# RulinShao/sink-flash-attention-kernel

Hardware: AMD Instinct MI355X
Metric: attn fwd+bwd TFLOP/s (% MFMA peak) at B=4 H=32 N=8192 D=128 bf16 (higher is better)
Workload: dtype bf16

## Files before the change

### include/sfa.h

```cpp
#ifndef SFA_H
#define SFA_H

#include <stddef.h>
#include <stdint.h>

#ifdef __cplusplus
extern "C" {
#endif

#define SFA_ABI_VERSION 2

#define SFA_DTYPE_F32 0
#define SFA_DTYPE_F16 1
#define SFA_DTYPE_BF16 2

#define SFA_OK 0
#define SFA_ERR_INVALID_ARGUMENT (-1)
#define SFA_ERR_UNSUPPORTED (-2)
#define SFA_ERR_WORKSPACE (-3)

#define SFA_FLAG_FORCE_GENERIC 0x1u
#define SFA_FLAG_DECODE_ONE_PASS 0x4u
#define SFA_FLAG_BWD_OVERLAP 0x8u
#define SFA_FLAG_BWD_DKDV_ASM 0x10u
#define SFA_FLAG_BWD_DKDV_WS 0x20u

typedef struct sfa_tensor {
    void* ptr;
    int64_t shape[4];
    int64_t stride[4];
    int32_t dtype;
    int32_t reserved;
} sfa_tensor;

int sfa_abi_version(void);

const char* sfa_last_error(void);

const char* sfa_last_path(void);

int sfa_debug_set_variant(int which, int value);
int sfa_debug_set_ptr(void* device_buffer);
int sfa_debug_set_stage_events(void* const* events, int count);

int sfa_fwd(const sfa_tensor* q, const sfa_tensor* k, const sfa_tensor* v, const sfa_tensor* o,
            float* lse, const float* s_aux, int num_sink, int window, float scale,
            unsigned flags, void* stream);

size_t sfa_bwd_workspace_bytes(int64_t B, int64_t Hq, int64_t Hkv, int64_t N, int64_t D, int dtype,
                               int num_sink, int window, unsigned flags);

int sfa_bwd(const sfa_tensor* q, const sfa_tensor* k, const sfa_tensor* v, const sfa_tensor* o,
            const sfa_tensor* d_o, const float* lse, const float* s_aux, const sfa_tensor* dq,
            const sfa_tensor* dk, const sfa_tensor* dv, float* ds_aux, void* workspace,
            size_t workspace_bytes, int num_sink, int window, float scale, unsigned flags,
            void* stream);

int sfa_varlen_supported(int dtype, int64_t D);

int sfa_fwd_varlen(const sfa_tensor* q, const sfa_tensor* k, const sfa_tensor* v, const sfa_tensor* o, float* lse,
                   const float* s_aux, const int32_t* cu_seqlens, int n_seq, int max_seqlen, int num_sink,
                   int window, float scale, unsigned flags, void* stream);

int sfa_bwd_varlen(const sfa_tensor* q, const sfa_tensor* k, const sfa_tensor* v, const sfa_tensor* o,
                   const sfa_tensor* d_o, const float* lse, const float* s_aux, const sfa_tensor* dq,
                   const sfa_tensor* dk, const sfa_tensor* dv, float* ds_aux, const int32_t* cu_seqlens, int n_seq,
                   int max_seqlen, void* workspace, size_t workspace_bytes, int num_sink, int window, float scale,
                   unsigned flags, void* stream);

size_t sfa_decode_workspace_bytes(int64_t B, int64_t Hq, int64_t Hkv, int64_t Nkv, int64_t D,
                                  int dtype);

int sfa_decode(const sfa_tensor* q, const sfa_tensor* k, const sfa_tensor* v, const sfa_tensor* o,
               const float* s_aux, void* workspace, size_t workspace_bytes, float scale,
               unsigned flags, void* stream);

int sfa_decode_ring(const sfa_tensor* q, const sfa_tensor* sink_k, const sfa_tensor* sink_v, int64_t sink_len,
                    const sfa_tensor* window_k, const sfa_tensor* window_v, int64_t window_len,
                    const sfa_tensor* o, const float* s_aux, void* workspace, size_t workspace_bytes,
                    float scale, unsigned flags, void* stream);

int sfa_decode_ring_step(const sfa_tensor* q, const sfa_tensor* sink_k, const sfa_tensor* sink_v, int64_t sink_len,
                         const sfa_tensor* window_k, const sfa_tensor* window_v, int64_t window_len,
                         int64_t write_pos, const sfa_tensor* k_new, const sfa_tensor* v_new, const sfa_tensor* o,
                         const float* s_aux, void* workspace, size_t workspace_bytes, float scale, unsigned flags,
                         void* stream);

int sfa_decode_ring_step_dyn(const sfa_tensor* q, const sfa_tensor* sink_k, const sfa_tensor* sink_v,
                             const sfa_tensor* window_k, const sfa_tensor* window_v, const sfa_tensor* k_new,
                             const sfa_tensor* v_new, const sfa_tensor* o, const float* s_aux, int32_t* state,
                             void* workspace, size_t workspace_bytes, float scale, unsigned flags, void* stream);

size_t sfa_decode_multi_workspace_bytes(int64_t B, int64_t Hq, int64_t Hkv, int64_t n_new, int64_t Nkv, int64_t D,
                                        int dtype);

int sfa_decode_ring_multi(const sfa_tensor* q, const sfa_tensor* sink_k, const sfa_tensor* sink_v, int64_t sink_len,
                          const sfa_tensor* window_k, const sfa_tensor* window_v, int64_t window_len,
                          int64_t write_pos, const sfa_tensor* k_new, const sfa_tensor* v_new, const sfa_tensor* o,
                          const float* s_aux, int commit, void* workspace, size_t workspace_bytes, float scale,
                          unsigned flags, void* stream);

int sfa_decode_ring_multi_dyn(const sfa_tensor* q, const sfa_tensor* sink_k, const sfa_tensor* sink_v,
                              const sfa_tensor* window_k, const sfa_tensor* window_v, const sfa_tensor* k_new,
                              const sfa_tensor* v_new, const sfa_tensor* o, const float* s_aux, int commit,
                              int32_t* state, void* workspace, size_t workspace_bytes, float scale, unsigned flags,
                              void* stream);

int sfa_ring_commit_dyn(const sfa_tensor* window_k, const sfa_tensor* window_v, const sfa_tensor* k_new,
                        const sfa_tensor* v_new, const int32_t* count, int32_t* state, void* stream);


int sfa_decode_ring_step_rows(const sfa_tensor* q, const sfa_tensor* sink_k, const sfa_tensor* sink_v,
                              const sfa_tensor* window_k, const sfa_tensor* window_v, const sfa_tensor* k_new,
                              const sfa_tensor* v_new, const sfa_tensor* o, const float* s_aux, int32_t* state,
                              void* workspace, size_t workspace_bytes, float scale, unsigned flags, void* stream);

int sfa_decode_ring_multi_rows(const sfa_tensor* q, const sfa_tensor* sink_k, const sfa_tensor* sink_v,
                               const sfa_tensor* window_k, const sfa_tensor* window_v, const sfa_tensor* k_new,
                               const sfa_tensor* v_new, const sfa_tensor* o, const float* s_aux, int commit,
                               int32_t* state, void* workspace, size_t workspace_bytes, float scale, unsigned flags,
                               void* stream);

int sfa_ring_commit_rows(const sfa_tensor* window_k, const sfa_tensor* window_v, const sfa_tensor* k_new,
                         const sfa_tensor* v_new, const int32_t* count, int32_t* state, void* stream);

int sfa_ring_fill_varlen(const sfa_tensor* sink_k, const sfa_tensor* sink_v, const sfa_tensor* window_k,
                         const sfa_tensor* window_v, const sfa_tensor* k, const sfa_tensor* v,
                         const int32_t* cu_seqlens, int n_seq, int32_t* state, void* stream);

int sfa_decode_ring_tree(const sfa_tensor* q, const sfa_tensor* sink_k, const sfa_tensor* sink_v, int64_t sink_len,
                         const sfa_tensor* window_k, const sfa_tensor* window_v, int64_t window_len,
                         int64_t write_pos, const sfa_tensor* k_new, const sfa_tensor* v_new, const sfa_tensor* o,
                         const float* s_aux, const int32_t* parent, int64_t parent_bstride, void* workspace,
                         size_t workspace_bytes, float scale, unsigned flags, void* stream);

int sfa_decode_ring_tree_dyn(const sfa_tensor* q, const sfa_tensor* sink_k, const sfa_tensor* sink_v,
                             const sfa_tensor* window_k, const sfa_tensor* window_v, const sfa_tensor* k_new,
                             const sfa_tensor* v_new, const sfa_tensor* o, const float* s_aux, const int32_t* parent,
                             int64_t parent_bstride, int32_t* state, void* workspace, size_t workspace_bytes,
                             float scale, unsigned flags, void* stream);

int sfa_decode_ring_tree_rows(const sfa_tensor* q, const sfa_tensor* sink_k, const sfa_tensor* sink_v,
                              const sfa_tensor* window_k, const sfa_tensor* window_v, const sfa_tensor* k_new,
                              const sfa_tensor* v_new, const sfa_tensor* o, const float* s_aux, const int32_t* parent,
                              int64_t parent_bstride, int32_t* state, void* workspace, size_t workspace_bytes,
                              float scale, unsigned flags, void* stream);

int sfa_ring_commit_path_dyn(const sfa_tensor* window_k, const sfa_tensor* window_v, const sfa_tensor* k_new,
                             const sfa_tensor* v_new, const int32_t* count, const int32_t* path, int64_t path_bstride,
                             int32_t* state, void* stream);

int sfa_ring_commit_path_rows(const sfa_tensor* window_k, const sfa_tensor* window_v, const sfa_tensor* k_new,
                              const sfa_tensor* v_new, const int32_t* count, const int32_t* path, int64_t path_bstride,
                              int32_t* state, void* stream);


int sfa_decode_ring_step_slots(const sfa_tensor* q, const sfa_tensor* sink_k, const sfa_tensor* sink_v,
                               const sfa_tensor* window_k, const sfa_tensor* window_v, const sfa_tensor* k_new,
                               const sfa_tensor* v_new, const sfa_tensor* o, const float* s_aux, int32_t* state,
                               const int32_t* slots, void* workspace, size_t workspace_bytes, float scale,
                               unsigned flags, void* stream);

int sfa_decode_ring_multi_slots(const sfa_tensor* q, const sfa_tensor* sink_k, const sfa_tensor* sink_v,
                                const sfa_tensor* window_k, const sfa_tensor* window_v, const sfa_tensor* k_new,
                                const sfa_tensor* v_new, const sfa_tensor* o, const float* s_aux, int commit,
                                int32_t* state, const int32_t* slots, void* workspace, size_t workspace_bytes,
                                float scale, unsigned flags, void* stream);

int sfa_decode_ring_tree_slots(const sfa_tensor* q, const sfa_tensor* sink_k, const sfa_tensor* sink_v,
                               const sfa_tensor* window_k, const sfa_tensor* window_v, const sfa_tensor* k_new,
                               const sfa_tensor* v_new, const sfa_tensor* o, const float* s_aux, const int32_t* parent,
                               int64_t parent_bstride, int32_t* state, const int32_t* slots, void* workspace,
                               size_t workspace_bytes, float scale, unsigned flags, void* stream);

int sfa_ring_commit_slots(const sfa_tensor* window_k, const sfa_tensor* window_v, const sfa_tensor* k_new,
                          const sfa_tensor* v_new, const int32_t* count, int32_t* state, const int32_t* slots,
                          void* stream);

int sfa_ring_commit_path_slots(const sfa_tensor* window_k, const sfa_tensor* window_v, const sfa_tensor* k_new,
                               const sfa_tensor* v_new, const int32_t* count, const int32_t* path, int64_t path_bstride,
                               int32_t* state, const int32_t* slots, void* stream);

int sfa_ring_fill_varlen_slots(const sfa_tensor* sink_k, const sfa_tensor* sink_v, const sfa_tensor* window_k,
                               const sfa_tensor* window_v, const sfa_tensor* k, const sfa_tensor* v,
                               const int32_t* cu_seqlens, int n_seq, int32_t* state, const int32_t* slots,
                               void* stream);

size_t sfa_decode_ragged_workspace_bytes(int64_t n_seq, int64_t Hq, int64_t Hkv, int64_t T, int64_t Nkv_cache,
                                         int64_t D, int dtype);

int sfa_decode_ring_ragged_slots(const sfa_tensor* q, const sfa_tensor* sink_k, const sfa_tensor* sink_v,
                                 const sfa_tensor* window_k, const sfa_tensor* window_v, const sfa_tensor* k_new,
                                 const sfa_tensor* v_new, const sfa_tensor* o, const float* s_aux, int commit,
                                 int32_t* state, const int32_t* slots, const int32_t* cu_q, int n_seq,
                                 void* workspace, size_t workspace_bytes, float scale, unsigned flags, void* stream);

#ifdef __cplusplus
}
#endif
#endif
```

### sink-flash-attention-kernel_amd/csrc/sfa_api.hip

```cpp
#include <cmath>
#include <cstring>
#include <initializer_list>

#include "sfa_common.hpp"
#include "sfa_internal.hpp"

namespace sfa {

static thread_local char g_err[512] = "";
static char g_path[128] = "";

void* g_debug_ptr = nullptr;
int g_variant[8] = {0, 0, 0, 0, 0, 0, 0, 0};
static void* const* g_stage_events = nullptr;
static int g_stage_count = 0;
bool stage_events_armed() { return g_stage_events != nullptr; }
void record_stage(int i, hipStream_t stream) {
    if (g_stage_events && i < g_stage_count && g_stage_events[i]) (void)hipEventRecord((hipEvent_t)g_stage_events[i], stream);
}

void set_error(const char* fmt, ...) {
    va_list ap;
    va_start(ap, fmt);
    vsnprintf(g_err, sizeof(g_err), fmt, ap);
    va_end(ap);
}
void set_path(const char* fmt, ...) {
    va_list ap;
    va_start(ap, fmt);
    vsnprintf(g_path, sizeof(g_path), fmt, ap);
    va_end(ap);
}

namespace {

int check_tensor(const sfa_tensor* t, const char* name) {
    SFA_CHECK_ARG(t != nullptr, "%s: null tensor descriptor", name);
    SFA_CHECK_ARG(t->dtype == SFA_DTYPE_F32 || t->dtype == SFA_DTYPE_F16 || t->dtype == SFA_DTYPE_BF16,
                  "%s: unknown dtype %d", name, t->dtype);
    for (int i = 0; i < 4; ++i) SFA_CHECK_ARG(t->shape[i] >= 0, "%s: negative shape[%d]", name, i);
    const bool empty = t->shape[0] == 0 || t->shape[1] == 0 || t->shape[2] == 0 || t->shape[3] == 0;
    SFA_CHECK_ARG(empty || t->ptr != nullptr, "%s: null data pointer", name);
    SFA_CHECK_ARG(t->shape[3] <= 1 || t->stride[3] == 1, "%s: last-dim stride must be 1 (got %lld)", name,
                  (long long)t->stride[3]);
    for (int i = 0; i < 3; ++i)
        SFA_CHECK_ARG(t->stride[i] >= 0, "%s: negative stride[%d] not supported", name, i);
    return SFA_OK;
}

int same_shape(const sfa_tensor* a, const sfa_tensor* b, const char* an, const char* bn) {
    for (int i = 0; i < 4; ++i)
        SFA_CHECK_ARG(a->shape[i] == b->shape[i], "%s and %s differ in shape[%d]: %lld vs %lld", an, bn, i,
                      (long long)a->shape[i], (long long)b->shape[i]);
    SFA_CHECK_ARG(a->dtype == b->dtype, "%s and %s differ in dtype", an, bn);
    return SFA_OK;
}

int check_prefill(const sfa_tensor* q, const sfa_tensor* k, const sfa_tensor* v, Problem* p, int num_sink,
                  int window, float scale) {
    int st;
    if ((st = check_tensor(q, "q")) || (st = check_tensor(k, "k")) || (st = check_tensor(v, "v"))) return st;
    if ((st = same_shape(k, v, "k", "v"))) return st;
    SFA_CHECK_ARG(q->dtype == k->dtype, "q and k differ in dtype");
    SFA_CHECK_ARG(q->shape[0] == k->shape[0], "batch mismatch: q %lld vs k %lld", (long long)q->shape[0],
                  (long long)k->shape[0]);
    SFA_CHECK_ARG(q->shape[2] <= k->shape[2], "prefill needs N_q <= N_kv (q %lld, k %lld)", (long long)q->shape[2],
                  (long long)k->shape[2]);
    SFA_CHECK_ARG(q->shape[3] == k->shape[3], "head dim mismatch");
    SFA_CHECK_ARG(k->shape[1] > 0 && q->shape[1] % k->shape[1] == 0, "H_q (%lld) must be divisible by H_kv (%lld)",
                  (long long)q->shape[1], (long long)k->shape[1]);
    SFA_CHECK_ARG(q->shape[2] < (1ll << 30) && q->shape[0] * q->shape[1] < (1ll << 30), "problem too large");
    SFA_CHECK_ARG(num_sink >= 0, "num_sink must be >= 0");
    SFA_CHECK_ARG(std::isfinite(scale), "scale must be finite");
    p->B = (int)q->shape[0];
    p->Hq = (int)q->shape[1];
    p->Hkv = (int)k->shape[1];
    p->N = (int)q->shape[2];
    p->Nk = (int)k->shape[2];
    p->D = (int)q->shape[3];
    p->num_sink = num_sink;
    p->window = window;
    p->scale = scale;
    return SFA_OK;
}

inline size_t align256(size_t x) { return (x + 255) & ~(size_t)255; }

struct BwdWorkspace {
    size_t delta_off, dsaux_off, mfma_off, total;
};

BwdWorkspace bwd_layout(const Problem& p, int dtype, bool use_mfma, unsigned flags) {
    BwdWorkspace w;
    size_t off = 0;
    w.delta_off = off;
    off += align256((size_t)p.B * p.Hq * p.N * sizeof(float));
    w.dsaux_off = off;
    off += align256((size_t)p.B * p.Hq * (size_t)bwd_preprocess_nblk(p.N) * sizeof(float));
    w.mfma_off = off;
    if (use_mfma) off += align256(bwd_mfma_workspace_bytes(p, dtype, flags));
    w.total = off;
    return w;
}

}
}

using namespace sfa;

extern "C" {

int sfa_abi_version(void) { return SFA_ABI_VERSION; }
const char* sfa_last_error(void) { return g_err; }
const char* sfa_last_path(void) { return g_path; }
int sfa_debug_set_variant(int which, int value) {
    if (which < 0 || which >= 8) return SFA_ERR_INVALID_ARGUMENT;
    __atomic_store_n(&sfa::g_variant[which], value, __ATOMIC_RELAXED);
    return SFA_OK;
}

int sfa_debug_set_ptr(void* p) {
    sfa::g_debug_ptr = p;
    return SFA_OK;
}

int sfa_debug_set_stage_events(void* const* events, int count) {
    g_stage_events = count > 0 ? events : nullptr;
    g_stage_count = count > 0 ? count : 0;
    return SFA_OK;
}

int sfa_fwd(const sfa_tensor* q, const sfa_tensor* k, const sfa_tensor* v, const sfa_tensor* o, float* lse,
            const float* s_aux, int num_sink, int window, float scale, unsigned flags, void* stream) {
    g_err[0] = 0;
    Problem p;
    int st = check_prefill(q, k, v, &p, num_sink, window, scale);
    if (st) return st;
    if ((st = check_tensor(o, "o")) || (st = same_shape(q, o, "q", "o"))) return st;
    if (p.B == 0 || p.Hq == 0 || p.N == 0) return SFA_OK;
    SFA_CHECK_ARG(p.D > 0, "head dim must be > 0");
    SFA_CHECK_ARG(lse != nullptr, "lse: null pointer");
    hipStream_t s = (hipStream_t)stream;
    if (!(flags & SFA_FLAG_FORCE_GENERIC) && fwd_mfma_supported(q->dtype, p.D))
        return fwd_mfma(q, k, v, o, lse, s_aux, p, s);
    if (p.Nk != p.N) {
        set_error("N_q != N_kv is served by the MFMA kernels only (16-bit dtypes, head dims 64/80/96/128)");
        return SFA_ERR_UNSUPPORTED;
    }
    return fwd_generic(q, k, v, o, lse, s_aux, p, s);
}

size_t sfa_bwd_workspace_bytes(int64_t B, int64_t Hq, int64_t Hkv, int64_t N, int64_t D, int dtype, int num_sink,
                               int window, unsigned flags) {
    Problem p{(int)B, (int)Hq, (int)Hkv, (int)N, (int)D, num_sink, window, 1.f};
    const bool use_mfma = !(flags & SFA_FLAG_FORCE_GENERIC) && bwd_mfma_supported(dtype, (int)D);
    return bwd_layout(p, dtype, use_mfma, flags).total;
}

int sfa_bwd(const sfa_tensor* q, const sfa_tensor* k, const sfa_tensor* v, const sfa_tensor* o,
            const sfa_tensor* d_o, const float* lse, const float* s_aux, const sfa_tensor* dq, const sfa_tensor* dk,
            const sfa_tensor* dv, float* ds_aux, void* workspace, size_t workspace_bytes, int num_sink, int window,
            float scale, unsigned flags, void* stream) {
    g_err[0] = 0;
    Problem p;
    int st = check_prefill(q, k, v, &p, num_sink, window, scale);
    if (st) return st;
    if ((st = check_tensor(o, "o")) || (st = same_shape(q, o, "q", "o"))) return st;
    if ((st = check_tensor(d_o, "do")) || (st = same_shape(q, d_o, "q", "do"))) return st;
    if ((st = check_tensor(dq, "dq")) || (st = same_shape(q, dq, "q", "dq"))) return st;
    if ((st = check_tensor(dk, "dk")) || (st = same_shape(k, dk, "k", "dk"))) return st;
    if ((st = check_tensor(dv, "dv")) || (st = same_shape(v, dv, "v", "dv"))) return st;
    if (p.B == 0 || p.Hq == 0 || p.N == 0) return SFA_OK;
    SFA_CHECK_ARG(p.D > 0, "head dim must be > 0");
    SFA_CHECK_ARG(lse != nullptr, "lse: null pointer");
    SFA_CHECK_ARG((s_aux == nullptr) == (ds_aux == nullptr), "ds_aux must be given iff s_aux is");
    const bool use_mfma = !(flags & SFA_FLAG_FORCE_GENERIC) && bwd_mfma_supported(q->dtype, p.D);
    if (use_mfma && (st = bwd_mfma_refused(q, k, v, d_o, dq, dk, dv, p))) return st;
    const BwdWorkspace w = bwd_layout(p, q->dtype, use_mfma, flags);
    if (workspace == nullptr || workspace_bytes < w.total || ((uintptr_t)workspace & 255) != 0) {
        set_error("bwd workspace: need %zu bytes, 256-byte aligned (got %zu at %p)", w.total, workspace_bytes,
                  workspace);
        return SFA_ERR_WORKSPACE;
    }
    hipStream_t s = (hipStream_t)stream;
    float* delta = reinterpret_cast<float*>((char*)workspace + w.delta_off);
    float* dsaux_part = reinterpret_cast<float*>((char*)workspace + w.dsaux_off);
    record_stage(0, s);
    const bool fuse = use_mfma && bwd_mfma_wants_consts() && bwd_preprocess_vectorised(o, d_o, p);
    st = bwd_preprocess(o, d_o, lse, s_aux, delta, dsaux_part, ds_aux, p, s,
                        fuse ? reinterpret_cast<float*>((char*)workspace + w.mfma_off) : nullptr, bwd_mfma_lse_factor(p, flags));
    record_stage(1, s);
    if (st) return st;
    if (use_mfma)
        st = bwd_mfma(q, k, v, d_o, lse, delta, dq, dk, dv, (char*)workspace + w.mfma_off, p, flags, s, fuse);
    else if (p.Nk != p.N) {
        set_error("N_q != N_kv is served by the MFMA kernels only (16-bit dtypes, head dims 64/80/96/128)");
        st = SFA_ERR_UNSUPPORTED;
    } else
        st = bwd_generic(q, k, v, d_o, lse, delta, dq, dk, dv, p, s);
    record_stage(3, s);
    return st;
}

int sfa_varlen_supported(int dtype, int64_t D) {
    return fwd_mfma_supported(dtype, (int)D) && bwd_mfma_varlen_supported(dtype, (int)D) ? 1 : 0;
}

static int check_varlen(const sfa_tensor* q, const sfa_tensor* k, const sfa_tensor* v, const int32_t* cu, int n_seq,
                        int max_seqlen, int num_sink, int window, float scale, Problem* p, Problem* run) {
    int st = check_prefill(q, k, v, p, num_sink, window, scale);
    if (st) return st;
    SFA_CHECK_ARG(p->B == 1, "packed layout: batch dim must be 1 (got %d)", p->B);
    SFA_CHECK_ARG(p->N == p->Nk, "packed layout: q and k must have the same number of rows");
    SFA_CHECK_ARG(cu != nullptr && n_seq >= 1, "cu_seqlens: need a device array of n_seq + 1 >= 2 offsets");
    SFA_CHECK_ARG(max_seqlen >= 1 && max_seqlen <= p->N, "max_seqlen %d out of range (total rows %d)", max_seqlen, p->N);
    if (!sfa_varlen_supported(q->dtype, p->D)) {
        set_error("packed (varlen) kernels exist for 16-bit dtypes and head dims 64/80/96/128 only");
        return SFA_ERR_UNSUPPORTED;
    }
    *run = *p;
    run->B = n_seq;
    run->N = max_seqlen;
    run->cu = cu;
    run->n_total = p->N;
    run->Nk = 0;
    return SFA_OK;
}

int sfa_fwd_varlen(const sfa_tensor* q, const sfa_tensor* k, const sfa_tensor* v, const sfa_tensor* o, float* lse,
                   const float* s_aux, const int32_t* cu_seqlens, int n_seq, int max_seqlen, int num_sink, int window,
                   float scale, unsigned flags, void* stream) {
    g_err[0] = 0;
    (void)flags;
    Problem p, run;
    int st = check_varlen(q, k, v, cu_seqlens, n_seq, max_seqlen, num_sink, window, scale, &p, &run);
    if (st) return st;
    if ((st = check_tensor(o, "o")) || (st = same_shape(q, o, "q", "o"))) return st;
    if (p.Hq == 0 || p.N == 0) return SFA_OK;
    SFA_CHECK_ARG(lse != nullptr, "lse: null pointer");
    return fwd_mfma(q, k, v, o, lse, s_aux, run, (hipStream_t)stream);
}

int sfa_bwd_varlen(const sfa_tensor* q, const sfa_tensor* k, const sfa_tensor* v, const sfa_tensor* o,
                   const sfa_tensor* d_o, const float* lse, const float* s_aux, const sfa_tensor* dq,
                   const sfa_tensor* dk, const sfa_tensor* dv, float* ds_aux, const int32_t* cu_seqlens, int n_seq,
                   int max_seqlen, void* workspace, size_t workspace_bytes, int num_sink, int window, float scale,
                   unsigned flags, void* stream) {
    g_err[0] = 0;
    (void)flags;
    Problem p, run;
    int st = check_varlen(q, k, v, cu_seqlens, n_seq, max_seqlen, num_sink, window, scale, &p, &run);
    if (st) return st;
    if ((st = check_tensor(o, "o")) || (st = same_shape(q, o, "q", "o"))) return st;
    if ((st = check_tensor(d_o, "do")) || (st = same_shape(q, d_o, "q", "do"))) return st;
    if ((st = check_tensor(dq, "dq")) || (st = same_shape(q, dq, "q", "dq"))) return st;
    if ((st = check_tensor(dk, "dk")) || (st = same_shape(k, dk, "k", "dk"))) return st;
    if ((st = check_tensor(dv, "dv")) || (st = same_shape(v, dv, "v", "dv"))) return st;
    if (p.Hq == 0 || p.N == 0) return SFA_OK;
    SFA_CHECK_ARG(lse != nullptr, "lse: null pointer");
    SFA_CHECK_ARG((s_aux == nullptr) == (ds_aux == nullptr), "ds_aux must be given iff s_aux is");
    if ((st = bwd_mfma_refused(q, k, v, d_o, dq, dk, dv, run))) return st;
    const BwdWorkspace w = bwd_layout(p, q->dtype, true, 0);
    if (workspace == nullptr || workspace_bytes < w.total || ((uintptr_t)workspace & 255) != 0) {
        set_error("bwd workspace: need %zu bytes, 256-byte aligned (got %zu at %p)", w.total, workspace_bytes,
                  workspace);
        return SFA_ERR_WORKSPACE;
    }
    hipStream_t s = (hipStream_t)stream;
    float* delta = reinterpret_cast<float*>((char*)workspace + w.delta_off);
    float* dsaux_part = reinterpret_cast<float*>((char*)workspace + w.dsaux_off);
    record_stage(0, s);
    const bool fuse = bwd_mfma_wants_consts() && bwd_preprocess_vectorised(o, d_o, p);
    st = bwd_preprocess(o, d_o, lse, s_aux, delta, dsaux_part, ds_aux, p, s,
                        fuse ? reinterpret_cast<float*>((char*)workspace + w.mfma_off) : nullptr,
                        bwd_mfma_lse_factor(run, flags));
    record_stage(1, s);
    if (st) return st;
    st = bwd_mfma(q, k, v, d_o, lse, delta, dq, dk, dv, (char*)workspace + w.mfma_off, run, flags, s, fuse);
    record_stage(3, s);
    return st;
}

size_t sfa_decode_workspace_bytes(int64_t B, int64_t Hq, int64_t Hkv, int64_t Nkv, int64_t D, int dtype) {
    DecodePlan pl;
    if (decode_plan(B, Hq, Hkv, Nkv, D, dtype, &pl) != SFA_OK) return 0;
    return decode_counter_bytes(B, Hkv) + align256((size_t)B * Hq * pl.max_splits * (size_t)(D + 2) * sizeof(float));
}

}

namespace {

#define SFA_NEED(p, what) SFA_CHECK_ARG((p) != nullptr, what ": null device pointer")

int check_rows16(std::initializer_list<const sfa_tensor*> ts, int es, unsigned skip, const char* msg) {
    for (const sfa_tensor* t : ts) {
        if (!t || ((skip & 1) && t->shape[0] == 0) || ((skip & 2) && t->shape[1] == 0) || ((skip & 4) && t->shape[2] == 0))
            continue;
        SFA_CHECK_ARG(((uintptr_t)t->ptr % 16) == 0 && (t->stride[0] * es) % 16 == 0 && (t->stride[1] * es) % 16 == 0 &&
                          (t->stride[2] * es) % 16 == 0,
                      "%s", msg);
    }
    return SFA_OK;
}

int check_workspace(const char* name, size_t need, bool sized, void* workspace, size_t workspace_bytes) {
    if (!sized || workspace == nullptr || workspace_bytes < need || ((uintptr_t)workspace & 255) != 0) {
        set_error("%s workspace: need %zu bytes, 256-byte aligned (got %zu at %p)", name, need, workspace_bytes, workspace);
        return SFA_ERR_WORKSPACE;
    }
    return SFA_OK;
}

RingCall attend_call(const sfa_tensor* q, const sfa_tensor* sink_k, const sfa_tensor* sink_v, const sfa_tensor* window_k,
                     const sfa_tensor* window_v, const sfa_tensor* k_new, const sfa_tensor* v_new, const sfa_tensor* o,
                     const float* s_aux, void* workspace, size_t workspace_bytes, float scale, unsigned flags,
                     void* stream) {
    RingCall c{};
    c.q = q, c.sink_k = sink_k, c.sink_v = sink_v, c.window_k = window_k, c.window_v = window_v;
    c.k_new = k_new, c.v_new = v_new, c.o = o, c.s_aux = s_aux;
    c.workspace = workspace, c.workspace_bytes = workspace_bytes;
    c.scale = scale, c.flags = flags, c.stream = (hipStream_t)stream;
    return c;
}

RingCall& host_state(RingCall& c, int64_t sink_len, int64_t window_len, int64_t write_pos) {
    c.mode = RingState::Host, c.sink_len = sink_len, c.window_len = window_len, c.write_pos = write_pos;
    return c;
}

RingCall& device_state(RingCall& c, RingState mode, int32_t* state, const int32_t* slots) {
    c.mode = mode, c.state = state, c.slots = slots;
    c.sink_len = c.sink_k ? c.sink_k->shape[2] : 0, c.window_len = c.window_k ? c.window_k->shape[2] : 0;
    return c;
}

int check_device_state(const RingCall& c) {
    if (c.mode == RingState::Host) return SFA_OK;
    SFA_NEED(c.state, "state");
    SFA_CHECK_ARG(c.sink_k != nullptr && c.window_k != nullptr, "cache buffers: null tensor descriptor");
    return SFA_OK;
}

int ring_step(const RingCall& c) {
    g_err[0] = 0;
    int st;
    if ((st = check_device_state(c))) return st;
    const sfa_tensor *q = c.q, *k = c.sink_k, *v = c.sink_v, *k2 = c.window_k, *v2 = c.window_v, *o = c.o;
    const sfa_tensor *k_new = c.k_new, *v_new = c.v_new;
    const int64_t n1 = c.sink_len, n2 = c.window_len;
    const bool pool = c.slots != nullptr;
    if ((st = check_tensor(q, "q")) || (st = check_tensor(k, "k")) || (st = check_tensor(v, "v")) ||
        (st = check_tensor(o, "o")))
        return st;
    if ((st = same_shape(k, v, "k", "v")) || (st = same_shape(q, o, "q", "o"))) return st;
    SFA_CHECK_ARG(q->dtype == k->dtype, "q and k differ in dtype");
    SFA_CHECK_ARG(q->shape[2] == 1, "sink_decode_attention requires N_q=1, got %lld", (long long)q->shape[2]);
    if (pool)
        SFA_CHECK_ARG(k->shape[0] >= 1 && k->shape[0] < (1ll << 30),
                      "pool: the cache buffers need shape[0] = S slots, 1 <= S < 2^30 (got %lld)", (long long)k->shape[0]);
    SFA_CHECK_ARG((pool || q->shape[0] == k->shape[0]) && q->shape[3] == k->shape[3], "q/k batch or head-dim mismatch");
    SFA_CHECK_ARG(k->shape[1] > 0 && q->shape[1] % k->shape[1] == 0, "H_q (%lld) must be divisible by H_kv (%lld)",
                  (long long)q->shape[1], (long long)k->shape[1]);
    SFA_CHECK_ARG(std::isfinite(c.scale), "scale must be finite");
    SFA_CHECK_ARG(n1 >= 0 && n1 <= k->shape[2], "first key segment: %lld valid rows of %lld", (long long)n1,
                  (long long)k->shape[2]);
    if (k2 || v2 || n2) {
        SFA_CHECK_ARG(k2 && v2, "second key segment needs both k and v");
        if ((st = check_tensor(k2, "k2")) || (st = check_tensor(v2, "v2")) || (st = same_shape(k2, v2, "k2", "v2")))
            return st;
        if (pool)
            SFA_CHECK_ARG(k2->shape[0] == k->shape[0], "pool: sink and window buffers must share shape[0] = S (sink %lld, window %lld)",
                          (long long)k->shape[0], (long long)k2->shape[0]);
        SFA_CHECK_ARG(k2->dtype == k->dtype && k2->shape[0] == k->shape[0] && k2->shape[1] == k->shape[1] &&
                          k2->shape[3] == k->shape[3],
                      "the two key segments must agree in dtype, batch, heads and head dim");
        SFA_CHECK_ARG(n2 >= 0 && n2 <= k2->shape[2], "second key segment: %lld valid rows of %lld", (long long)n2,
                      (long long)k2->shape[2]);
    }
    SFA_CHECK_ARG(n1 + n2 < (1ll << 31) - 4096, "N_kv too large");
    if (k_new || v_new) {
        SFA_CHECK_ARG(k_new && v_new && k2 && v2, "fused step needs k_new, v_new and the window ring");
        if ((st = check_tensor(k_new, "k_new")) || (st = check_tensor(v_new, "v_new")) ||
            (st = same_shape(k_new, v_new, "k_new", "v_new")))
            return st;
        if (pool)
            SFA_CHECK_ARG(k_new->shape[0] == q->shape[0], "q, k_new, v_new and o must share shape[0] = B (q %lld, k_new %lld)",
                          (long long)q->shape[0], (long long)k_new->shape[0]);
        SFA_CHECK_ARG(k_new->dtype == k2->dtype && (pool || k_new->shape[0] == k2->shape[0]) && k_new->shape[1] == k2->shape[1] &&
                          k_new->shape[2] == 1 && k_new->shape[3] == k2->shape[3],
                      "k_new / v_new must be [B, H_kv, 1, D] in the ring's dtype");
        SFA_CHECK_ARG(c.mode != RingState::Host || (c.write_pos >= 0 && c.write_pos < n2),
                      "write slot %lld outside the %lld valid ring slots", (long long)c.write_pos, (long long)n2);
// ... 403 lines not shown
```

### sink-flash-attention-kernel_amd/csrc/sfa_bwd_mfma.hip

```cpp
#include "sfa_common.hpp"
#include "sfa_internal.hpp"
#include "sfa_worklist.hpp"

#include <cstdlib>
#include <type_traits>

#include "gen/dkdv_asm.inc"
#include "gen/dq_asm.inc"
#include "gen/dkdv_skew_asm.inc"
#include "gen/dq_strip_asm.inc"

namespace sfa {
namespace {

typedef __attribute__((ext_vector_type(8))) __bf16 bf16x8_t;
typedef __attribute__((ext_vector_type(8))) _Float16 f16x8_t;
typedef __attribute__((ext_vector_type(4))) short s16x4;
typedef __attribute__((ext_vector_type(8))) short s16x8;
typedef __attribute__((ext_vector_type(16))) float f32x16;
typedef __attribute__((ext_vector_type(4))) float f32x4;
typedef __attribute__((ext_vector_type(4))) unsigned int u32x4;
typedef __attribute__((ext_vector_type(2))) unsigned int u32x2;

#ifdef SFA_STAMPS
// ... 769 lines not shown
    s.q_lo = u((unsigned)qb); s.q_hi = u((unsigned)(qb >> 32));
    s.do_lo = u((unsigned)dob); s.do_hi = u((unsigned)(dob >> 32));
    s.c_lo = u((unsigned)cb); s.c_hi = u((unsigned)(cb >> 32));
    s.k_lo = u((unsigned)kbp); s.k_hi = u((unsigned)(kbp >> 32));
    s.v_lo = u((unsigned)vbp); s.v_hi = u((unsigned)(vbp >> 32));
    s.dk_lo = u((unsigned)dkb); s.dk_hi = u((unsigned)(dkb >> 32));
    s.dv_lo = u((unsigned)dvb); s.dv_hi = u((unsigned)(dvb >> 32));
    const bool split = (kb < a.sink_blocks ? a.sink_chunks : a.gen_chunks) > 1;
    s.pk_lo = s.pk_hi = s.pv_lo = s.pv_hi = s.p_rng = u(0u);
    if (split) {
        const uint64_t pb = (uint64_t)(a.sink_ws) +
                            ((uint64_t)grp * part_slots(a, a.n_kblocks) + part_first(a, kb) + chunk) * 2 * a.sink_rows * D * 4 -
                            (uint64_t)kb0 * D * 4;
        const uint64_t pvb = pb + (uint64_t)a.sink_rows * D * 4;
        s.pk_lo = u((unsigned)pb); s.pk_hi = u((unsigned)(pb >> 32));
        s.pv_lo = u((unsigned)pvb); s.pv_hi = u((unsigned)(pvb >> 32));
        s.p_rng = u((unsigned)((kb0 + a.sink_rows) * D * 4));
    }
    s.q_rng = u(seq_range(a.cu, a.q_range, N, a.q.sn, D));
    s.do_rng = u(seq_range(a.cu, a.do_range, N, a.d_o.sn, D));
    s.c_rng = u((unsigned)((2 * NT_ - sq.row0) * 4));
    s.k_rng = u(seq_range(a.cu, a.k_range, Nk, a.k.sn, D));
    s.v_rng = u(seq_range(a.cu, a.v_range, Nk, a.v.sn, D));
    s.dk_rng = u(seq_range(a.cu, a.dk_range, Nk, a.dk.sn, D));
    s.dv_rng = u(seq_range(a.cu, a.dv_range, Nk, a.dv.sn, D));
    s.q_sn = u((unsigned)(a.q.sn * 2)); s.do_sn = u((unsigned)(a.d_o.sn * 2));
    s.k_sn = u((unsigned)(a.k.sn * 2)); s.v_sn = u((unsigned)(a.v.sn * 2));
    s.dk_sn = u((unsigned)(a.dk.sn * 2)); s.dv_sn = u((unsigned)(a.dv.sn * 2));
    if (chunk > 0) s.dk_rng = s.dv_rng = u(0u);
    s.q_hs = u((unsigned)(a.q.sh * 2)); s.do_hs = u((unsigned)(a.d_o.sh * 2));
    s.c_hs = u((unsigned)(2 * NT_ * 4));
    s.nq = u((unsigned)nq); s.g = u((unsigned)g); s.q_row0 = u((unsigned)(qt_lo * 32)); s.kb0 = u((unsigned)kb0);
    s.pos0 = u((unsigned)P); s.W = u((unsigned)W); s.ns = u((unsigned)a.num_sink); s.nrows = u((unsigned)N);
    s.cdelta = u((unsigned)(NT_ * 4));
    s.c_log2 = u(__float_as_uint(a.scale_log2)); s.scale = u(__float_as_uint(a.scale));
#ifdef SFA_DKDV_STAMPS
    s.dbg_lo = u((unsigned)(uint64_t)a.dbg); s.dbg_hi = u((unsigned)((uint64_t)a.dbg >> 32)); s.bid = u((unsigned)bid);
#endif
    const unsigned tid = threadIdx.x;
    if (a.B < 0) smem[tid] = 0;
#ifdef SFA_AB
    if constexpr (ALT == 1) {
        asm volatile(SFA_DKDV_ASM_BF16_ALT : : SFA_DKDV_INPUTS(s), [tid] "v"(tid) : SFA_DKDV_CLOBBERS);
        return;
    }
#endif
#define SFA_DKDV_BODY(DD)                                                                                        \
    if constexpr (D == DD) {                                                                                       \
        if constexpr (std::is_same<T, bf16_t>::value)                                                              \
            asm volatile(SFA_DKDV_ASM_BF16_D##DD : : SFA_DKDV_INPUTS(s), [tid] "v"(tid) : SFA_DKDV_CLOBBERS);       \
        else                                                                                                       \
            asm volatile(SFA_DKDV_ASM_F16_D##DD : : SFA_DKDV_INPUTS(s), [tid] "v"(tid) : SFA_DKDV_CLOBBERS);        \
    }
    SFA_DKDV_BODY(64) SFA_DKDV_BODY(80) SFA_DKDV_BODY(96) SFA_DKDV_BODY(128)
#undef SFA_DKDV_BODY
}

template <typename T, int D>
__global__ __launch_bounds__(256) void bwd_dkdv_skew_asm_kernel(BwdArgs a) {
    extern __shared__ __attribute__((aligned(16))) char smem[];
    const int nK = a.n_kblocks;
    const int bid = xcd_remap((int)blockIdx.x, (int)gridDim.x);
    const int kb = bid % nK, grp = bid / nK;
    const int hk = grp % a.Hkv;
    const int b = grp / a.Hkv;
    const SeqInfo sq = seq_of(a.cu, b, a.N);
    const int N = sq.N;
    const int W = a.window < N ? a.window : N;
    const int NT_ = a.cu ? a.n_total : N;
    const int g = a.Hq / a.Hkv;
    const int kb0 = kb * kKBA;
    if (kb0 >= N) return;
    int trips = (62 + W) / 32 + 1;
    if (trips < SFA_DKDVSK_SKEW) trips = SFA_DKDVSK_SKEW;
    const int head0 = hk * g;
    const uint64_t qb = (uint64_t)(a.q.ptr + ((int64_t)sq.bb * a.q.sb + (int64_t)head0 * a.q.sh + (int64_t)sq.row0 * a.q.sn) * 2);
    const uint64_t dob = (uint64_t)(a.d_o.ptr + ((int64_t)sq.bb * a.d_o.sb + (int64_t)head0 * a.d_o.sh + (int64_t)sq.row0 * a.d_o.sn) * 2);
    const uint64_t cb = (uint64_t)(a.consts + ((int64_t)sq.bb * a.Hq + head0) * 2 * NT_ + sq.row0);
    const uint64_t kbp = (uint64_t)(a.k.ptr + ((int64_t)sq.bb * a.k.sb + (int64_t)hk * a.k.sh + (int64_t)sq.row0 * a.k.sn) * 2);
    const uint64_t vbp = (uint64_t)(a.v.ptr + ((int64_t)sq.bb * a.v.sb + (int64_t)hk * a.v.sh + (int64_t)sq.row0 * a.v.sn) * 2);
    const uint64_t dkb = (uint64_t)(a.dk.ptr + ((int64_t)sq.bb * a.dk.sb + (int64_t)hk * a.dk.sh + (int64_t)sq.row0 * a.dk.sn) * 2);
    const uint64_t dvb = (uint64_t)(a.dv.ptr + ((int64_t)sq.bb * a.dv.sb + (int64_t)hk * a.dv.sh + (int64_t)sq.row0 * a.dv.sn) * 2);
    auto u = [](unsigned x) { return (unsigned)__builtin_amdgcn_readfirstlane((int)x); };
    DkdvSkewScalars s;
    s.q_lo = u((unsigned)qb); s.q_hi = u((unsigned)(qb >> 32));
    s.do_lo = u((unsigned)dob); s.do_hi = u((unsigned)(dob >> 32));
    s.c_lo = u((unsigned)cb); s.c_hi = u((unsigned)(cb >> 32));
    s.k_lo = u((unsigned)kbp); s.k_hi = u((unsigned)(kbp >> 32));
    s.v_lo = u((unsigned)vbp); s.v_hi = u((unsigned)(vbp >> 32));
    s.dk_lo = u((unsigned)dkb); s.dk_hi = u((unsigned)(dkb >> 32));
    s.dv_lo = u((unsigned)dvb); s.dv_hi = u((unsigned)(dvb >> 32));
    s.q_rng = u(seq_range(a.cu, a.q_range, N, a.q.sn, D));
    s.do_rng = u(seq_range(a.cu, a.do_range, N, a.d_o.sn, D));
    s.c_rng = u((unsigned)((2 * NT_ - sq.row0) * 4));
    s.k_rng = u(seq_range(a.cu, a.k_range, N, a.k.sn, D));
    s.v_rng = u(seq_range(a.cu, a.v_range, N, a.v.sn, D));
    s.dk_rng = u(seq_range(a.cu, a.dk_range, N, a.dk.sn, D));
    s.dv_rng = u(seq_range(a.cu, a.dv_range, N, a.dv.sn, D));
    s.q_sn = u((unsigned)(a.q.sn * 2)); s.do_sn = u((unsigned)(a.d_o.sn * 2));
    s.k_sn = u((unsigned)(a.k.sn * 2)); s.v_sn = u((unsigned)(a.v.sn * 2));
    s.dk_sn = u((unsigned)(a.dk.sn * 2)); s.dv_sn = u((unsigned)(a.dv.sn * 2));
    s.q_hs = u((unsigned)(a.q.sh * 2)); s.do_hs = u((unsigned)(a.d_o.sh * 2));
    s.c_hs = u((unsigned)(2 * NT_ * 4));
    s.nq = u((unsigned)trips); s.g = u((unsigned)g); s.q_row0 = u((unsigned)kb0); s.kb0 = u((unsigned)kb0);
    s.W = u((unsigned)W); s.nrows = u((unsigned)N);
    s.cdelta = u((unsigned)(NT_ * 4));
    s.c_log2 = u(__float_as_uint(a.scale_log2)); s.scale = u(__float_as_uint(a.scale));
    const unsigned tid = threadIdx.x;
    if (a.B < 0) smem[tid] = 0;
#define SFA_DKDVSK_BODY(DD)                                                                                          \
    if constexpr (D == DD) {                                                                                           \
        if constexpr (std::is_same<T, bf16_t>::value)                                                                  \
            asm volatile(SFA_DKDVSK_ASM_BF16_D##DD : : SFA_DKDVSK_INPUTS(s), [tid] "v"(tid) : SFA_DKDVSK_CLOBBERS);     \
        else                                                                                                           \
            asm volatile(SFA_DKDVSK_ASM_F16_D##DD : : SFA_DKDVSK_INPUTS(s), [tid] "v"(tid) : SFA_DKDVSK_CLOBBERS);      \
    }
    SFA_DKDVSK_BODY(64) SFA_DKDVSK_BODY(80) SFA_DKDVSK_BODY(96)
#undef SFA_DKDVSK_BODY
}

constexpr int kDynTicketDword = 512;
template <typename T, int D, int ALT>
__global__ __launch_bounds__(256) void bwd_dq_asm_pk_kernel(BwdArgs a) {
    extern __shared__ __attribute__((aligned(16))) char smem[];
    const int G = (int)gridDim.x, w = (int)blockIdx.x;
    const unsigned tid = threadIdx.x;
    const int n_groups = a.hgroups * a.Hkv * a.B;
    const int64_t n_ranks = (int64_t)a.n_qtiles * n_groups;
    const int g = a.Hq / a.Hkv, BM = 64 * a.rb, ns = a.num_sink;
    auto u = [](unsigned x) { return (unsigned)__builtin_amdgcn_readfirstlane((int)x); };
#ifdef SFA_WL_STAMPS
    const unsigned wl_t0 = u((unsigned)__builtin_amdgcn_s_memrealtime());
    const unsigned wl_c0 = u((unsigned)__builtin_amdgcn_s_memtime());
#endif
    DqPkScalars s;
    s.q_hs = u((unsigned)(a.q.sh * 2)); s.q_sn = u((unsigned)(a.q.sn * 2));
    s.do_hs = u((unsigned)(a.d_o.sh * 2)); s.do_sn = u((unsigned)(a.d_o.sn * 2));
    s.dq_hs = u((unsigned)(a.dq.sh * 2)); s.dq_sn = u((unsigned)(a.dq.sn * 2));
    s.k_sn = u((unsigned)(a.k.sn * 2)); s.v_sn = u((unsigned)(a.v.sn * 2));
    s.ld_hs = u((unsigned)((a.cu ? a.n_total : a.N) * 4));
    s.pos0 = u((unsigned)(a.cu ? 0 : a.Nk - a.N)); s.W = u((unsigned)a.window); s.ns = u((unsigned)ns);
    s.hpw_log2 = u(a.hpw == 4 ? 2u : (a.hpw == 2 ? 1u : 0u));
    s.c_log2 = u(__float_as_uint(a.scale_log2)); s.nlog2e = u(__float_as_uint(-kLog2e)); s.scale = u(__float_as_uint(a.scale));
    const int64_t n_static = a.wl_dyn > 0 && a.wl_dyn < n_ranks ? a.wl_dyn : n_ranks;
    int n_done = 0;
    for (bool first = true;; first = false) {
        const int j = (int)tid;
        bool valid = false;
        unsigned d[SFA_WL_DESC_DWORDS];
#pragma unroll
        for (int i = 0; i < SFA_WL_DESC_DWORDS; ++i) d[i] = 0;
        int64_t r_dyn = -1;
        if (!first) {
            __syncthreads();
            if (tid == 0) reinterpret_cast<volatile int*>(smem)[8] = (int)atomicAdd(a.tickets + kDynTicketDword, 1u);
            __syncthreads();
            r_dyn = n_static + reinterpret_cast<volatile int*>(smem)[8];
            if (r_dyn >= n_ranks) break;
        }
        {
            const int64_t r = first ? ((int64_t)j * G < n_static ? wl_rank(j, w, G) : -1) : (j == 0 ? r_dyn : -1);
            const int qt = a.n_qtiles - 1 - (int)((r < 0 ? 0 : r) / n_groups);
            int rest = (int)((r < 0 ? 0 : r) % n_groups);
            if (r >= 0 && r < (first ? n_static : n_ranks)) {
                const int hg = rest % a.hgroups;
                rest /= a.hgroups;
                const int hk = rest % a.Hkv;
                const int b = rest / a.Hkv;
                const SeqInfo sq = seq_of(a.cu, b, a.N);
                const int N = sq.N;
                const int P = a.cu ? 0 : a.Nk - a.N;
                const int Nk = N + P;
                const int W = a.window < Nk ? a.window : Nk;
                const int q0 = qt * BM;
                if (q0 < N) {
                    valid = true;
                    const int q1 = (q0 + BM < N) ? q0 + BM : N;
                    const int ns_eff = ns < q1 + P ? ns : q1 + P;
                    const int ts_hi = (ns_eff + 63) >> 6;
                    int wlo = q0 + P - W + 1;
                    if (wlo < 0) wlo = 0;
                    int tw_lo = wlo >> 6;
                    if (tw_lo < ts_hi) tw_lo = ts_hi;
                    const int tw_hi = (q1 + P + 63) >> 6;
                    if (tw_lo > tw_hi) tw_lo = tw_hi;
                    const int head0 = hk * g + hg * a.hpw;
                    const int64_t lrow = a.cu ? (int64_t)head0 * a.n_total + sq.row0 : ((int64_t)b * a.Hq + head0) * N;
                    const uint64_t qb = (uint64_t)(a.q.ptr + ((int64_t)sq.bb * a.q.sb + (int64_t)head0 * a.q.sh + (int64_t)sq.row0 * a.q.sn) * 2);
                    const uint64_t dob = (uint64_t)(a.d_o.ptr + ((int64_t)sq.bb * a.d_o.sb + (int64_t)head0 * a.d_o.sh + (int64_t)sq.row0 * a.d_o.sn) * 2);
                    const uint64_t dqb = (uint64_t)(a.dq.ptr + ((int64_t)sq.bb * a.dq.sb + (int64_t)head0 * a.dq.sh + (int64_t)sq.row0 * a.dq.sn) * 2);
                    const uint64_t kbp = (uint64_t)(a.k.ptr + ((int64_t)sq.bb * a.k.sb + (int64_t)hk * a.k.sh + (int64_t)sq.row0 * a.k.sn) * 2);
                    const uint64_t vbp = (uint64_t)(a.v.ptr + ((int64_t)sq.bb * a.v.sb + (int64_t)hk * a.v.sh + (int64_t)sq.row0 * a.v.sn) * 2);
                    const uint64_t lb = (uint64_t)(a.lse + lrow), db_ = (uint64_t)(a.delta + lrow);
                    d[SFA_DQPK_F_q_lo] = (unsigned)qb; d[SFA_DQPK_F_q_hi] = (unsigned)(qb >> 32);
                    d[SFA_DQPK_F_do_lo] = (unsigned)dob; d[SFA_DQPK_F_do_hi] = (unsigned)(dob >> 32);
                    d[SFA_DQPK_F_lse_lo] = (unsigned)lb; d[SFA_DQPK_F_lse_hi] = (unsigned)(lb >> 32);
                    d[SFA_DQPK_F_dl_lo] = (unsigned)db_; d[SFA_DQPK_F_dl_hi] = (unsigned)(db_ >> 32);
                    d[SFA_DQPK_F_dq_lo] = (unsigned)dqb; d[SFA_DQPK_F_dq_hi] = (unsigned)(dqb >> 32);
                    d[SFA_DQPK_F_q0] = (unsigned)q0; d[SFA_DQPK_F_nrows] = (unsigned)N;
                    d[SFA_DQPK_F_q_rng] = seq_range(a.cu, a.q_range, N, a.q.sn, D);
                    d[SFA_DQPK_F_do_rng] = seq_range(a.cu, a.do_range, N, a.d_o.sn, D);
                    d[SFA_DQPK_F_dq_rng] = seq_range(a.cu, a.dq_range, N, a.dq.sn, D);
                    d[SFA_DQPK_F_k_lo] = (unsigned)kbp; d[SFA_DQPK_F_k_hi] = (unsigned)(kbp >> 32);
                    d[SFA_DQPK_F_v_lo] = (unsigned)vbp; d[SFA_DQPK_F_v_hi] = (unsigned)(vbp >> 32);
                    d[SFA_DQPK_F_k_rng] = seq_range(a.cu, a.k_range, Nk, a.k.sn, D);
                    d[SFA_DQPK_F_v_rng] = seq_range(a.cu, a.v_range, Nk, a.v.sn, D);
                    d[SFA_DQPK_F_nt] = (unsigned)(ts_hi + (tw_hi - tw_lo));
                    d[SFA_DQPK_F_ts_hi] = (unsigned)ts_hi; d[SFA_DQPK_F_tw_off] = (unsigned)(tw_lo - ts_hi);
                }
            }
        }
        int n_items = 0;
        const int idx = wl_compact(valid, reinterpret_cast<int*>(smem), &n_items);
        if (valid) {
            uint4* dst = reinterpret_cast<uint4*>(smem + SFA_DQPK_DESC_BASE + idx * (SFA_WL_DESC_DWORDS * 4));
#pragma unroll
            for (int i = 0; i < SFA_WL_DESC_DWORDS / 4; ++i) dst[i] = make_uint4(d[4 * i], d[4 * i + 1], d[4 * i + 2], d[4 * i + 3]);
        }
        __syncthreads();
        s.n_items = u((unsigned)n_items);
        n_done += n_items;
#ifdef SFA_DQPK_STAMPS
        s.dbg_lo = u((unsigned)(uint64_t)a.dbg); s.dbg_hi = u((unsigned)((uint64_t)a.dbg >> 32)); s.bid = u((unsigned)blockIdx.x);
#endif
        if (n_items > 0) {
#ifdef SFA_AB
            if constexpr (ALT == 1) asm volatile(SFA_DQPK_ASM_BF16_ALT : : SFA_DQPK_INPUTS(s), [tid] "v"(tid) : SFA_DQPK_CLOBBERS);
#endif
#define SFA_DQPK_BODY(DD)                                                                                      \
    if constexpr (D == DD && ALT == 0) {                                                                         \
        if constexpr (std::is_same<T, bf16_t>::value)                                                            \
            asm volatile(SFA_DQPK_ASM_BF16_D##DD : : SFA_DQPK_INPUTS(s), [tid] "v"(tid) : SFA_DQPK_CLOBBERS);     \
        else                                                                                                     \
            asm volatile(SFA_DQPK_ASM_F16_D##DD : : SFA_DQPK_INPUTS(s), [tid] "v"(tid) : SFA_DQPK_CLOBBERS);      \
    }
            SFA_DQPK_BODY(64) SFA_DQPK_BODY(80) SFA_DQPK_BODY(96) SFA_DQPK_BODY(128)
#undef SFA_DQPK_BODY
        }
        if (n_static >= n_ranks) break;
    }
    {
#ifdef SFA_WL_STAMPS
        if (a.dbg && threadIdx.x == 0) {
            unsigned* rec = reinterpret_cast<unsigned*>(a.dbg) + 4 * blockIdx.x;
            rec[0] = wl_t0;
            rec[1] = (unsigned)__builtin_amdgcn_s_memrealtime();
            rec[2] = (unsigned)__builtin_amdgcn_s_getreg(20 | (3 << 11));
            rec[3] = ((unsigned)n_done & 1023u) | ((((unsigned)__builtin_amdgcn_s_memtime() - wl_c0) >> 4) << 10);
        }
#endif
    }
    (void)n_done;
}

template <typename T, int D, int NT>
__global__ __launch_bounds__(256) void bwd_dq_strip_asm_kernel(BwdArgs a) {
    extern __shared__ __attribute__((aligned(16))) char smem[];
    const int bid = xcd_remap(blockIdx.x, gridDim.x);
    const int sidx = bid % a.n_strips;
    int rest = bid / a.n_strips;
    const int hg = rest % a.hgroups;
    rest /= a.hgroups;
    const int hk = rest % a.Hkv;
    const int b = rest / a.Hkv;
    const SeqInfo sq = seq_of(a.cu, b, a.N);
    const int N = sq.N;
    const int q0 = sidx * a.strip * 64;
    if (q0 >= N) return;
    const int n_tiles = (N + 63) >> 6;
    int n_it = n_tiles - sidx * a.strip;
    if (n_it > a.strip) n_it = a.strip;
    const int g = a.Hq / a.Hkv;
    const int head0 = hk * g + hg * 4;
    const int64_t lrow = a.cu ? (int64_t)head0 * a.n_total + sq.row0 : ((int64_t)b * a.Hq + head0) * N;
    const uint64_t qb = (uint64_t)(a.q.ptr + ((int64_t)sq.bb * a.q.sb + (int64_t)head0 * a.q.sh + (int64_t)sq.row0 * a.q.sn) * 2);
    const uint64_t dob = (uint64_t)(a.d_o.ptr + ((int64_t)sq.bb * a.d_o.sb + (int64_t)head0 * a.d_o.sh + (int64_t)sq.row0 * a.d_o.sn) * 2);
    const uint64_t dqb = (uint64_t)(a.dq.ptr + ((int64_t)sq.bb * a.dq.sb + (int64_t)head0 * a.dq.sh + (int64_t)sq.row0 * a.dq.sn) * 2);
    const uint64_t kbp = (uint64_t)(a.k.ptr + ((int64_t)sq.bb * a.k.sb + (int64_t)hk * a.k.sh + (int64_t)sq.row0 * a.k.sn) * 2);
    const uint64_t vbp = (uint64_t)(a.v.ptr + ((int64_t)sq.bb * a.v.sb + (int64_t)hk * a.v.sh + (int64_t)sq.row0 * a.v.sn) * 2);
    const uint64_t lb = (uint64_t)(a.lse + lrow), db_ = (uint64_t)(a.delta + lrow);
    auto u = [](unsigned x) { return (unsigned)__builtin_amdgcn_readfirstlane((int)x); };
    DqStripScalars s;
    s.q_lo = u((unsigned)qb); s.q_hi = u((unsigned)(qb >> 32)); s.q_hs = u((unsigned)(a.q.sh * 2));
    s.q_sn = u((unsigned)(a.q.sn * 2)); s.q_rng = u(seq_range(a.cu, a.q_range, N, a.q.sn, D));
    s.do_lo = u((unsigned)dob); s.do_hi = u((unsigned)(dob >> 32)); s.do_hs = u((unsigned)(a.d_o.sh * 2));
    s.do_sn = u((unsigned)(a.d_o.sn * 2)); s.do_rng = u(seq_range(a.cu, a.do_range, N, a.d_o.sn, D));
    s.dq_lo = u((unsigned)dqb); s.dq_hi = u((unsigned)(dqb >> 32)); s.dq_hs = u((unsigned)(a.dq.sh * 2));
    s.dq_sn = u((unsigned)(a.dq.sn * 2)); s.dq_rng = u(seq_range(a.cu, a.dq_range, N, a.dq.sn, D));
    s.k_lo = u((unsigned)kbp); s.k_hi = u((unsigned)(kbp >> 32)); s.k_sn = u((unsigned)(a.k.sn * 2));
    s.k_rng = u(seq_range(a.cu, a.k_range, N, a.k.sn, D));
    s.v_lo = u((unsigned)vbp); s.v_hi = u((unsigned)(vbp >> 32)); s.v_sn = u((unsigned)(a.v.sn * 2));
    s.v_rng = u(seq_range(a.cu, a.v_range, N, a.v.sn, D));
    s.lse_lo = u((unsigned)lb); s.lse_hi = u((unsigned)(lb >> 32)); s.dl_lo = u((unsigned)db_); s.dl_hi = u((unsigned)(db_ >> 32));
    s.ld_hs = u((unsigned)((a.cu ? a.n_total : N) * 4));
    s.q0 = u((unsigned)q0); s.n_it = u((unsigned)n_it); s.nrows = u((unsigned)N);
    s.W = u((unsigned)(a.window < N ? a.window : N));
    s.c_log2 = u(__float_as_uint(a.scale_log2)); s.nlog2e = u(__float_as_uint(-kLog2e)); s.scale = u(__float_as_uint(a.scale));
    const unsigned tid = threadIdx.x;
    if (a.B < 0) smem[tid] = 0;
#define SFA_DQSTRIP_BODY(DD, NN)                                                                                          \
    if constexpr (D == DD && NT == NN) {                                                                                    \
        if constexpr (std::is_same<T, bf16_t>::value)                                                                       \
            asm volatile(SFA_DQSTRIP_ASM_BF16_D##DD##_NT##NN : : SFA_DQSTRIP_INPUTS(s), [tid] "v"(tid) : SFA_DQSTRIP_CLOBBERS); \
        else                                                                                                                \
            asm volatile(SFA_DQSTRIP_ASM_F16_D##DD##_NT##NN : : SFA_DQSTRIP_INPUTS(s), [tid] "v"(tid) : SFA_DQSTRIP_CLOBBERS);  \
    }
    SFA_DQSTRIP_BODY(64, 2) SFA_DQSTRIP_BODY(64, 3) SFA_DQSTRIP_BODY(64, 4)
    SFA_DQSTRIP_BODY(80, 2) SFA_DQSTRIP_BODY(80, 3) SFA_DQSTRIP_BODY(80, 4)
#undef SFA_DQSTRIP_BODY
}
// ... 561 lines not shown
}
int device_cu_count();
bool asm_window_ok(int D, int window, int64_t wgs) {
    static const int min_window = env_int("SFA_ASM_MIN_WINDOW", kAsmMinWindow);
    if (D == 128) return true;
    if (!(D >= 64 && D < 128)) return false;
    return window > min_window || wgs >= 2 * (int64_t)device_cu_count();
}
int device_cu_count() {
    static const int n_cu = [] {
        int dev = 0, n = 256;
        if (hipGetDevice(&dev) != hipSuccess || hipDeviceGetAttribute(&n, hipDeviceAttributeMultiprocessorCount, dev) != hipSuccess) n = 256;
        return n > 0 ? n : 256;
    }();
    return n_cu;
}
constexpr int kSkewMaxWindow = 512;
bool dkdv_skew(int D, int window, int num_sink, bool self_attn, unsigned flags) {
    static const int knob = env_int("SFA_DKDV_SKEW", 1);
    if (!(D == 64 || D == 80 || D == 96) || knob != 1 || dkdv_mode() != 4) return false;
    if (flags & (SFA_FLAG_BWD_DKDV_WS | SFA_FLAG_BWD_DKDV_ASM)) return false;
    return num_sink <= 0 && self_attn && window >= 1 && window <= kSkewMaxWindow;
}
bool dkdv_asm(int D, int window, int Nk, int groups, bool can_split, unsigned flags, int num_sink, bool self_attn) {
    if (dkdv_skew(D, window, num_sink, self_attn, flags)) return true;
    if (!(dkdv_mode() == 4 && asm_window_ok(D, window, cdiv64(Nk, kKBA) * groups))) return false;
    if (flags & SFA_FLAG_BWD_DKDV_WS) return false;
    if (flags & SFA_FLAG_BWD_DKDV_ASM) return true;
    static const int min_wgs = env_int("SFA_DKDV_MIN_WGS", -1);
    static const int row_split = env_int("SFA_ROW_SPLIT", 1);
    const int64_t need = min_wgs >= 0 ? min_wgs : device_cu_count();
    return cdiv64(Nk, kKBA) * groups >= need || (can_split && row_split == 1);
}

struct SideStream {
    int dev = -1;
    hipStream_t stream = nullptr;
    hipEvent_t fork = nullptr, join = nullptr;
};
struct SideStreams {
    SideStream slot[16];
    int n = 0;
    ~SideStreams() {
        for (int i = 0; i < n; ++i) {
            if (slot[i].fork) (void)hipEventDestroy(slot[i].fork);
            if (slot[i].join) (void)hipEventDestroy(slot[i].join);
            if (slot[i].stream) (void)hipStreamDestroy(slot[i].stream);
        }
    }
};
SideStream* side_stream(hipStream_t caller) {
    thread_local SideStreams tls;
    int dev = -1;
    if (hipGetDevice(&dev) != hipSuccess) return nullptr;
    for (int i = 0; i < tls.n; ++i)
        if (tls.slot[i].dev == dev) return &tls.slot[i];
    hipStreamCaptureStatus cs = hipStreamCaptureStatusNone;
    if (hipStreamIsCapturing(caller, &cs) != hipSuccess || cs != hipStreamCaptureStatusNone) return nullptr;
    if (tls.n >= 16) return nullptr;
    SideStream s;
    s.dev = dev;
    int prio_least = 0, prio_greatest = 0;
    (void)hipDeviceGetStreamPriorityRange(&prio_least, &prio_greatest);
    if (hipStreamCreateWithPriority(&s.stream, hipStreamNonBlocking, prio_least) != hipSuccess) return nullptr;
    if (hipEventCreateWithFlags(&s.fork, hipEventDisableTiming) != hipSuccess ||
        hipEventCreateWithFlags(&s.join, hipEventDisableTiming) != hipSuccess) {
        if (s.fork) (void)hipEventDestroy(s.fork);
        (void)hipStreamDestroy(s.stream);
        return nullptr;
    }
    tls.slot[tls.n] = s;
    return &tls.slot[tls.n++];
}

int64_t worklist_grid(int64_t n_ranks) {
    const int64_t n_cu = device_cu_count();
    int64_t G = n_ranks < n_cu ? n_ranks : n_cu;
    const int64_t need = cdiv64(n_ranks, SFA_WL_MAX_ITEMS);
    return G > need ? G : need;
}

template <typename T, int D>
int launch_bwd(const BwdArgs& a, int B, hipStream_t stream) {
    constexpr int ROWB = (D <= 64) ? 128 : 256;
    const bool self_attn = a.cu != nullptr || a.Nk == a.N;
    bool skew = false;
    if constexpr (D == 64 || D == 80 || D == 96) skew = dkdv_skew(D, a.window, a.num_sink, self_attn, a.flags);
    const int mode = skew ? 5 : (dkdv_asm(D, a.window, a.Nk, a.Hkv * B, a.cu == nullptr && a.Nk == a.N, a.flags, a.num_sink, self_attn) ? 4 : 3);
    if (!a.consts_ready) {
        const int rows = a.cu ? a.n_total : a.N;
        const int64_t total = (a.cu ? 1 : (int64_t)B) * a.Hq * rows;
        bwd_consts_kernel<<<dim3((unsigned)cdiv64(total, 256)), dim3(256), 0, stream>>>(
            a.lse, a.delta, const_cast<float*>(a.consts), rows, total, mode >= 4 ? 1.f / a.scale : kLog2e);
    }
    static const int dq_asm_knob = env_int("SFA_DQ", 1);
    bool overlap = false;
    SideStream* ss = nullptr;
    if constexpr (D >= 64) {
        const int gq = a.Hq / a.Hkv, hpwq = gq % 4 == 0 ? 4 : (gq % 2 == 0 ? 2 : 1);
        const int64_t dq_wgs = cdiv64(a.N, 64 * (4 / hpwq)) * (gq / hpwq) * a.Hkv * B;
        overlap = (a.flags & SFA_FLAG_BWD_OVERLAP) && dq_wgs < 4 * (int64_t)device_cu_count() && !stage_events_armed() &&
                  dq_asm_knob == 1 && asm_window_ok(D, a.window, cdiv64(a.Nk, kKBA) * a.Hkv * B) && (a.window > 0 || a.num_sink > 0);
        if (overlap) {
            ss = side_stream(stream);
            overlap = ss != nullptr;
        }
        if (overlap) {
            (void)hipEventRecord(ss->fork, stream);
            (void)hipStreamWaitEvent(ss->stream, ss->fork, 0);
        }
    }
    struct Join {
        SideStream* s;
        hipStream_t main;
        ~Join() {
            if (s) {
                (void)hipEventRecord(s->join, s->stream);
                (void)hipStreamWaitEvent(main, s->join, 0);
            }
        }
    } join{overlap ? ss : nullptr, stream};
    int split_gen = 1;
    if constexpr (D == 64 || D == 80 || D == 96) if (mode == 5) {
        BwdArgs a5 = a;
        a5.n_kblocks = (int)cdiv64(a.Nk, kKBA);
        auto kern = bwd_dkdv_skew_asm_kernel<T, D>;
        static unsigned long long done = 0;
        ensure_dynamic_lds((const void*)kern, SFA_DKDVSK_LDS_BYTES, &done);
        kern<<<dim3(a5.n_kblocks * a.Hkv * B), dim3(256), SFA_DKDVSK_LDS_BYTES, stream>>>(a5);
        const int st = launch_status("bwd_dkdv_skew_asm");
        if (st) return st;
    }
    if constexpr (D >= 64) if (mode == 4) {
        BwdArgs a4 = a;
        a4.n_kblocks = (int)cdiv64(a.Nk, kKBA);
        a4.prio = variant(3);
        const SinkSplit sp = row_split_plan(a.N, a.Nk, a.num_sink, a.window, a.cu != nullptr, a.Hkv * B, a.Hq / a.Hkv);
        a4.sink_chunks = sp.chunks;
        a4.chunk_slices = sp.chunk_slices;
        a4.sink_rows = sp.rows;
        a4.gen_chunks = sp.gen;
        split_gen = sp.gen;
        a4.sink_blocks = sp.nsb;
        a4.n_extra = row_split_extras(sp, a4.n_kblocks) * a.Hkv * B;
        auto kern = bwd_dkdv_asm_kernel<T, D, 0>;
        static unsigned long long done = 0;
        ensure_dynamic_lds((const void*)kern, SFA_DKDV_LDS_BYTES, &done);
        static const int ticket_knob = env_int("SFA_TICKETS", 1);
        int grid = a4.n_extra + a4.n_kblocks * a.Hkv * B;
        if (ticket_knob == 1 && variant(7) == 0 && a4.n_kblocks * a.Hkv * B >= 2 * device_cu_count()) {
            a4.n_base = a4.n_kblocks * a.Hkv * B;
            const int surplus = ((a4.n_base / 8 + 7) / 8) * 8;
            grid += surplus;
            (void)hipMemsetAsync(a4.tickets, 0, 1024, stream);
        }
#ifdef SFA_AB
        if (variant(0) == 1 && std::is_same<T, bf16_t>::value && D == 128) {
            auto kalt = bwd_dkdv_asm_kernel<T, 128, 1>;
            static unsigned long long done_alt = 0;
            ensure_dynamic_lds((const void*)kalt, SFA_DKDV_LDS_BYTES, &done_alt);
            kalt<<<dim3(grid), dim3(256), SFA_DKDV_LDS_BYTES, stream>>>(a4);
        } else
#endif
        kern<<<dim3(grid), dim3(256), SFA_DKDV_LDS_BYTES, stream>>>(a4);
        int st = launch_status("bwd_dkdv_asm");
        if (st) return st;
        if (a4.n_extra > 0) {
            bwd_part_reduce_kernel<T><<<dim3(a.Hkv * B, sp.gen > 1 ? a4.n_kblocks : sp.nsb, sp.gen > 1 ? 8 : 1), dim3(256), 0, stream>>>(
                a4, D, a4.n_kblocks);
            st = launch_status("bwd_part_reduce");
            if (st) return st;
        }
    }
    if (mode == 3) {
        constexpr int lds = 4 * (2 * 32 * ROWB + 256) + 2 * 4 * 4096;
        BwdArgs aw = a;
        const SinkSplit sp = sink_split_plan(a.N, a.Nk, a.num_sink, a.window, a.cu != nullptr, kKB);
        aw.sink_chunks = sp.chunks;
        aw.chunk_slices = sp.chunk_slices;
        aw.sink_rows = sp.rows;
        aw.gen_chunks = 1;
        aw.sink_blocks = 1;
        aw.n_extra = (sp.chunks - 1) * a.Hkv * B;
        const int nblk = aw.n_extra + a.n_kblocks * a.Hkv * B;
        auto kern = bwd_dkdv_mfma_kernel_ws<T, D>;
        static unsigned long long done = 0;
        ensure_dynamic_lds((const void*)kern, lds, &done);
        kern<<<dim3(nblk), dim3(512), lds, stream>>>(aw);
        int st = launch_status("bwd_dkdv_mfma_ws");
        if (st) return st;
        if (sp.chunks > 1) {
            bwd_sink_reduce_kernel<T><<<dim3(a.Hkv * B, 1), dim3(256), 0, stream>>>(aw, D, 1);
            st = launch_status("bwd_sink_reduce");
            if (st) return st;
        }
    }
    record_stage(2, stream);
    static const int dq_strip_knob = env_int("SFA_DQ_STRIP_ASM", 1);
    if constexpr (D == 64 || D == 80) if (dq_strip_knob == 1 && !overlap && a.num_sink <= 0 && a.Nk == a.N && (a.Hq / a.Hkv) % 4 == 0 &&
                                          strip_asm_nt(a.win_caller) > 0 &&
                                          cdiv64(a.N, 64) * (a.Hq / a.Hkv / 4) * a.Hkv * B >= 2 * (int64_t)device_cu_count()) {
        const int nt = strip_asm_nt(a.win_caller);
        const int st = launch_dq_strip<T, D>(a, B, nt, stream);
        if (st) return st;
        char dk_name[32];
        if (mode == 4 && split_gen > 1) snprintf(dk_name, sizeof dk_name, "asm4x64rs%d", split_gen);
        else snprintf(dk_name, sizeof dk_name, "%s", mode == 5 ? "asmskew" : (mode == 4 ? "asm4x64" : "ws8"));
        set_path("bwd_mfma_%s_d%d_dkdv%s_dqstripasm_nt%d", DT<T>::id == SFA_DTYPE_BF16 ? "bf16" : "f16", D, dk_name, nt);
        return SFA_OK;
    }
    if constexpr (D >= 64) if (dq_asm_knob == 1 && asm_window_ok(D, a.window, cdiv64(a.Nk, kKBA) * a.Hkv * B) && (a.window > 0 || a.num_sink > 0)) {
        hipStream_t dqs = overlap ? ss->stream : stream;
        BwdArgs a4 = a;
        const int g = a.Hq / a.Hkv;
        a4.hpw = g % 4 == 0 ? 4 : (g % 2 == 0 ? 2 : 1);
        a4.rb = 4 / a4.hpw;
        a4.n_qtiles = (int)cdiv64(a.N, 64 * a4.rb);
        a4.hgroups = g / a4.hpw;
        const int64_t nblk = (int64_t)a4.n_qtiles * a4.hgroups * a.Hkv * B;
        a4.B = B;
        auto kpk = bwd_dq_asm_pk_kernel<T, D, 0>;
        static unsigned long long done_pk = 0;
        ensure_dynamic_lds((const void*)kpk, SFA_DQPK_LDS_BYTES, &done_pk);
#ifdef SFA_AB
        if (variant(2) == 1 && std::is_same<T, bf16_t>::value && D == 128) {
            kpk = bwd_dq_asm_pk_kernel<T, D, 1>;
            static unsigned long long done_alt = 0;
            ensure_dynamic_lds((const void*)kpk, SFA_DQPK_LDS_BYTES, &done_alt);
        }
#endif
        const int64_t Gd = worklist_grid(nblk);
        a4.wl_dyn = 0;
        {
            static const int dyn_knob = env_int("SFA_WL_DYN", 1);
            const int64_t rounds = cdiv64(nblk, Gd);
            if (dyn_knob == 1 && variant(5) == 0 && Gd == device_cu_count() && rounds >= 12 && a.tickets != nullptr) {
                int64_t tail = 2;
                if (variant(6) > 0) tail = variant(6);
                a4.wl_dyn = (rounds - tail) * Gd;
                (void)hipMemsetAsync(a.tickets + kDynTicketDword, 0, 128, dqs);
            }
        }
        kpk<<<dim3((unsigned)Gd), dim3(256), SFA_DQPK_LDS_BYTES, dqs>>>(a4);
        char dk_name[32];
        if (mode == 4 && split_gen > 1) snprintf(dk_name, sizeof dk_name, "asm4x64rs%d", split_gen);
        else snprintf(dk_name, sizeof dk_name, "%s", mode == 5 ? "asmskew" : (mode == 4 ? "asm4x64" : "ws8"));
        set_path("bwd_mfma_%s_d%d_dkdv%s_dqasm4x64pk_hpw%d%s", DT<T>::id == SFA_DTYPE_BF16 ? "bf16" : "f16", D, dk_name, a4.hpw,
                 overlap ? "_overlap" : "");
        return launch_status("bwd_dq_asm_pk");
    }
    static const int dq_nw_env = env_int("SFA_DQ_NW", 0);
    const int dq_nw = (dq_nw_env == 4 || dq_nw_env == 8) ? dq_nw_env : (a.window <= 2048 ? 4 : 8);
    if (dq_nw == 4) {
        constexpr int NW = 4;
        constexpr int lds = 2 * 2 * 64 * ROWB;
        BwdArgs a4 = a;
        const int g = a.Hq / a.Hkv;
        a4.hpw = g % 4 == 0 ? 4 : (g % 2 == 0 ? 2 : 1);
        a4.rb = NW / a4.hpw;
        a4.n_qtiles = (int)cdiv64(a.N, 32 * a4.rb);
        a4.hgroups = g / a4.hpw;
        auto kern = bwd_dq_mfma_kernel<T, D, NW>;
        static unsigned long long done = 0;
        ensure_dynamic_lds((const void*)kern, lds, &done);
        const int64_t nblk = (int64_t)a4.n_qtiles * a4.hgroups * a.Hkv * B;
        kern<<<dim3((unsigned)nblk), dim3(NW * 64), lds, stream>>>(a4);
    } else {
        constexpr int NW = 8;
        constexpr int lds = 2 * 2 * 64 * ROWB;
        auto kern = bwd_dq_mfma_kernel<T, D, NW>;
        static unsigned long long done = 0;
        ensure_dynamic_lds((const void*)kern, lds, &done);
        const int nblk = a.n_qtiles * a.hgroups * a.Hkv * B;
        kern<<<dim3(nblk), dim3(NW * 64), lds, stream>>>(a);
    }
    set_path("bwd_mfma_%s_d%d_dkdv%s_dq%dw_hpw%d", DT<T>::id == SFA_DTYPE_BF16 ? "bf16" : "f16", D,
             mode == 5 ? "asmskew" : (mode == 4 ? "asm4x64" : "ws8"), dq_nw, a.hpw);
    return launch_status("bwd_dq_mfma");
}

template <typename T>
int launch_bwd_256(const BwdArgs& a, int B, hipStream_t stream) {
    constexpr int D = 256;
    {
        constexpr int lds = 2 * (2 * 32 * 512 + 256);
        auto kern = bwd_dkdv_split_kernel<T, D>;
        static unsigned long long done = 0;
        ensure_dynamic_lds((const void*)kern, lds, &done);
        kern<<<dim3(a.n_kblocks * a.Hkv * B, 2), dim3(256), lds, stream>>>(a);
        int st = launch_status("bwd_dkdv_split");
        if (st) return st;
    }
    record_stage(2, stream);
    constexpr int NW = 4;
    constexpr int lds = 2 * 2 * 64 * 512;
    BwdArgs a4 = a;
    const int g = a.Hq / a.Hkv;
    a4.hpw = g % 4 == 0 ? 4 : (g % 2 == 0 ? 2 : 1);
    a4.rb = NW / a4.hpw;
    a4.n_qtiles = (int)cdiv64(a.N, 32 * a4.rb);
    a4.hgroups = g / a4.hpw;
    auto kern = bwd_dq_mfma_kernel<T, D, NW>;
    static unsigned long long done = 0;
    ensure_dynamic_lds((const void*)kern, lds, &done);
    const int64_t nblk = (int64_t)a4.n_qtiles * a4.hgroups * a.Hkv * B;
    kern<<<dim3((unsigned)nblk), dim3(NW * 64), lds, stream>>>(a4);
    set_path("bwd_mfma_%s_d256_dkdvsplit_dq4w_hpw%d", DT<T>::id == SFA_DTYPE_BF16 ? "bf16" : "f16", a4.hpw);
    return launch_status("bwd_dq_mfma");
}

template <typename T>
int launch_bwd_d(const BwdArgs& a, int D, int B, hipStream_t stream) {
    switch (D) {
        case 256: return launch_bwd_256<T>(a, B, stream);
        case 32: return launch_bwd<T, 32>(a, B, stream);
        case 64: return launch_bwd<T, 64>(a, B, stream);
        case 80: return launch_bwd<T, 80>(a, B, stream);
        case 96: return launch_bwd<T, 96>(a, B, stream);
        case 128: return launch_bwd<T, 128>(a, B, stream);
    }
    set_error("bwd_mfma: unsupported head dim %d", D);
    return SFA_ERR_UNSUPPORTED;
}

int gcd(int x, int y) { return y == 0 ? x : gcd(y, x % y); }

unsigned slice_range(const sfa_tensor* t) { return (unsigned)(((t->shape[2] - 1) * t->stride[2] + t->shape[3]) * 2); }
bool slice_ok(const sfa_tensor* t) {
    const int64_t reach = (t->shape[2] + 1280) * t->stride[2] * 2 + 512;
    const bool head_ok = t->stride[1] >= 0 && t->stride[1] * 2 < (1ll << 32);
    return reach < (1ll << 32) - 65536 && head_ok && ((uintptr_t)t->ptr % 16) == 0 && (t->stride[0] * 2) % 16 == 0 &&
           (t->stride[1] * 2) % 16 == 0 && (t->stride[2] * 2) % 16 == 0;
}

}

bool bwd_mfma_supported(int dtype, int D) {
    return (dtype == SFA_DTYPE_BF16 || dtype == SFA_DTYPE_F16) &&
           (D == 32 || D == 64 || D == 80 || D == 96 || D == 128 || D == 256);
}
bool bwd_mfma_varlen_supported(int dtype, int D) { return bwd_mfma_supported(dtype, D) && D != 256; }

static size_t consts_bytes(const Problem& p) {
    const size_t rows = p.cu ? (size_t)p.n_total : (size_t)p.B * p.N;
    return (rows * p.Hq * 2 * sizeof(float) + 255) & ~(size_t)255;
}

bool bwd_mfma_varlen_ok() { return true; }
bool bwd_mfma_wants_consts() { return true; }
float bwd_mfma_lse_factor(const Problem& p, unsigned flags) {
    const int Nk = p.cu ? p.N : (p.Nk > 0 ? p.Nk : p.N);
    const int W = p.window < 0 ? 0 : (p.window > Nk ? Nk : p.window);
    return dkdv_asm(p.D, W, Nk, p.Hkv * p.B, p.cu == nullptr && Nk == p.N, flags, p.num_sink, p.cu != nullptr || Nk == p.N) ? 1.f / p.scale : kLog2e;
}

static size_t sink_ws_bytes(const Problem& p) {
    const int Nk = p.cu ? p.N : (p.Nk > 0 ? p.Nk : p.N);
    const int Wn = p.window < 0 ? 0 : (p.window > p.N ? p.N : p.window);
    const SinkSplit sp = sink_split_plan(p.N, p.N < Nk ? p.N : Nk, p.num_sink, Wn, p.cu != nullptr, kKB);
    size_t sink_only = 0;
    if (sp.chunks > 1) {
        const int rows = p.num_sink < kKBA ? p.num_sink : kKBA;
        sink_only = (size_t)p.B * p.Hkv * (sp.chunks - 1) * 2 * rows * p.D * 2;
    }
    size_t general = 0;
    if (p.D >= 64 && p.D <= 128) {
        const SinkSplit rs = row_split_plan(p.N, p.N, p.num_sink, Wn, p.cu != nullptr, p.Hkv * p.B, p.Hq / p.Hkv);
        const int nK = (int)cdiv64(p.N, kKBA);
        const size_t slots = (size_t)rs.nsb * rs.chunks + (rs.gen > 1 ? (size_t)(nK - rs.nsb) * rs.gen : 0);
        if (rs.chunks > 1 || rs.gen > 1) general = (size_t)p.B * p.Hkv * slots * 2 * rs.rows * p.D * 4;
    }
    const size_t need = sink_only > general ? sink_only : general;
    return (need + 255) & ~(size_t)255;
}

constexpr size_t kTicketBytes = 4096;
size_t bwd_mfma_workspace_bytes(const Problem& p, int, unsigned) {
    return consts_bytes(p) + ((sink_ws_bytes(p) + 255) & ~(size_t)255) + kTicketBytes;
}

static bool slices_ok(const sfa_tensor* q, const sfa_tensor* k, const sfa_tensor* v, const sfa_tensor* d_o,
                      const sfa_tensor* dq, const sfa_tensor* dk, const sfa_tensor* dv) {
    return slice_ok(q) && slice_ok(k) && slice_ok(v) && slice_ok(d_o) && slice_ok(dq) && slice_ok(dk) && slice_ok(dv);
}

int bwd_mfma_refused(const sfa_tensor* q, const sfa_tensor* k, const sfa_tensor* v, const sfa_tensor* d_o,
                     const sfa_tensor* dq, const sfa_tensor* dk, const sfa_tensor* dv, const Problem& p) {
    if (!slices_ok(q, k, v, d_o, dq, dk, dv) && (p.cu || (p.Nk > 0 && p.Nk != p.N))) {
        set_error("packed (varlen) / N_q != N_kv backward needs 16-byte aligned rows, < 4 GiB head slices and < 4 GiB head strides");
        return SFA_ERR_UNSUPPORTED;
    }
    if (p.D == 256 && p.cu) {
        set_error("packed (varlen) backward: head dim 256 runs sequence by sequence");
// ... 62 lines not shown
```

### sink-flash-attention-kernel_amd/csrc/sfa_common.hpp

```cpp
#pragma once

#include <hip/hip_runtime.h>
#include <hip/hip_bf16.h>
#include <hip/hip_fp16.h>

#include <cstdarg>
#include <cstdint>
#include <cstdio>
#include <cstdlib>

#include "sfa.h"

namespace sfa {

void set_error(const char* fmt, ...);
void set_path(const char* fmt, ...);
void record_stage(int i, hipStream_t stream);
bool stage_events_armed();
extern void* g_debug_ptr;
extern int g_variant[8];
#ifdef SFA_AB
inline int variant(int which) { return __atomic_load_n(&g_variant[which], __ATOMIC_RELAXED); }
#else
inline int variant(int) { return 0; }
#endif

#define SFA_CHECK_ARG(cond, ...)             \
    do {                                     \
        if (!(cond)) {                       \
            ::sfa::set_error(__VA_ARGS__);   \
            return SFA_ERR_INVALID_ARGUMENT; \
        }                                    \
    } while (0)

inline void ensure_dynamic_lds(const void* kernel, int bytes, unsigned long long* flags) {
    int dev = 0;
    (void)hipGetDevice(&dev);
    const unsigned long long bit = 1ull << (dev & 63);
    if (!(__atomic_load_n(flags, __ATOMIC_ACQUIRE) & bit)) {
        (void)hipFuncSetAttribute(kernel, hipFuncAttributeMaxDynamicSharedMemorySize, bytes);
        __atomic_fetch_or(flags, bit, __ATOMIC_RELEASE);
    }
}

inline int env_int(const char* name, int dflt) {
#ifdef SFA_AB
    const char* e = getenv(name);
    return e ? atoi(e) : dflt;
#else
    (void)name;
    return dflt;
#endif
}

inline int launch_status(const char* what) {
    hipError_t e = hipGetLastError();
    if (e != hipSuccess) {
        set_error("%s: launch failed: %s", what, hipGetErrorString(e));
        return (int)e;
    }
    return SFA_OK;
}

struct View {
    char* ptr;
    int64_t sb, sh, sn;
};

inline View make_view(const sfa_tensor* t) {
    return View{(char*)t->ptr, t->stride[0], t->stride[1], t->stride[2]};
}

struct Problem {
    int B, Hq, Hkv, N, D;
    int num_sink, window;
    float scale;
    const int* cu = nullptr;
    int n_total = 0;
    int Nk = 0;
};

#ifdef __HIPCC__
struct SeqInfo {
    int N;
    int row0;
    int bb;
};
__device__ __forceinline__ SeqInfo seq_of(const int* cu, int b, int N) {
    if (cu) {
        const int r0 = cu[b];
        return SeqInfo{cu[b + 1] - r0, r0, 0};
    }
    return SeqInfo{N, 0, b};
}
__device__ __forceinline__ unsigned seq_range(const int* cu, unsigned whole, int N, int64_t sn, int D) {
    return cu ? (unsigned)((((int64_t)N - 1) * sn + D) * 2) : whole;
}
#endif

inline int dtype_size(int dt) { return dt == SFA_DTYPE_F32 ? 4 : 2; }

inline int64_t cdiv64(int64_t a, int64_t b) { return (a + b - 1) / b; }

using bf16_t = __hip_bfloat16;
using f16_t = __half;

template <typename T> struct DT;
template <> struct DT<float> { static constexpr int id = SFA_DTYPE_F32; };
template <> struct DT<f16_t> { static constexpr int id = SFA_DTYPE_F16; };
template <> struct DT<bf16_t> { static constexpr int id = SFA_DTYPE_BF16; };

__device__ __forceinline__ float to_f32(float x) { return x; }
__device__ __forceinline__ float to_f32(f16_t x) { return __half2float(x); }
__device__ __forceinline__ float to_f32(bf16_t x) { return __bfloat162float(x); }

template <typename T> __device__ __forceinline__ T from_f32(float x);
template <> __device__ __forceinline__ float from_f32<float>(float x) { return x; }
template <> __device__ __forceinline__ f16_t from_f32<f16_t>(float x) { return __float2half_rn(x); }
template <> __device__ __forceinline__ bf16_t from_f32<bf16_t>(float x) { return __float2bfloat16(x); }

__device__ __forceinline__ float bf16_bits_to_f32(unsigned short b) { return __uint_as_float(((unsigned)b) << 16); }

template <typename T> __device__ __forceinline__ float raw16_to_f32(unsigned short b);
template <> __device__ __forceinline__ float raw16_to_f32<bf16_t>(unsigned short b) { return bf16_bits_to_f32(b); }
template <> __device__ __forceinline__ float raw16_to_f32<f16_t>(unsigned short b) {
    return __half2float(__ushort_as_half(b));
}

constexpr float kLog2e = 1.4426950408889634f;
constexpr float kLn2 = 0.6931471805599453f;

__device__ __forceinline__ float wave_sum(float x) {
#pragma unroll
    for (int o = 32; o > 0; o >>= 1) x += __shfl_xor(x, o, 64);
    return x;
}
__device__ __forceinline__ float wave_max(float x) {
#pragma unroll
    for (int o = 32; o > 0; o >>= 1) x = fmaxf(x, __shfl_xor(x, o, 64));
    return x;
}

}
```

### sink-flash-attention-kernel_amd/csrc/sfa_fwd_mfma.hip

```cpp
#include "sfa_common.hpp"
#include "sfa_internal.hpp"
#include "sfa_worklist.hpp"

#include <cstdlib>
#include <type_traits>

#include "gen/fwd_asm.inc"
#include "gen/fwd_strip_asm.inc"

namespace sfa {
namespace {

typedef __attribute__((ext_vector_type(8))) __bf16 bf16x8_t;
typedef __attribute__((ext_vector_type(8))) _Float16 f16x8_t;
typedef __attribute__((ext_vector_type(4))) short s16x4;
typedef __attribute__((ext_vector_type(8))) short s16x8;
typedef __attribute__((ext_vector_type(16))) float f32x16;
typedef __attribute__((ext_vector_type(4))) unsigned int u32x4;
typedef __attribute__((ext_vector_type(2))) unsigned int u32x2;

template <typename T> struct Mma;
template <> struct Mma<bf16_t> {
    using frag = bf16x8_t;
    using elem = __bf16;
    static __device__ __forceinline__ f32x16 run(frag a, frag b, f32x16 c) {
        return __builtin_amdgcn_mfma_f32_32x32x16_bf16(a, b, c, 0, 0, 0);
    }
};
template <> struct Mma<f16_t> {
    using frag = f16x8_t;
    using elem = _Float16;
    static __device__ __forceinline__ f32x16 run(frag a, frag b, f32x16 c) {
        return __builtin_amdgcn_mfma_f32_32x32x16_f16(a, b, c, 0, 0, 0);
    }
};

struct FwdArgs {
    View q, k, v, o;
    float* lse;
    const float* s_aux;
    int B, Hq, Hkv, N;
    int num_sink, window;
    float scale_log2;
    int hpw, rb;
    int n_qtiles, hgroups;
    unsigned q_range, k_range, v_range, o_range;
    int prio;
    const int* cu;
    int n_total;
    int Nk;
    int strip, n_strips;
    int ring, ts;
    char* dbg;
};

__device__ __forceinline__ void sync_lds() { asm volatile("s_waitcnt lgkmcnt(0)\n\ts_barrier" ::: "memory"); }

__device__ __forceinline__ float half_swap_max(float x) {
    auto r = __builtin_amdgcn_permlane32_swap(__float_as_uint(x), __float_as_uint(x), false, false);
    return fmaxf(__uint_as_float(r[0]), __uint_as_float(r[1]));
}
__device__ __forceinline__ float half_swap_sum(float x) {
    auto r = __builtin_amdgcn_permlane32_swap(__float_as_uint(x), __float_as_uint(x), false, false);
    return __uint_as_float(r[0]) + __uint_as_float(r[1]);
}

template <typename T, int D, int NW>
__global__ __launch_bounds__(NW * 64, D > 128 ? 1 : 2) void fwd_mfma_kernel(FwdArgs a) {
    using M = Mma<T>;
    using frag = typename M::frag;
    constexpr int DK = D / 16;
    constexpr int DVB = (D + 31) / 32;
    constexpr int CPR = D / 8;
    constexpr int ROWB = (D <= 64) ? 128 : (D <= 128 ? 256 : 512);
    constexpr int TILE_BYTES = 64 * ROWB;
    constexpr int NT = NW * 64;
    constexpr int NCH = 64 * CPR;
    constexpr int NLD = (NCH + NT - 1) / NT;
    extern __shared__ __attribute__((aligned(16))) char smem[];

    int bid = blockIdx.x;
    {
        const int nblk = gridDim.x, q8 = nblk >> 3, r8 = nblk & 7, xcd = bid & 7;
        bid = (xcd < r8 ? xcd * (q8 + 1) : r8 * (q8 + 1) + (xcd - r8) * q8) + (bid >> 3);
    }
    const int qt = a.n_qtiles - 1 - bid % a.n_qtiles;
    int rest = bid / a.n_qtiles;
    const int hg = rest % a.hgroups;
    rest /= a.hgroups;
    const int hk = rest % a.Hkv;
    const int b = rest / a.Hkv;

    const int tid = threadIdx.x, lane = tid & 63;
    const int wave = __builtin_amdgcn_readfirstlane(tid >> 6);
    const int r = lane & 31, h = lane >> 5;
    const int g = a.Hq / a.Hkv;
    const int hh = wave % a.hpw, rbi = wave / a.hpw;
    const int head = hk * g + hg * a.hpw + hh;
    const SeqInfo sq = seq_of(a.cu, b, a.N);
    const int N = sq.N, ns = a.num_sink;
    const int P = a.cu ? 0 : a.Nk - a.N;
    const int W = a.window < N + P ? a.window : N + P;
    const int BM = 32 * a.rb;
    const int q0 = qt * BM;
    if (q0 >= N) return;
    const int q1 = (q0 + BM < N) ? q0 + BM : N;
    const int qw0 = q0 + 32 * rbi;
    const int qw_hi = (qw0 + 31 < N - 1) ? qw0 + 31 : N - 1;
    const int qrow = qw0 + r;
    const bool wave_live = qw0 < N;
    const int pw0 = qw0 + P, pw_hi = qw_hi + P;

    const int ns_eff = ns < q1 + P ? ns : q1 + P;
    const int ts_hi = (ns_eff + 63) >> 6;
    int wlo = q0 + P - W + 1;
    if (wlo < 0) wlo = 0;
    int tw_lo = wlo >> 6;
    if (tw_lo < ts_hi) tw_lo = ts_hi;
    const int tw_hi = (q1 + P + 63) >> 6;
    if (tw_lo > tw_hi) tw_lo = tw_hi;
    const int nt = ts_hi + (tw_hi - tw_lo);

    const char* qb = a.q.ptr + ((int64_t)sq.bb * a.q.sb + (int64_t)head * a.q.sh + (int64_t)sq.row0 * a.q.sn) * 2;
    const char* kb = a.k.ptr + ((int64_t)sq.bb * a.k.sb + (int64_t)hk * a.k.sh + (int64_t)sq.row0 * a.k.sn) * 2;
    const char* vb = a.v.ptr + ((int64_t)sq.bb * a.v.sb + (int64_t)hk * a.v.sh + (int64_t)sq.row0 * a.v.sn) * 2;
    char* ob = a.o.ptr + ((int64_t)sq.bb * a.o.sb + (int64_t)head * a.o.sh + (int64_t)sq.row0 * a.o.sn) * 2;
    const __amdgpu_buffer_rsrc_t rq = __builtin_amdgcn_make_buffer_rsrc((void*)qb, 0, seq_range(a.cu, a.q_range, N, a.q.sn, D), 0x00020000);
    const __amdgpu_buffer_rsrc_t rk = __builtin_amdgcn_make_buffer_rsrc((void*)kb, 0, seq_range(a.cu, a.k_range, N, a.k.sn, D), 0x00020000);
    const __amdgpu_buffer_rsrc_t rv = __builtin_amdgcn_make_buffer_rsrc((void*)vb, 0, seq_range(a.cu, a.v_range, N, a.v.sn, D), 0x00020000);
    const __amdgpu_buffer_rsrc_t ro = __builtin_amdgcn_make_buffer_rsrc((void*)ob, 0, seq_range(a.cu, a.o_range, N, a.o.sn, D), 0x00020000);

    frag qf[DK];
#pragma unroll
    for (int ks = 0; ks < DK; ++ks) {
        const unsigned off = (unsigned)qrow * (unsigned)(a.q.sn * 2) + (unsigned)((2 * ks + h) * 16);
        qf[ks] = __builtin_bit_cast(frag, __builtin_amdgcn_raw_buffer_load_b128(rq, off, 0, 0));
    }

    u32x4 kst[NLD], vst[NLD];
    const unsigned ksn2 = (unsigned)(a.k.sn * 2), vsn2 = (unsigned)(a.v.sn * 2);
    auto issue_loads = [&](int t) {
#pragma unroll
        for (int i = 0; i < NLD; ++i) {
            const int c = tid + i * NT;
            const int key = c / CPR, ch = c % CPR;
            const bool in = (NCH % NT == 0) || (c < NCH);
            const unsigned row = (unsigned)(64 * t + key);
            const unsigned ko = in ? row * ksn2 + (unsigned)(ch * 16) : 0xFFFFFFF0u;
            const unsigned vo = in ? row * vsn2 + (unsigned)(ch * 16) : 0xFFFFFFF0u;
            kst[i] = __builtin_amdgcn_raw_buffer_load_b128(rk, ko, 0, 0);
            vst[i] = __builtin_amdgcn_raw_buffer_load_b128(rv, vo, 0, 0);
        }
    };
    auto write_lds = [&](int buf) {
        char* kl = smem + buf * 2 * TILE_BYTES;
        char* vl = kl + TILE_BYTES;
#pragma unroll
        for (int i = 0; i < NLD; ++i) {
            const int c = tid + i * NT;
            const int key = c / CPR, ch = c % CPR;
            const int ksw = (ROWB == 512) ? (key & 31) : (ROWB == 256) ? (key & 15) : ((key >> 1) & 7);
            const int vsw = (ROWB >= 256) ? ((key & 3) << 2) : (((key >> 1) & 1) << 2);
            if ((NCH % NT == 0) || (c < NCH)) {
                *reinterpret_cast<u32x4*>(kl + key * ROWB + ((ch ^ ksw) << 4)) = kst[i];
                *reinterpret_cast<u32x4*>(vl + key * ROWB + ((ch ^ vsw) << 4)) = vst[i];
            }
        }
    };
    auto tile_of = [&](int it) { return it < ts_hi ? it : tw_lo + (it - ts_hi); };

    const int ksw_l = (ROWB == 512) ? r : (ROWB == 256) ? (r & 15) : ((r >> 1) & 7);
    const int k_rowoff = r * ROWB;
    const int q4 = (lane & 15) >> 2, p4 = lane & 3, g1 = (lane >> 4) & 1;
    const int vsw_l = (ROWB >= 256) ? (q4 << 2) : (((q4 >> 1) & 1) << 2);
    const int v_rowoff = (4 * h + q4) * ROWB + (p4 & 1) * 8;
    const int v_chunk_lo = 2 * g1 + (p4 >> 1);

    float m = -INFINITY, l = 0.f;
    if (a.s_aux) {
        m = a.s_aux[head] * kLog2e;
        l = (h == 0) ? 1.f : 0.f;
    }
    f32x16 o[DVB];
#pragma unroll
    for (int db = 0; db < DVB; ++db)
#pragma unroll
        for (int i = 0; i < 16; ++i) o[db][i] = 0.f;
    const float c = a.scale_log2;
    if (NW == 8 && a.prio && wave >= 4) __builtin_amdgcn_s_setprio(1);

    if (nt > 0) {
        issue_loads(tile_of(0));
        write_lds(0);
    }
    __builtin_amdgcn_s_waitcnt(0x0F70);
    __syncthreads();

    for (int it = 0; it < nt; ++it) {
        const int buf = it & 1;
        if (it + 1 < nt) issue_loads(tile_of(it + 1));
        const int k0 = tile_of(it) * 64;
        const bool needed = wave_live && (k0 <= pw_hi) && (k0 < ns || k0 + 63 >= pw0 - W + 1);
        if (needed) {
            const bool full = (k0 + 63 <= pw0) && ((k0 + 63 < ns) || (k0 >= pw_hi - W + 1));
            const char* kl = smem + buf * 2 * TILE_BYTES;
            const char* vl = kl + TILE_BYTES;
// ... 388 lines not shown
#pragma unroll
                        for (int i = 0; i < 16; ++i) s[kh][i] = (32 * kh + (i & 3) + 8 * (i >> 2) > tt) ? s[kh][i] : -INFINITY;
                } else {
#pragma unroll
                    for (int kh = 0; kh < 2; ++kh)
#pragma unroll
                        for (int i = 0; i < 16; ++i) {
                            const int key = k0 + 32 * kh + (i & 3) + 8 * (i >> 2) + 4 * h;
                            const bool valid = (key <= qm) && (key < ns || key + W > qm);
                            s[kh][i] = valid ? s[kh][i] : -INFINITY;
                        }
                }
            }
            float mx = -INFINITY;
#pragma unroll
            for (int kh = 0; kh < 2; ++kh)
#pragma unroll
                for (int i = 0; i < 16; ++i) mx = fmaxf(mx, s[kh][i]);
            mx = half_swap_max(mx);
            const float m_cand = fmaxf(m, mx * c);
            const float m_new = (m_cand > m + 8.f || m == -INFINITY) ? m_cand : m;
            const float m_safe = (m_new == -INFINITY) ? 0.f : m_new;
            const float alpha = __builtin_amdgcn_exp2f(m - m_safe);
            float rs = 0.f;
#pragma unroll
            for (int kh = 0; kh < 2; ++kh)
                if (kh == 0 ? nh0 : nh1) {
#pragma unroll
                    for (int i = 0; i < 16; ++i) {
                        const float pv = __builtin_amdgcn_exp2f(fmaf(s[kh][i], c, -m_safe));
                        s[kh][i] = pv;
                        rs += pv;
                    }
                }
            l = fmaf(l, alpha, rs);
            m = m_new;
            if (!__all(alpha == 1.f)) {
#pragma unroll
                for (int db = 0; db < DVB; ++db)
#pragma unroll
                    for (int i = 0; i < 16; ++i) o[db][i] *= alpha;
            }
#pragma unroll
            for (int kh = 0; kh < 2; ++kh)
                if (kh == 0 ? nh0 : nh1) {
                    frag vt[2][DVB], pf8[2];
#pragma unroll
                    for (int st = 0; st < 2; ++st) {
#pragma unroll
                        for (int j = 0; j < 8; ++j) pf8[st][j] = (typename M::elem)s[kh][8 * st + j];
                        const char* vrow = vl + (32 * kh + 16 * st) * ROWB + v_rowoff;
#pragma unroll
                        for (int db = 0; db < DVB; ++db) {
                            const int ch = (4 * db + v_chunk_lo) ^ vsw_l;
                            const char* p1 = vrow + (ch << 4);
                            const s16x4 lo4 = __builtin_amdgcn_ds_read_tr16_b64_v4i16(
                                (s16x4 __attribute__((address_space(3)))*)(p1));
                            const s16x4 hi4 = __builtin_amdgcn_ds_read_tr16_b64_v4i16(
                                (s16x4 __attribute__((address_space(3)))*)(p1 + 8 * ROWB));
                            s16x8 vv;
                            vv[0] = lo4[0]; vv[1] = lo4[1]; vv[2] = lo4[2]; vv[3] = lo4[3];
                            vv[4] = hi4[0]; vv[5] = hi4[1]; vv[6] = hi4[2]; vv[7] = hi4[3];
                            vt[st][db] = __builtin_bit_cast(frag, vv);
                        }
                    }
                    __builtin_amdgcn_sched_barrier(0);
#pragma unroll
                    for (int st = 0; st < 2; ++st)
#pragma unroll
                        for (int db = 0; db < DVB; ++db) o[db] = M::run(vt[st][db], pf8[st], o[db]);
                }
        }

        STRIP_STAMP(2)
        float lt = half_swap_sum(l);
        if (lt == 0.f) lt = 1.f;
        const float inv = 1.f / lt;
        const unsigned orow = (unsigned)qrow * (unsigned)(a.o.sn * 2);
#pragma unroll
        for (int db = 0; db < DVB; ++db)
#pragma unroll
            for (int p2 = 0; p2 < 2; ++p2) {
                if (32 * db + 16 * p2 < D) {
                    typedef typename M::elem E;
                    typedef __attribute__((ext_vector_type(4))) E e4;
                    e4 pe, po;
#pragma unroll
                    for (int e = 0; e < 4; ++e) {
                        pe[e] = (E)(o[db][8 * p2 + e] * inv);
                        po[e] = (E)(o[db][8 * p2 + 4 + e] * inv);
                    }
                    const u32x2 ev = __builtin_bit_cast(u32x2, pe), od = __builtin_bit_cast(u32x2, po);
                    const auto s0 = __builtin_amdgcn_permlane32_swap(ev[0], od[0], false, false);
                    const auto s1 = __builtin_amdgcn_permlane32_swap(ev[1], od[1], false, false);
                    u32x4 w;
                    w[0] = s0[0]; w[1] = s1[0]; w[2] = s0[1]; w[3] = s1[1];
                    const int d = 32 * db + 16 * p2 + 8 * h;
                    const unsigned off = wave_live ? orow + (unsigned)(d * 2) : 0xFFFFFFF0u;
                    #ifndef SFA_STRIP_NOSTORE
                    __builtin_amdgcn_raw_buffer_store_b128(w, ro, off, 0, 0);
#else
                    if (w[0] == 0x12345678u) __builtin_amdgcn_raw_buffer_store_b128(w, ro, off, 0, 0);
#endif
                }
            }
        if (h == 0 && qrow < N) {
            const int64_t lrow = a.cu ? (int64_t)head * a.n_total + sq.row0 : ((int64_t)b * a.Hq + head) * N;
            a.lse[lrow + qrow] = (m + __log2f(lt)) * kLn2;
        }

        STRIP_STAMP(3)
        sync_lds();
        if (pf) {
            write_lds(next_load, kst, vst);
            ++next_load;
        }
        if (has_next) {
#pragma unroll
            for (int ks = 0; ks < DK; ++ks) qf[ks] = qn[ks];
        }
        STRIP_STAMP(4)
    }
#ifdef SFA_STRIP_STAMPS
    if (a.dbg && lane == 0) {
        unsigned long long* d = reinterpret_cast<unsigned long long*>(a.dbg) + ((size_t)blockIdx.x * NW + wave) * 8;
        for (int i = 0; i < 5; ++i) d[i] = tacc[i];
    }
#endif
#undef STRIP_STAMP
}

template <typename T, int D, int ALT>
__global__ __launch_bounds__(256) void fwd_asm_pk_kernel(FwdArgs a) {
    extern __shared__ __attribute__((aligned(16))) char smem[];
    const int G = (int)gridDim.x, w = (int)blockIdx.x;
    const unsigned tid = threadIdx.x;
    const int n_groups = a.hgroups * a.Hkv * a.B;
    const int64_t n_ranks = (int64_t)a.n_qtiles * n_groups;
    const int g = a.Hq / a.Hkv, BM = 64 * a.rb, ns = a.num_sink;
    auto u = [](unsigned x) { return (unsigned)__builtin_amdgcn_readfirstlane((int)x); };
#ifdef SFA_WL_STAMPS
    const unsigned wl_t0 = u((unsigned)__builtin_amdgcn_s_memrealtime());
    const unsigned wl_c0 = u((unsigned)__builtin_amdgcn_s_memtime());
#endif
    FwdPkScalars s;
    s.q_hs = u((unsigned)(a.q.sh * 2)); s.q_sn = u((unsigned)(a.q.sn * 2));
    s.o_hs = u((unsigned)(a.o.sh * 2)); s.o_sn = u((unsigned)(a.o.sn * 2));
    s.k_sn = u((unsigned)(a.k.sn * 2)); s.v_sn = u((unsigned)(a.v.sn * 2));
    s.ld_hs = u((unsigned)((a.cu ? a.n_total : a.N) * 4));
    s.l0 = u(__float_as_uint(a.s_aux ? 1.f : 0.f));
    s.pos0 = u((unsigned)(a.cu ? 0 : a.Nk - a.N)); s.W = u((unsigned)a.window); s.ns = u((unsigned)ns);
    s.hpw_log2 = u(a.hpw == 4 ? 2u : (a.hpw == 2 ? 1u : 0u));
    s.c_log2 = u(__float_as_uint(a.scale_log2)); s.ln2 = u(__float_as_uint(kLn2));
    {
        const int j = (int)tid;
        bool valid = false;
        unsigned d[SFA_WL_DESC_DWORDS];
#pragma unroll
        for (int i = 0; i < SFA_WL_DESC_DWORDS; ++i) d[i] = 0;
        const int64_t r = (int64_t)j * G < n_ranks ? wl_rank(j, w, G) : -1;
        if (r >= 0 && r < n_ranks) {
            const int qt = a.n_qtiles - 1 - (int)(r / n_groups);
            int rest = (int)(r % n_groups);
            const int hg = rest % a.hgroups;
            rest /= a.hgroups;
            const int hk = rest % a.Hkv;
            const int b = rest / a.Hkv;
            const SeqInfo sq = seq_of(a.cu, b, a.N);
            const int N = sq.N;
            const int P = a.cu ? 0 : a.Nk - a.N;
            const int Nk = N + P;
            const int W = a.window < Nk ? a.window : Nk;
            const int q0 = qt * BM;
            if (q0 < N) {
                valid = true;
                const int q1 = (q0 + BM < N) ? q0 + BM : N;
                const int ns_eff = ns < q1 + P ? ns : q1 + P;
                const int ts_hi = (ns_eff + 63) >> 6;
                int wlo = q0 + P - W + 1;
                if (wlo < 0) wlo = 0;
                int tw_lo = wlo >> 6;
                if (tw_lo < ts_hi) tw_lo = ts_hi;
                const int tw_hi = (q1 + P + 63) >> 6;
                if (tw_lo > tw_hi) tw_lo = tw_hi;
                const int head0 = hk * g + hg * a.hpw;
                const int64_t lrow = a.cu ? (int64_t)head0 * a.n_total + sq.row0 : ((int64_t)b * a.Hq + head0) * N;
                const uint64_t qb = (uint64_t)(a.q.ptr + ((int64_t)sq.bb * a.q.sb + (int64_t)head0 * a.q.sh + (int64_t)sq.row0 * a.q.sn) * 2);
                const uint64_t ob = (uint64_t)(a.o.ptr + ((int64_t)sq.bb * a.o.sb + (int64_t)head0 * a.o.sh + (int64_t)sq.row0 * a.o.sn) * 2);
                const uint64_t kbp = (uint64_t)(a.k.ptr + ((int64_t)sq.bb * a.k.sb + (int64_t)hk * a.k.sh + (int64_t)sq.row0 * a.k.sn) * 2);
                const uint64_t vbp = (uint64_t)(a.v.ptr + ((int64_t)sq.bb * a.v.sb + (int64_t)hk * a.v.sh + (int64_t)sq.row0 * a.v.sn) * 2);
                const uint64_t lb = (uint64_t)(a.lse + lrow);
                const unsigned ninf = 0xFF800000u;
                d[SFA_FWDPK_F_q_lo] = (unsigned)qb; d[SFA_FWDPK_F_q_hi] = (unsigned)(qb >> 32);
                d[SFA_FWDPK_F_o_lo] = (unsigned)ob; d[SFA_FWDPK_F_o_hi] = (unsigned)(ob >> 32);
                d[SFA_FWDPK_F_lse_lo] = (unsigned)lb; d[SFA_FWDPK_F_lse_hi] = (unsigned)(lb >> 32);
                d[SFA_FWDPK_F_q0] = (unsigned)q0; d[SFA_FWDPK_F_nrows] = (unsigned)N;
                d[SFA_FWDPK_F_q_rng] = seq_range(a.cu, a.q_range, N, a.q.sn, D);
                d[SFA_FWDPK_F_o_rng] = seq_range(a.cu, a.o_range, N, a.o.sn, D);
                d[SFA_FWDPK_F_m0_0] = a.s_aux ? __float_as_uint(a.s_aux[head0] * kLog2e) : ninf;
                d[SFA_FWDPK_F_m0_1] = a.s_aux && a.hpw > 1 ? __float_as_uint(a.s_aux[head0 + 1] * kLog2e) : ninf;
                d[SFA_FWDPK_F_m0_2] = a.s_aux && a.hpw > 2 ? __float_as_uint(a.s_aux[head0 + 2] * kLog2e) : ninf;
                d[SFA_FWDPK_F_m0_3] = a.s_aux && a.hpw > 3 ? __float_as_uint(a.s_aux[head0 + 3] * kLog2e) : ninf;
                d[SFA_FWDPK_F_k_lo] = (unsigned)kbp; d[SFA_FWDPK_F_k_hi] = (unsigned)(kbp >> 32);
                d[SFA_FWDPK_F_v_lo] = (unsigned)vbp; d[SFA_FWDPK_F_v_hi] = (unsigned)(vbp >> 32);
                d[SFA_FWDPK_F_k_rng] = seq_range(a.cu, a.k_range, Nk, a.k.sn, D);
                d[SFA_FWDPK_F_v_rng] = seq_range(a.cu, a.v_range, Nk, a.v.sn, D);
                d[SFA_FWDPK_F_nt] = (unsigned)(ts_hi + (tw_hi - tw_lo));
                d[SFA_FWDPK_F_ts_hi] = (unsigned)ts_hi; d[SFA_FWDPK_F_tw_off] = (unsigned)(tw_lo - ts_hi);
            }
        }
        int n_items = 0;
        const int idx = wl_compact(valid, reinterpret_cast<int*>(smem), &n_items);
        if (valid) {
            uint4* dst = reinterpret_cast<uint4*>(smem + SFA_FWDPK_DESC_BASE + idx * (SFA_WL_DESC_DWORDS * 4));
#pragma unroll
            for (int i = 0; i < SFA_WL_DESC_DWORDS / 4; ++i) dst[i] = make_uint4(d[4 * i], d[4 * i + 1], d[4 * i + 2], d[4 * i + 3]);
        }
        __syncthreads();
        s.n_items = u((unsigned)n_items);
        if (n_items > 0) {
#ifdef SFA_AB
            if constexpr (ALT == 1) asm volatile(SFA_FWDPK_ASM_BF16_ALT : : SFA_FWDPK_INPUTS(s), [tid] "v"(tid) : SFA_FWDPK_CLOBBERS);
#endif
#define SFA_FWDPK_BODY(DD)                                                                                      \
    if constexpr (D == DD && ALT == 0) {                                                                          \
        if constexpr (std::is_same<T, bf16_t>::value)                                                             \
            asm volatile(SFA_FWDPK_ASM_BF16_D##DD : : SFA_FWDPK_INPUTS(s), [tid] "v"(tid) : SFA_FWDPK_CLOBBERS);   \
        else                                                                                                      \
            asm volatile(SFA_FWDPK_ASM_F16_D##DD : : SFA_FWDPK_INPUTS(s), [tid] "v"(tid) : SFA_FWDPK_CLOBBERS);    \
    }
            SFA_FWDPK_BODY(64) SFA_FWDPK_BODY(80) SFA_FWDPK_BODY(96) SFA_FWDPK_BODY(128)
#undef SFA_FWDPK_BODY
        }
#ifdef SFA_WL_STAMPS
        if (a.dbg && threadIdx.x == 0) {
            unsigned* rec = reinterpret_cast<unsigned*>(a.dbg) + 4 * blockIdx.x;
            rec[0] = wl_t0;
            rec[1] = (unsigned)__builtin_amdgcn_s_memrealtime();
            rec[2] = (unsigned)__builtin_amdgcn_s_getreg(20 | (3 << 11));
            rec[3] = (s.n_items & 1023u) | ((((unsigned)__builtin_amdgcn_s_memtime() - wl_c0) >> 4) << 10);
        }
#endif
    }
}

template <typename T, int D>
int launch_asm(const FwdArgs& a0, const Problem& p, hipStream_t stream) {
    FwdArgs a = a0;
    const int g = p.Hq / p.Hkv;
    a.hpw = g % 4 == 0 ? 4 : (g % 2 == 0 ? 2 : 1);
    a.rb = 4 / a.hpw;
    a.n_qtiles = (int)cdiv64(p.N, 64 * a.rb);
    a.hgroups = g / a.hpw;
    const int64_t nblk = (int64_t)a.n_qtiles * a.hgroups * p.Hkv * p.B;
    if (nblk >= (1ll << 31)) {
        set_error("fwd_asm: grid too large");
        return SFA_ERR_UNSUPPORTED;
    }
    auto kpk = fwd_asm_pk_kernel<T, D, 0>;
    static unsigned long long done_pk = 0;
    ensure_dynamic_lds((const void*)kpk, SFA_FWDPK_LDS_BYTES, &done_pk);
#ifdef SFA_AB
    if (variant(1) == 1 && std::is_same<T, bf16_t>::value && D == 128) {
        kpk = fwd_asm_pk_kernel<T, D, 1>;
        static unsigned long long done_alt = 0;
        ensure_dynamic_lds((const void*)kpk, SFA_FWDPK_LDS_BYTES, &done_alt);
    }
#endif
    int dev = 0, n_cu = 256;
    if (hipGetDevice(&dev) != hipSuccess || hipDeviceGetAttribute(&n_cu, hipDeviceAttributeMultiprocessorCount, dev) != hipSuccess || n_cu <= 0) n_cu = 256;
    int64_t grid = nblk < n_cu ? nblk : n_cu;
    const int64_t need = cdiv64(nblk, SFA_WL_MAX_ITEMS);
    if (grid < need) grid = need;
    kpk<<<dim3((unsigned)grid), dim3(256), SFA_FWDPK_LDS_BYTES, stream>>>(a);
    set_path("fwd_mfma_%s_d%d_asm4x64pk_hpw%d", DT<T>::id == SFA_DTYPE_BF16 ? "bf16" : "f16", D, a.hpw);
    return launch_status("fwd_asm_pk");
}

template <typename T, int D, int NT>
__global__ __launch_bounds__(256) void fwd_strip_asm_kernel(FwdArgs a) {
    extern __shared__ __attribute__((aligned(16))) char smem[];
    int bid = blockIdx.x;
    {
        const int nblk = gridDim.x, q8 = nblk >> 3, r8 = nblk & 7, xcd = bid & 7;
        bid = (xcd < r8 ? xcd * (q8 + 1) : r8 * (q8 + 1) + (xcd - r8) * q8) + (bid >> 3);
    }
    const int sidx = bid % a.n_strips;
    int rest = bid / a.n_strips;
    const int hg = rest % a.hgroups;
    rest /= a.hgroups;
    const int hk = rest % a.Hkv;
    const int b = rest / a.Hkv;
    const SeqInfo sq = seq_of(a.cu, b, a.N);
    const int N = sq.N;
    const int q0 = sidx * a.strip * 64;
    if (q0 >= N) return;
    const int n_tiles = (N + 63) >> 6;
    int n_it = n_tiles - sidx * a.strip;
    if (n_it > a.strip) n_it = a.strip;
    const int g = a.Hq / a.Hkv;
    const int head0 = hk * g + hg * 4;
    const int64_t lrow = a.cu ? (int64_t)head0 * a.n_total + sq.row0 : ((int64_t)b * a.Hq + head0) * N;
    const uint64_t qb = (uint64_t)(a.q.ptr + ((int64_t)sq.bb * a.q.sb + (int64_t)head0 * a.q.sh + (int64_t)sq.row0 * a.q.sn) * 2);
    const uint64_t ob = (uint64_t)(a.o.ptr + ((int64_t)sq.bb * a.o.sb + (int64_t)head0 * a.o.sh + (int64_t)sq.row0 * a.o.sn) * 2);
    const uint64_t kbp = (uint64_t)(a.k.ptr + ((int64_t)sq.bb * a.k.sb + (int64_t)hk * a.k.sh + (int64_t)sq.row0 * a.k.sn) * 2);
    const uint64_t vbp = (uint64_t)(a.v.ptr + ((int64_t)sq.bb * a.v.sb + (int64_t)hk * a.v.sh + (int64_t)sq.row0 * a.v.sn) * 2);
    const uint64_t lb = (uint64_t)(a.lse + lrow);
    auto u = [](unsigned x) { return (unsigned)__builtin_amdgcn_readfirstlane((int)x); };
    FwdStripScalars s;
    s.q_lo = u((unsigned)qb); s.q_hi = u((unsigned)(qb >> 32)); s.q_hs = u((unsigned)(a.q.sh * 2));
    s.q_sn = u((unsigned)(a.q.sn * 2)); s.q_rng = u(seq_range(a.cu, a.q_range, N, a.q.sn, D));
    s.o_lo = u((unsigned)ob); s.o_hi = u((unsigned)(ob >> 32)); s.o_hs = u((unsigned)(a.o.sh * 2));
    s.o_sn = u((unsigned)(a.o.sn * 2)); s.o_rng = u(seq_range(a.cu, a.o_range, N, a.o.sn, D));
    s.k_lo = u((unsigned)kbp); s.k_hi = u((unsigned)(kbp >> 32)); s.k_sn = u((unsigned)(a.k.sn * 2));
    s.k_rng = u(seq_range(a.cu, a.k_range, N, a.k.sn, D));
    s.v_lo = u((unsigned)vbp); s.v_hi = u((unsigned)(vbp >> 32)); s.v_sn = u((unsigned)(a.v.sn * 2));
    s.v_rng = u(seq_range(a.cu, a.v_range, N, a.v.sn, D));
    s.lse_lo = u((unsigned)lb); s.lse_hi = u((unsigned)(lb >> 32));
    s.ld_hs = u((unsigned)((a.cu ? a.n_total : N) * 4));
    const unsigned ninf = 0xFF800000u;
    s.m0_0 = u(a.s_aux ? __float_as_uint(a.s_aux[head0] * kLog2e) : ninf);
    s.m0_1 = u(a.s_aux ? __float_as_uint(a.s_aux[head0 + 1] * kLog2e) : ninf);
    s.m0_2 = u(a.s_aux ? __float_as_uint(a.s_aux[head0 + 2] * kLog2e) : ninf);
    s.m0_3 = u(a.s_aux ? __float_as_uint(a.s_aux[head0 + 3] * kLog2e) : ninf);
    s.l0 = u(__float_as_uint(a.s_aux ? 1.f : 0.f));
    s.q0 = u((unsigned)q0); s.n_it = u((unsigned)n_it); s.nrows = u((unsigned)N);
    s.W = u((unsigned)(a.window < N ? a.window : N));
    s.c_log2 = u(__float_as_uint(a.scale_log2)); s.ln2 = u(__float_as_uint(kLn2));
    const unsigned tid = threadIdx.x;
    if (a.B < 0) smem[tid] = 0;
#define SFA_FSTRIP_BODY(DD, NN)                                                                                          \
    if constexpr (D == DD && NT == NN) {                                                                                   \
        if constexpr (std::is_same<T, bf16_t>::value)                                                                      \
            asm volatile(SFA_FSTRIP_ASM_BF16_D##DD##_NT##NN : : SFA_FSTRIP_INPUTS(s), [tid] "v"(tid) : SFA_FSTRIP_CLOBBERS); \
        else                                                                                                               \
            asm volatile(SFA_FSTRIP_ASM_F16_D##DD##_NT##NN : : SFA_FSTRIP_INPUTS(s), [tid] "v"(tid) : SFA_FSTRIP_CLOBBERS);  \
    }
    SFA_FSTRIP_BODY(64, 2) SFA_FSTRIP_BODY(64, 3) SFA_FSTRIP_BODY(64, 4)
    SFA_FSTRIP_BODY(80, 2) SFA_FSTRIP_BODY(80, 3) SFA_FSTRIP_BODY(80, 4)
    SFA_FSTRIP_BODY(96, 2) SFA_FSTRIP_BODY(96, 3) SFA_FSTRIP_BODY(96, 4)
#undef SFA_FSTRIP_BODY
}

template <typename T, int D, int NT>
int launch_strip_asm_nt(const FwdArgs& a0, const Problem& p, hipStream_t stream) {
    FwdArgs a = a0;
    const int g = p.Hq / p.Hkv;
    a.hpw = 4;
    a.rb = 1;
    a.hgroups = g / 4;
    a.n_qtiles = (int)cdiv64(p.N, 64);
    int dev = 0, n_cu = 256;
    if (hipGetDevice(&dev) != hipSuccess || hipDeviceGetAttribute(&n_cu, hipDeviceAttributeMultiprocessorCount, dev) != hipSuccess || n_cu <= 0) n_cu = 256;
    const int64_t groups = (int64_t)a.hgroups * p.Hkv * p.B;
    int64_t L = (int64_t)a.n_qtiles * groups / n_cu;
    if (L < 1) L = 1;
    if (L > a.n_qtiles) L = a.n_qtiles;
    a.strip = (int)L;
    a.n_strips = (int)cdiv64(a.n_qtiles, a.strip);
    const int64_t nblk = (int64_t)a.n_strips * groups;
    if (nblk >= (1ll << 31)) {
        set_error("fwd_strip_asm: grid too large");
        return SFA_ERR_UNSUPPORTED;
    }
    constexpr int lds = (NT + 1) * SFA_FSTRIP_SLOT_BYTES;
    auto kern = fwd_strip_asm_kernel<T, D, NT>;
    static unsigned long long done = 0;
    ensure_dynamic_lds((const void*)kern, lds, &done);
    kern<<<dim3((unsigned)nblk), dim3(256), lds, stream>>>(a);
    set_path("fwd_mfma_%s_d%d_stripasm_nt%d_len%d", DT<T>::id == SFA_DTYPE_BF16 ? "bf16" : "f16", D, NT, a.strip);
    return launch_status("fwd_strip_asm");
}

inline int strip_asm_nt(int W) {
    if (W < 1 || W > 193) return 0;
    const int nt = (W - 1 + 63) / 64 + 1;
    return nt < 2 ? 2 : nt;
}

template <typename T, int D>
int launch_strip_asm(const FwdArgs& a, const Problem& p, int nt, hipStream_t stream) {
    switch (nt) {
        case 2: return launch_strip_asm_nt<T, D, 2>(a, p, stream);
        case 3: return launch_strip_asm_nt<T, D, 3>(a, p, stream);
        default: return launch_strip_asm_nt<T, D, 4>(a, p, stream);
    }
}

int gcd(int x, int y);

template <typename T, int D>
int launch_strip(const FwdArgs& a0, const Problem& p, int ring, int ts, int lds, hipStream_t stream) {
    FwdArgs a = a0;
    constexpr int NW = 8;
    const int g = p.Hq / p.Hkv;
    a.hpw = gcd(g, NW);
    a.rb = NW / a.hpw;
    a.n_qtiles = (int)cdiv64(p.N, 32 * a.rb);
    a.hgroups = g / a.hpw;
    a.ring = ring;
    a.ts = ts;
    static const int n_cu = [] {
        int dev = 0, n = 256;
        if (hipGetDevice(&dev) != hipSuccess || hipDeviceGetAttribute(&n, hipDeviceAttributeMultiprocessorCount, dev) != hipSuccess) n = 256;
        return n > 0 ? n : 256;
    }();
    static const int min_strip = env_int("SFA_FWD_STRIP_MIN", 4);
    const int64_t base = (int64_t)a.hgroups * p.Hkv * p.B;
    int per_seq = (int)(base >= n_cu ? 1 : n_cu / base);
    a.strip = (int)cdiv64(a.n_qtiles, per_seq);
    if (a.strip < min_strip) a.strip = min_strip;
    if (a.strip > a.n_qtiles) a.strip = a.n_qtiles;
    a.n_strips = (int)cdiv64(a.n_qtiles, a.strip);
    const int64_t nblk = (int64_t)a.n_strips * base;
    if (nblk >= (1ll << 31)) {
        set_error("fwd_strip: grid too large");
        return SFA_ERR_UNSUPPORTED;
    }
    auto kern = fwd_strip_kernel<T, D, NW>;
    static unsigned long long done = 0;
    ensure_dynamic_lds((const void*)kern, 160 * 1024, &done);
    kern<<<dim3((unsigned)nblk), dim3(NW * 64), lds, stream>>>(a);
    set_path("fwd_mfma_%s_d%d_strip%d_ring%d_hpw%d", DT<T>::id == SFA_DTYPE_BF16 ? "bf16" : "f16", D, a.strip, ring, a.hpw);
    return launch_status("fwd_strip");
}

template <typename T, int D, int NW>
int launch(const FwdArgs& a, int nblk, hipStream_t stream) {
    constexpr int ROWB = (D <= 64) ? 128 : (D <= 128 ? 256 : 512);
    constexpr int lds = 2 * 2 * 64 * ROWB;
    auto kern = fwd_mfma_kernel<T, D, NW>;
    static unsigned long long attr_done = 0;
    ensure_dynamic_lds((const void*)kern, lds, &attr_done);
    kern<<<dim3(nblk), dim3(NW * 64), lds, stream>>>(a);
    set_path("fwd_mfma_%s_d%d_nw%d_hpw%d", sizeof(T) == 2 && DT<T>::id == SFA_DTYPE_BF16 ? "bf16" : "f16", D, NW,
             a.hpw);
    return launch_status("fwd_mfma");
}

template <typename T, int NW>
int launch_d(const FwdArgs& a, int D, int nblk, hipStream_t stream) {
    switch (D) {
        case 32: return launch<T, 32, NW>(a, nblk, stream);
        case 256:
            if (NW == 4) return launch<T, 256, 4>(a, nblk, stream);
            break;
        case 64: return launch<T, 64, NW>(a, nblk, stream);
        case 80: return launch<T, 80, NW>(a, nblk, stream);
        case 96: return launch<T, 96, NW>(a, nblk, stream);
        case 128: return launch<T, 128, NW>(a, nblk, stream);
    }
    set_error("fwd_mfma: unsupported head dim %d", D);
    return SFA_ERR_UNSUPPORTED;
}

int gcd(int x, int y) { return y == 0 ? x : gcd(y, x % y); }

unsigned slice_range(const sfa_tensor* t) {
    return (unsigned)(((t->shape[2] - 1) * t->stride[2] + t->shape[3]) * 2);
}
bool slice_ok(const sfa_tensor* t) {
    const int64_t reach = (t->shape[2] + 320) * t->stride[2] * 2 + 512;
    const bool head_ok = t->stride[1] >= 0 && t->stride[1] * 2 < (1ll << 32);
    return reach < (1ll << 32) - 65536 && head_ok && ((uintptr_t)t->ptr % 16) == 0 && (t->stride[0] * 2) % 16 == 0 &&
           (t->stride[1] * 2) % 16 == 0 && (t->stride[2] * 2) % 16 == 0;
}

}

bool fwd_mfma_supported(int dtype, int D) {
    return (dtype == SFA_DTYPE_BF16 || dtype == SFA_DTYPE_F16) &&
           (D == 32 || D == 64 || D == 80 || D == 96 || D == 128 || D == 256);
}

int fwd_mfma(const sfa_tensor* q, const sfa_tensor* k, const sfa_tensor* v, const sfa_tensor* o, float* lse,
             const float* s_aux, const Problem& p, hipStream_t stream) {
    if (!(slice_ok(q) && slice_ok(k) && slice_ok(v) && slice_ok(o))) {
        if (p.cu || (p.Nk > 0 && p.Nk != p.N)) {
            set_error("packed (varlen) / N_q != N_kv forward needs 16-byte aligned rows, < 4 GiB head slices and < 4 GiB head strides");
            return SFA_ERR_UNSUPPORTED;
        }
        return fwd_generic(q, k, v, o, lse, s_aux, p, stream);
    }
    int NW = (p.window >= 0 && p.window <= 2048) ? 4 : 8;
    static const int nw_knob = env_int("SFA_FWD_NW", 0);
    if (nw_knob == 4 || nw_knob == 8) NW = nw_knob;
    if (p.D == 256) NW = 4;
    const int g = p.Hq / p.Hkv;
    FwdArgs a;
    a.q = make_view(q); a.k = make_view(k); a.v = make_view(v); a.o = make_view(o);
    a.lse = lse; a.s_aux = s_aux;
    a.B = p.B; a.Hq = p.Hq; a.Hkv = p.Hkv; a.N = p.N;
    a.cu = p.cu; a.n_total = p.n_total;
    a.Nk = p.cu ? p.N : (p.Nk > 0 ? p.Nk : p.N);
    a.num_sink = p.num_sink;
    a.window = p.window < 0 ? 0 : (p.window > a.Nk ? a.Nk : p.window);
    a.scale_log2 = p.scale * kLog2e;
    a.hpw = gcd(g, NW);
    a.rb = NW / a.hpw;
    a.n_qtiles = (int)cdiv64(p.N, 32 * a.rb);
    a.hgroups = g / a.hpw;
    static const int prio_knob = env_int("SFA_FWD_PRIO", 1);
    a.prio = prio_knob;
    a.q_range = slice_range(q); a.k_range = slice_range(k); a.v_range = slice_range(v); a.o_range = slice_range(o);
    a.dbg = (char*)g_debug_ptr;
    static const int strip_knob = env_int("SFA_FWD_STRIP", 1);
    static const int strip_maxw = env_int("SFA_FWD_STRIP_MAXW", 256);
    static const int strip_asm_knob = env_int("SFA_FWD_STRIP_ASM", 1);
    if (strip_asm_knob == 1 && p.num_sink <= 0 && a.Nk == p.N && g % 4 == 0 && (p.D == 64 || p.D == 80 || p.D == 96) &&
        strip_asm_nt(p.window) > 0) {
        const int nt = strip_asm_nt(p.window);
        const bool bf = q->dtype == SFA_DTYPE_BF16;
        switch (p.D) {
            case 64: return bf ? launch_strip_asm<bf16_t, 64>(a, p, nt, stream) : launch_strip_asm<f16_t, 64>(a, p, nt, stream);
            case 80: return bf ? launch_strip_asm<bf16_t, 80>(a, p, nt, stream) : launch_strip_asm<f16_t, 80>(a, p, nt, stream);
            case 96: return bf ? launch_strip_asm<bf16_t, 96>(a, p, nt, stream) : launch_strip_asm<f16_t, 96>(a, p, nt, stream);
        }
    }
    if (strip_knob == 1 && p.window > 0 && p.window <= strip_maxw && p.D < 128) {
        const int hpw8 = gcd(g, 8), bm = 32 * (8 / hpw8);
        const int slot = 2 * 64 * (p.D <= 64 ? 128 : 256);
        const int ring = (a.window + bm - 1 + 63) / 64 + 1;
        const int nse = p.num_sink < a.Nk ? p.num_sink : a.Nk;
        const int ts = (nse + 63) / 64;
        const int lds = (ring + ts) * slot;
        if (lds <= 160 * 1024) {
            const bool bf = q->dtype == SFA_DTYPE_BF16;
            switch (p.D) {
                case 32: return bf ? launch_strip<bf16_t, 32>(a, p, ring, ts, lds, stream) : launch_strip<f16_t, 32>(a, p, ring, ts, lds, stream);
                case 64: return bf ? launch_strip<bf16_t, 64>(a, p, ring, ts, lds, stream) : launch_strip<f16_t, 64>(a, p, ring, ts, lds, stream);
                case 80: return bf ? launch_strip<bf16_t, 80>(a, p, ring, ts, lds, stream) : launch_strip<f16_t, 80>(a, p, ring, ts, lds, stream);
                case 96: return bf ? launch_strip<bf16_t, 96>(a, p, ring, ts, lds, stream) : launch_strip<f16_t, 96>(a, p, ring, ts, lds, stream);
                case 128: return bf ? launch_strip<bf16_t, 128>(a, p, ring, ts, lds, stream) : launch_strip<f16_t, 128>(a, p, ring, ts, lds, stream);
            }
        }
    }
    static const int fwd_asm_knob = env_int("SFA_FWD", 1);
    static const int asm_min_window = env_int("SFA_ASM_MIN_WINDOW", 256);
    if (fwd_asm_knob == 1 && (p.D == 128 || a.window > asm_min_window) && (a.window > 0 || p.num_sink > 0)) {
        const bool bf = q->dtype == SFA_DTYPE_BF16;
        switch (p.D) {
            case 64: return bf ? launch_asm<bf16_t, 64>(a, p, stream) : launch_asm<f16_t, 64>(a, p, stream);
            case 80: return bf ? launch_asm<bf16_t, 80>(a, p, stream) : launch_asm<f16_t, 80>(a, p, stream);
            case 96: return bf ? launch_asm<bf16_t, 96>(a, p, stream) : launch_asm<f16_t, 96>(a, p, stream);
            case 128: return bf ? launch_asm<bf16_t, 128>(a, p, stream) : launch_asm<f16_t, 128>(a, p, stream);
        }
    }
    const int64_t nblk = (int64_t)a.n_qtiles * a.hgroups * p.Hkv * p.B;
    if (nblk >= (1ll << 31)) {
        set_error("fwd_mfma: grid too large");
        return SFA_ERR_UNSUPPORTED;
    }
    if (q->dtype == SFA_DTYPE_BF16)
        return NW == 8 ? launch_d<bf16_t, 8>(a, p.D, (int)nblk, stream) : launch_d<bf16_t, 4>(a, p.D, (int)nblk, stream);
    return NW == 8 ? launch_d<f16_t, 8>(a, p.D, (int)nblk, stream) : launch_d<f16_t, 4>(a, p.D, (int)nblk, stream);
}

}
```

### sink-flash-attention-kernel_amd/csrc/sfa_internal.hpp

```cpp
#pragma once
#include "sfa_common.hpp"

namespace sfa {

int fwd_generic(const sfa_tensor* q, const sfa_tensor* k, const sfa_tensor* v, const sfa_tensor* o, float* lse,
                const float* s_aux, const Problem& p, hipStream_t stream);
int bwd_preprocess(const sfa_tensor* o, const sfa_tensor* d_o, const float* lse, const float* s_aux, float* delta,
                   float* dsaux_part, float* ds_aux, const Problem& p, hipStream_t stream, float* consts,
                   float lse_factor);
bool bwd_preprocess_vectorised(const sfa_tensor* o, const sfa_tensor* d_o, const Problem& p);
int64_t bwd_preprocess_nblk(int64_t N);
int bwd_generic(const sfa_tensor* q, const sfa_tensor* k, const sfa_tensor* v, const sfa_tensor* d_o,
                const float* lse, const float* delta, const sfa_tensor* dq, const sfa_tensor* dk,
                const sfa_tensor* dv, const Problem& p, hipStream_t stream);

bool fwd_mfma_supported(int dtype, int D);
int fwd_mfma(const sfa_tensor* q, const sfa_tensor* k, const sfa_tensor* v, const sfa_tensor* o, float* lse,
             const float* s_aux, const Problem& p, hipStream_t stream);

bool bwd_mfma_supported(int dtype, int D);
bool bwd_mfma_varlen_supported(int dtype, int D);
size_t bwd_mfma_workspace_bytes(const Problem& p, int dtype, unsigned flags);
int bwd_mfma(const sfa_tensor* q, const sfa_tensor* k, const sfa_tensor* v, const sfa_tensor* d_o,
             const float* lse, const float* delta, const sfa_tensor* dq, const sfa_tensor* dk,
             const sfa_tensor* dv, void* workspace, const Problem& p, unsigned flags, hipStream_t stream,
             bool consts_ready);
int bwd_mfma_refused(const sfa_tensor* q, const sfa_tensor* k, const sfa_tensor* v, const sfa_tensor* d_o,
                     const sfa_tensor* dq, const sfa_tensor* dk, const sfa_tensor* dv, const Problem& p);
bool bwd_mfma_wants_consts();
float bwd_mfma_lse_factor(const Problem& p, unsigned flags);

enum class RingState {
    Host,
    Shared,
    Rows,
};
struct RingCall {
    const sfa_tensor *q, *sink_k, *sink_v, *window_k, *window_v, *k_new, *v_new, *o;
    const float* s_aux;
    float scale;
    unsigned flags;
    hipStream_t stream;
    void* workspace;
    size_t workspace_bytes;
    int commit;
    RingState mode;
    int64_t sink_len, window_len, write_pos;
    int32_t* state;
    const int32_t* slots;
    const int32_t* parent;
    int64_t parent_bstride;
    const int32_t* path;
    int64_t path_bstride;
    const int32_t* count;
    const int32_t* cu_q;
    int n_seq;
};

struct DecodePlan {
    int splits;
    int keys_per_split;
    int lpk;
    int gt;
    int max_splits;
};
inline size_t decode_counter_bytes(int64_t B, int64_t Hkv) { return (((size_t)(B * Hkv + 1) * sizeof(int)) + 255) & ~(size_t)255; }
int decode_plan(int64_t B, int64_t Hq, int64_t Hkv, int64_t Nkv, int64_t D, int dtype, DecodePlan* plan);
int decode_launch(const RingCall& c, const DecodePlan& plan);

int decode_multi_check_head_dim(int64_t D, int dtype);
size_t decode_multi_workspace(int64_t B, int64_t Hq, int64_t Hkv, int64_t n_new, int64_t Nkv, int64_t D, int dtype);
int decode_multi_launch(const RingCall& c);

size_t decode_ragged_workspace(int64_t n_seq, int64_t Hq, int64_t Hkv, int64_t T, int64_t Nkv_cache, int64_t D, int dtype);
int decode_ragged_launch(const RingCall& c);

int ring_commit_dyn_launch(const RingCall& c);
int ring_fill_varlen_launch(const sfa_tensor* sink_k, const sfa_tensor* sink_v, const sfa_tensor* window_k,
                            const sfa_tensor* window_v, const sfa_tensor* k, const sfa_tensor* v, const int32_t* cu,
                            int n_seq, int32_t* state, hipStream_t stream, const int32_t* slots);

}
```

### sink-flash-attention-kernel_amd/csrc/sfa_worklist.hpp

```cpp
#pragma once
#include "sfa_common.hpp"

namespace sfa {

__device__ __forceinline__ int64_t wl_rank(int j, int w, int G) {
    int pos = w;
    if (j & 1) pos = (G & 7) == 0 ? ((G >> 3) - 1 - (w >> 3)) * 8 + (w & 7) : G - 1 - w;
    return (int64_t)j * G + pos;
}

__device__ __forceinline__ int wl_compact(bool valid, int* cnt, int* total) {
    const unsigned long long m = __ballot(valid);
    const int lane = threadIdx.x & 63, wv = threadIdx.x >> 6;
    __syncthreads();
    if (lane == 0) cnt[wv] = __popcll(m);
    __syncthreads();
    int base = 0, tot = 0;
#pragma unroll
    for (int i = 0; i < 4; ++i) {
        const int c = cnt[i];
        if (i < wv) base += c;
        tot += c;
    }
    *total = tot;
    return base + __popcll(m & ((1ull << lane) - 1ull));
}

__device__ __forceinline__ int wl_ticket(unsigned* heads, int n, int* scratch) {
    if (threadIdx.x == 0) {
        const int x = (int)__builtin_amdgcn_s_getreg(20 | (3 << 11)) & 7;
        const int q8 = n >> 3, r8 = n & 7;
        int got = -1;
        for (int k = 0; k < 8 && got < 0; ++k) {
            const int y = (x + k) & 7;
            const int cnt = q8 + (y < r8 ? 1 : 0);
            if (cnt == 0) continue;
            const unsigned t = atomicAdd(heads + 32 * y, 1u);
            if (t < (unsigned)cnt) got = (y < r8 ? y * (q8 + 1) : r8 * (q8 + 1) + (y - r8) * q8) + (int)t;
        }
        *scratch = got;
    }
    __syncthreads();
    const int r = *scratch;
    __syncthreads();
    return r;
}

}
```

### sink-flash-attention-kernel_amd/sink_attention/_native.py

```python
from __future__ import annotations

import ctypes
import os
import struct
import threading

import torch

_HERE = os.path.dirname(os.path.abspath(__file__))
LIB_PATH = os.environ.get("SFA_LIB_PATH") or os.path.join(_HERE, "libsfa.so")

SFA_DTYPE = {torch.float32: 0, torch.float16: 1, torch.bfloat16: 2}
FLAG_FORCE_GENERIC = 0x1
FLAG_DECODE_ONE_PASS = 0x4
FLAG_BWD_OVERLAP = 0x8
FLAG_BWD_DKDV_ASM = 0x10
FLAG_BWD_DKDV_WS = 0x20
ABI_VERSION = 2

_bwd_flags = FLAG_BWD_OVERLAP


def set_backward_options(overlap=None, dkdv=None):
    global _bwd_flags
    prev = (bool(_bwd_flags & FLAG_BWD_OVERLAP),
            "asm" if _bwd_flags & FLAG_BWD_DKDV_ASM else ("ws" if _bwd_flags & FLAG_BWD_DKDV_WS else None))
    f = _bwd_flags
    if overlap is not None:
        f = (f | FLAG_BWD_OVERLAP) if overlap else (f & ~FLAG_BWD_OVERLAP)
    if dkdv is not None or overlap is None:
        f &= ~(FLAG_BWD_DKDV_ASM | FLAG_BWD_DKDV_WS)
        if dkdv == "asm":
            f |= FLAG_BWD_DKDV_ASM
        elif dkdv == "ws":
            f |= FLAG_BWD_DKDV_WS
        elif dkdv not in (None, "rule"):
            raise ValueError("dkdv must be None, 'rule', 'asm' or 'ws'")
    _bwd_flags = f
    return prev


def bwd_flags(flags=0) -> int:
    return flags | _bwd_flags


class SfaTensor(ctypes.Structure):
    _fields_ = [
        ("ptr", ctypes.c_void_p),
        ("shape", ctypes.c_int64 * 4),
        ("stride", ctypes.c_int64 * 4),
        ("dtype", ctypes.c_int32),
        ("reserved", ctypes.c_int32),
    ]


_lib = None
_lock = threading.Lock()


def _bind(lib):
    P = ctypes.POINTER(SfaTensor)
    vp, i32, u32, f32, sz, i64 = (ctypes.c_void_p, ctypes.c_int, ctypes.c_uint, ctypes.c_float, ctypes.c_size_t,
                                   ctypes.c_int64)
    lib.sfa_abi_version.restype = i32
    lib.sfa_abi_version.argtypes = []
    lib.sfa_last_error.restype = ctypes.c_char_p
    lib.sfa_last_error.argtypes = []
    lib.sfa_last_path.restype = ctypes.c_char_p
    lib.sfa_last_path.argtypes = []
    lib.sfa_debug_set_ptr.restype = i32
    lib.sfa_debug_set_ptr.argtypes = [ctypes.c_void_p]
    lib.sfa_debug_set_variant.restype = i32
    lib.sfa_debug_set_variant.argtypes = [i32, i32]
    lib.sfa_debug_set_stage_events.restype = i32
    lib.sfa_debug_set_stage_events.argtypes = [ctypes.POINTER(ctypes.c_void_p), i32]
    lib.sfa_fwd.restype = i32
    lib.sfa_fwd.argtypes = [P, P, P, P, vp, vp, i32, i32, f32, u32, vp]
    lib.sfa_bwd_workspace_bytes.restype = sz
    lib.sfa_bwd_workspace_bytes.argtypes = [i64, i64, i64, i64, i64, i32, i32, i32, u32]
    lib.sfa_bwd.restype = i32
    lib.sfa_bwd.argtypes = [P, P, P, P, P, vp, vp, P, P, P, vp, vp, sz, i32, i32, f32, u32, vp]
    lib.sfa_varlen_supported.restype = i32
    lib.sfa_varlen_supported.argtypes = [i32, i64]
    lib.sfa_fwd_varlen.restype = i32
    lib.sfa_fwd_varlen.argtypes = [P, P, P, P, vp, vp, vp, i32, i32, i32, i32, f32, u32, vp]
    lib.sfa_bwd_varlen.restype = i32
    lib.sfa_bwd_varlen.argtypes = [P, P, P, P, P, vp, vp, P, P, P, vp, vp, i32, i32, vp, sz, i32, i32, f32, u32, vp]
    lib.sfa_decode_workspace_bytes.restype = sz
    lib.sfa_decode_workspace_bytes.argtypes = [i64, i64, i64, i64, i64, i32]
    lib.sfa_decode.restype = i32
    lib.sfa_decode.argtypes = [P, P, P, P, vp, vp, sz, f32, u32, vp]
    lib.sfa_decode_ring.restype = i32
    lib.sfa_decode_ring.argtypes = [P, P, P, i64, P, P, i64, P, vp, vp, sz, f32, u32, vp]
    lib.sfa_decode_ring_step.restype = i32
    lib.sfa_decode_ring_step.argtypes = [P, P, P, i64, P, P, i64, i64, P, P, P, vp, vp, sz, f32, u32, vp]
    lib.sfa_decode_ring_step_dyn.restype = i32
    lib.sfa_decode_ring_step_dyn.argtypes = [P, P, P, P, P, P, P, P, vp, vp, vp, sz, f32, u32, vp]
    lib.sfa_decode_multi_workspace_bytes.restype = sz
    lib.sfa_decode_multi_workspace_bytes.argtypes = [i64, i64, i64, i64, i64, i64, i32]
    lib.sfa_decode_ring_multi.restype = i32
    lib.sfa_decode_ring_multi.argtypes = [P, P, P, i64, P, P, i64, i64, P, P, P, vp, i32, vp, sz, f32, u32, vp]
    lib.sfa_decode_ring_multi_dyn.restype = i32
    lib.sfa_decode_ring_multi_dyn.argtypes = [P, P, P, P, P, P, P, P, vp, i32, vp, vp, sz, f32, u32, vp]
    lib.sfa_ring_commit_dyn.restype = i32
    lib.sfa_ring_commit_dyn.argtypes = [P, P, P, P, vp, vp, vp]
    lib.sfa_decode_ring_step_rows.restype = i32
    lib.sfa_decode_ring_step_rows.argtypes = [P, P, P, P, P, P, P, P, vp, vp, vp, sz, f32, u32, vp]
    lib.sfa_decode_ring_multi_rows.restype = i32
    lib.sfa_decode_ring_multi_rows.argtypes = [P, P, P, P, P, P, P, P, vp, i32, vp, vp, sz, f32, u32, vp]
    lib.sfa_ring_commit_rows.restype = i32
    lib.sfa_ring_commit_rows.argtypes = [P, P, P, P, vp, vp, vp]
    lib.sfa_decode_ring_tree.restype = i32
    lib.sfa_decode_ring_tree.argtypes = [P, P, P, i64, P, P, i64, i64, P, P, P, vp, vp, i64, vp, sz, f32, u32, vp]
    lib.sfa_decode_ring_tree_dyn.restype = i32
    lib.sfa_decode_ring_tree_dyn.argtypes = [P, P, P, P, P, P, P, P, vp, vp, i64, vp, vp, sz, f32, u32, vp]
    lib.sfa_decode_ring_tree_rows.restype = i32
    lib.sfa_decode_ring_tree_rows.argtypes = [P, P, P, P, P, P, P, P, vp, vp, i64, vp, vp, sz, f32, u32, vp]
    lib.sfa_ring_commit_path_dyn.restype = i32
    lib.sfa_ring_commit_path_dyn.argtypes = [P, P, P, P, vp, vp, i64, vp, vp]
    lib.sfa_ring_commit_path_rows.restype = i32
    lib.sfa_ring_commit_path_rows.argtypes = [P, P, P, P, vp, vp, i64, vp, vp]
    lib.sfa_ring_fill_varlen.restype = i32
    lib.sfa_ring_fill_varlen.argtypes = [P, P, P, P, P, P, vp, i32, vp, vp]
    lib.sfa_decode_ring_step_slots.restype = i32
    lib.sfa_decode_ring_step_slots.argtypes = [P, P, P, P, P, P, P, P, vp, vp, vp, vp, sz, f32, u32, vp]
    lib.sfa_decode_ring_multi_slots.restype = i32
    lib.sfa_decode_ring_multi_slots.argtypes = [P, P, P, P, P, P, P, P, vp, i32, vp, vp, vp, sz, f32, u32, vp]
    lib.sfa_decode_ring_tree_slots.restype = i32
    lib.sfa_decode_ring_tree_slots.argtypes = [P, P, P, P, P, P, P, P, vp, vp, i64, vp, vp, vp, sz, f32, u32, vp]
    lib.sfa_ring_commit_slots.restype = i32
    lib.sfa_ring_commit_slots.argtypes = [P, P, P, P, vp, vp, vp, vp]
    lib.sfa_ring_commit_path_slots.restype = i32
    lib.sfa_ring_commit_path_slots.argtypes = [P, P, P, P, vp, vp, i64, vp, vp, vp]
    lib.sfa_ring_fill_varlen_slots.restype = i32
    lib.sfa_ring_fill_varlen_slots.argtypes = [P, P, P, P, P, P, vp, i32, vp, vp, vp]
    lib.sfa_decode_ragged_workspace_bytes.restype = sz
    lib.sfa_decode_ragged_workspace_bytes.argtypes = [i64, i64, i64, i64, i64, i64, i32]
    lib.sfa_decode_ring_ragged_slots.restype = i32
    lib.sfa_decode_ring_ragged_slots.argtypes = [P, P, P, P, P, P, P, P, vp, i32, vp, vp, vp, i32, vp, sz, f32, u32, vp]


def lib():
    global _lib
    if _lib is None:
        with _lock:
            if _lib is None:
                if not os.path.exists(LIB_PATH):
                    raise RuntimeError(
                        f"sink_attention: {LIB_PATH} not found. The HIP extension is required (there is no "
                        "Python/CPU fallback). Build it with `make -C sink-flash-attention-kernel_amd`.")
                handle = ctypes.CDLL(LIB_PATH)
                _bind(handle)
                v = handle.sfa_abi_version()
                if v != ABI_VERSION:
                    raise RuntimeError(f"libsfa.so ABI version {v}, expected {ABI_VERSION}: rebuild the extension")
                _lib = handle
    return _lib


def last_path() -> str:
    return lib().sfa_last_path().decode()


_DESC = struct.Struct("P4q4qii")
assert _DESC.size == ctypes.sizeof(SfaTensor)


def desc(t: torch.Tensor) -> SfaTensor:
    return SfaTensor.from_buffer_copy(_DESC.pack(t.data_ptr(), *t.shape, *t.stride(), SFA_DTYPE[t.dtype], 0))


def check(status: int, what: str):
    if status != 0:
        msg = lib().sfa_last_error().decode()
        kind = "argument/support error" if status < 0 else "HIP error"
        raise RuntimeError(f"{what} failed ({kind} {status}): {msg}")


def require_gpu(*tensors):
    for t in tensors:
        if t is not None and not t.is_cuda:
            raise RuntimeError(
                "sink_attention runs only on MI355X (HIP) tensors; got a CPU tensor and there is no CPU fallback")


def unit_inner(t: torch.Tensor) -> torch.Tensor:
    if t.stride(-1) != 1 and t.shape[-1] > 1:
        return t.contiguous()
    return t


def stream_ptr(device) -> int:
    return torch.cuda.current_stream(device).cuda_stream
```

### sink-flash-attention-kernel_amd/sink_attention/sink_flash_attention.py

```python
import math
import os

import torch

from . import _native as N


class SinkFlashAttentionFunc(torch.autograd.Function):
    @staticmethod
    def forward(ctx, q, k, v, num_sink, window_size, s_aux=None, out_bnhd=False, flags=0):
        N.require_gpu(q, k, v, s_aux)
        B, H_q, Nq, D = q.shape
        H_kv = k.shape[1]
        Nk = k.shape[2]
        assert k.shape == (B, H_kv, Nk, D) and Nk >= Nq, f"k {tuple(k.shape)} does not fit q {tuple(q.shape)}"
        assert v.shape == (B, H_kv, Nk, D)
        assert H_q % H_kv == 0
        if q.dtype not in N.SFA_DTYPE or k.dtype != q.dtype or v.dtype != q.dtype:
            raise TypeError(f"q/k/v must share one dtype in (float32, float16, bfloat16); got "
                            f"{q.dtype}, {k.dtype}, {v.dtype}")
        use_s_aux = s_aux is not None
        s_aux_f = None
        if use_s_aux:
            assert s_aux.shape == (H_q,), f"s_aux shape must be [H_q={H_q}], got {s_aux.shape}"
            s_aux_f = s_aux.detach().contiguous().float()
        num_sink, window_size = int(num_sink), int(window_size)
        scale = 1.0 / math.sqrt(D) if D > 0 else 1.0

        q, k, v = N.unit_inner(q), N.unit_inner(k), N.unit_inner(v)
        if out_bnhd:
            o = torch.empty((B, Nq, H_q, D), device=q.device, dtype=q.dtype).transpose(1, 2)
        else:
            o = torch.empty((B, H_q, Nq, D), device=q.device, dtype=q.dtype)
        lse = torch.empty((B, H_q, Nq), device=q.device, dtype=torch.float32)
        lib = N.lib()
        with torch.cuda.device(q.device):
            st = lib.sfa_fwd(N.desc(q), N.desc(k), N.desc(v), N.desc(o), lse.data_ptr(),
                             s_aux_f.data_ptr() if use_s_aux else None, num_sink, window_size, scale, flags,
                             N.stream_ptr(q.device))
        N.check(st, "sfa_fwd")

        ctx.save_for_backward(q, k, v, o, lse, s_aux_f if use_s_aux else torch.empty(0, device=q.device))
        ctx.num_sink, ctx.window_size, ctx.scale = num_sink, window_size, scale
        ctx.use_s_aux, ctx.flags = use_s_aux, flags
        ctx.s_aux_dtype = s_aux.dtype if use_s_aux else None
        return o

    @staticmethod
    @torch.autograd.function.once_differentiable
    def backward(ctx, do):
        q, k, v, o, lse, s_aux_f = ctx.saved_tensors
        B, H_q, Nq, D = q.shape
        H_kv = k.shape[1]
        do = N.unit_inner(do)
        if do.dtype != q.dtype:
            do = do.to(q.dtype)
        dq = torch.empty((B, H_q, Nq, D), device=q.device, dtype=q.dtype)
        mk = torch.zeros if (Nq == 0 or B == 0 or H_q == 0) else torch.empty
        dk = mk((B, H_kv, k.shape[2], D), device=q.device, dtype=q.dtype)
        dv = mk((B, H_kv, k.shape[2], D), device=q.device, dtype=q.dtype)
        ds_aux = mk((H_q,), device=q.device, dtype=torch.float32) if ctx.use_s_aux else None
        lib = N.lib()
        flags = N.bwd_flags(ctx.flags)
        ws_bytes = lib.sfa_bwd_workspace_bytes(B, H_q, H_kv, Nq, D, N.SFA_DTYPE[q.dtype], ctx.num_sink,
                                               ctx.window_size, flags)
        ws = torch.empty((max(int(ws_bytes), 256),), device=q.device, dtype=torch.uint8)
        with torch.cuda.device(q.device):
            st = lib.sfa_bwd(N.desc(q), N.desc(k), N.desc(v), N.desc(o), N.desc(do), lse.data_ptr(),
                             s_aux_f.data_ptr() if ctx.use_s_aux else None, N.desc(dq), N.desc(dk), N.desc(dv),
                             ds_aux.data_ptr() if ctx.use_s_aux else None, ws.data_ptr(), ws.numel(),
                             ctx.num_sink, ctx.window_size, ctx.scale, flags, N.stream_ptr(q.device))
        N.check(st, "sfa_bwd")
        if ctx.use_s_aux and ds_aux.dtype != ctx.s_aux_dtype:
            ds_aux = ds_aux.to(ctx.s_aux_dtype)
        return dq, dk, dv, None, None, ds_aux, None, None


def sink_flash_attention(q, k, v, num_sink=4, window_size=512, s_aux=None):
    return SinkFlashAttentionFunc.apply(q, k, v, num_sink, window_size, s_aux)


def _sink_flash_attention_ex(q, k, v, num_sink, window_size, s_aux=None, out_bnhd=False, force_generic=False):
    return SinkFlashAttentionFunc.apply(q, k, v, num_sink, window_size, s_aux, out_bnhd,
                                        N.FLAG_FORCE_GENERIC if force_generic else 0)
```

### sink-flash-attention-kernel_amd/sink_attention/varlen.py

```python
import math
import os
from typing import List, Sequence, Union

import torch

from . import _native as N
from .sink_flash_attention import _sink_flash_attention_ex


_CHECK_CU = os.environ.get("SINK_ATTENTION_CHECK_CU", "0") == "1"


def seq_bounds_from_position_ids(position_ids: torch.Tensor) -> List[int]:
    pid = position_ids.reshape(-1)
    starts = (pid == 0).nonzero(as_tuple=False).flatten().tolist()
    if not starts or starts[0] != 0:
        starts = [0] + starts
    return starts + [pid.numel()]


class SinkFlashAttentionVarlenFunc(torch.autograd.Function):

    @staticmethod
    def forward(ctx, q, k, v, cu_dev, max_seqlen, num_sink, window_size, s_aux, checked=True):
        _, H_q, T, D = q.shape
        alloc = torch.empty if checked else torch.zeros
        use_s_aux = s_aux is not None
        s_aux_f = s_aux.detach().contiguous().float() if use_s_aux else None
        scale = 1.0 / math.sqrt(D)
        q, k, v = N.unit_inner(q), N.unit_inner(k), N.unit_inner(v)
        o = alloc((1, H_q, T, D), device=q.device, dtype=q.dtype)
        lse = alloc((H_q, T), device=q.device, dtype=torch.float32)
        lib = N.lib()
        with torch.cuda.device(q.device):
            st = lib.sfa_fwd_varlen(N.desc(q), N.desc(k), N.desc(v), N.desc(o), lse.data_ptr(),
                                    s_aux_f.data_ptr() if use_s_aux else None, cu_dev.data_ptr(), cu_dev.numel() - 1,
                                    max_seqlen, num_sink, window_size, scale, 0, N.stream_ptr(q.device))
        N.check(st, "sfa_fwd_varlen")
        ctx.save_for_backward(q, k, v, o, lse, cu_dev, s_aux_f if use_s_aux else torch.empty(0, device=q.device))
        ctx.cfg = (max_seqlen, num_sink, window_size, scale, use_s_aux, s_aux.dtype if use_s_aux else None, checked)
        return o

    @staticmethod
    @torch.autograd.function.once_differentiable
    def backward(ctx, do):
        q, k, v, o, lse, cu_dev, s_aux_f = ctx.saved_tensors
        max_seqlen, num_sink, window_size, scale, use_s_aux, s_aux_dtype, checked = ctx.cfg
        alloc = torch.empty if checked else torch.zeros
        _, H_q, T, D = q.shape
        H_kv = k.shape[1]
        do = N.unit_inner(do)
        if do.dtype != q.dtype:
            do = do.to(q.dtype)
        dq = alloc((1, H_q, T, D), device=q.device, dtype=q.dtype)
        dk = alloc((1, H_kv, T, D), device=q.device, dtype=q.dtype)
        dv = alloc((1, H_kv, T, D), device=q.device, dtype=q.dtype)
        ds_aux = torch.empty((H_q,), device=q.device, dtype=torch.float32) if use_s_aux else None
        lib = N.lib()
        flags = N.bwd_flags()
        ws_bytes = lib.sfa_bwd_workspace_bytes(1, H_q, H_kv, T, D, N.SFA_DTYPE[q.dtype], num_sink, window_size, flags)
        ws = torch.empty((max(int(ws_bytes), 256),), device=q.device, dtype=torch.uint8)
        with torch.cuda.device(q.device):
            st = lib.sfa_bwd_varlen(N.desc(q), N.desc(k), N.desc(v), N.desc(o), N.desc(do), lse.data_ptr(),
                                    s_aux_f.data_ptr() if use_s_aux else None, N.desc(dq), N.desc(dk), N.desc(dv),
                                    ds_aux.data_ptr() if use_s_aux else None, cu_dev.data_ptr(), cu_dev.numel() - 1,
                                    max_seqlen, ws.data_ptr(), ws.numel(), num_sink, window_size, scale, flags,
                                    N.stream_ptr(q.device))
        N.check(st, "sfa_bwd_varlen")
        if use_s_aux and ds_aux.dtype != s_aux_dtype:
            ds_aux = ds_aux.to(s_aux_dtype)
        return dq, dk, dv, None, None, None, None, ds_aux, None


def _aligned(t: torch.Tensor) -> bool:
    es = t.element_size()
    return (t.data_ptr() % 16 == 0 and all((t.stride(i) * es) % 16 == 0 for i in range(3))
            and (t.shape[2] + 64) * t.stride(2) * es + 512 < (1 << 32) - 65536)


def sink_flash_attention_varlen(q: torch.Tensor, k: torch.Tensor, v: torch.Tensor,
                                cu_seqlens: Union[torch.Tensor, Sequence[int]], num_sink: int = 4,
                                window_size: int = 512, s_aux: torch.Tensor = None,
                                max_seqlen: int = None) -> torch.Tensor:
    N.require_gpu(q, k, v, s_aux)
    assert q.shape[0] == 1 and k.shape[0] == 1 and v.shape[0] == 1, "packed layout: batch dim must be 1"
    T = q.shape[2]
    native = (q.dtype in (torch.float16, torch.bfloat16) and k.dtype == q.dtype and v.dtype == q.dtype
              and N.lib().sfa_varlen_supported(N.SFA_DTYPE[q.dtype], q.shape[3]) == 1)
    if native:
        qq, kk, vv = N.unit_inner(q), N.unit_inner(k), N.unit_inner(v)
        native = _aligned(qq) and _aligned(kk) and _aligned(vv)
    if native:
        checked = True
        if isinstance(cu_seqlens, torch.Tensor) and cu_seqlens.is_cuda and max_seqlen is not None:
            cu_dev = cu_seqlens.to(torch.int32).contiguous()
            checked = False
            if _CHECK_CU:
                cu = cu_dev.tolist()
                assert len(cu) >= 2 and cu[0] == 0 and cu[-1] <= T, f"bad cu_seqlens {cu} for T={T}"
                assert all(b >= a for a, b in zip(cu[:-1], cu[1:])), f"cu_seqlens must be non-decreasing: {cu}"
                assert max_seqlen >= max(b - a for a, b in zip(cu[:-1], cu[1:])), "max_seqlen understates the longest sequence"
                checked = cu[-1] == T
        else:
            cu = cu_seqlens.tolist() if isinstance(cu_seqlens, torch.Tensor) else list(cu_seqlens)
            assert len(cu) >= 2 and cu[0] == 0 and cu[-1] == T, f"bad cu_seqlens {cu} for T={T}"
            assert all(b >= a for a, b in zip(cu[:-1], cu[1:])), f"cu_seqlens must be non-decreasing: {cu}"
            max_seqlen = max(b - a for a, b in zip(cu[:-1], cu[1:]))
            cu_dev = torch.tensor(cu, dtype=torch.int32, device=q.device)
        if T == 0 or max_seqlen == 0:
            return torch.empty_like(q)
        return SinkFlashAttentionVarlenFunc.apply(q, k, v, cu_dev, int(min(max_seqlen, T)), int(num_sink),
                                                  int(window_size), s_aux, checked)

    cu = cu_seqlens.tolist() if isinstance(cu_seqlens, torch.Tensor) else list(cu_seqlens)
    assert len(cu) >= 2 and cu[0] == 0 and cu[-1] == T, f"bad cu_seqlens {cu} for T={T}"
    outs = []
    for a, b in zip(cu[:-1], cu[1:]):
        assert b >= a
        if b == a:
            continue
        outs.append(_sink_flash_attention_ex(q[:, :, a:b], k[:, :, a:b], v[:, :, a:b], num_sink, window_size,
                                             s_aux=s_aux))
    return torch.cat(outs, dim=2) if len(outs) != 1 else outs[0]
```

Baseline: 981.4.

## Add dynamic tail work-stealing to forward persistent kernel via workspace counter

The forward persistent MFMA kernel now assigns work statically only up to the last couple of rounds, then has blocks claim the remaining work items one at a time through an atomic counter kept in a new forward workspace. This targets tail imbalance, where some CUs finish early while others still hold leftover items. The Python wrapper allocates the workspace, and a tiny kernel zeroes the counter before each launch. In exchange there is an extra kernel launch, a torch allocation per call, and per-item barrier and atomic overhead in the tail.

```diff
diff --git a/include/sfa.h b/include/sfa.h
--- a/include/sfa.h
+++ b/include/sfa.h
@@ -47,6 +47,13 @@
             float* lse, const float* s_aux, int num_sink, int window, float scale,
             unsigned flags, void* stream);
 
+size_t sfa_fwd_workspace_bytes(int64_t B, int64_t Hq, int64_t Hkv, int64_t N, int64_t D, int dtype,
+                               int num_sink, int window, unsigned flags);
+
+int sfa_fwd_ws(const sfa_tensor* q, const sfa_tensor* k, const sfa_tensor* v, const sfa_tensor* o,
+               float* lse, const float* s_aux, int num_sink, int window, float scale,
+               unsigned flags, void* workspace, size_t workspace_bytes, void* stream);
+
 size_t sfa_bwd_workspace_bytes(int64_t B, int64_t Hq, int64_t Hkv, int64_t N, int64_t D, int dtype,
                                int num_sink, int window, unsigned flags);
 
@@ -62,6 +69,13 @@
                    const float* s_aux, const int32_t* cu_seqlens, int n_seq, int max_seqlen, int num_sink,
                    int window, float scale, unsigned flags, void* stream);
 
+size_t sfa_fwd_varlen_workspace_bytes(int64_t Hq, int64_t Hkv, int64_t D, int dtype, int n_seq, int max_seqlen,
+                                      int num_sink, int window, unsigned flags);
+
+int sfa_fwd_varlen_ws(const sfa_tensor* q, const sfa_tensor* k, const sfa_tensor* v, const sfa_tensor* o, float* lse,
+                      const float* s_aux, const int32_t* cu_seqlens, int n_seq, int max_seqlen, int num_sink,
+                      int window, float scale, unsigned flags, void* workspace, size_t workspace_bytes, void* stream);
+
 int sfa_bwd_varlen(const sfa_tensor* q, const sfa_tensor* k, const sfa_tensor* v, const sfa_tensor* o,
                    const sfa_tensor* d_o, const float* lse, const float* s_aux, const sfa_tensor* dq,
                    const sfa_tensor* dk, const sfa_tensor* dv, float* ds_aux, const int32_t* cu_seqlens, int n_seq,
diff --git a/sink-flash-attention-kernel_amd/csrc/sfa_api.hip b/sink-flash-attention-kernel_amd/csrc/sfa_api.hip
--- a/sink-flash-attention-kernel_amd/csrc/sfa_api.hip
+++ b/sink-flash-attention-kernel_amd/csrc/sfa_api.hip
@@ -11,7 +11,7 @@
 static char g_path[128] = "";
 
 void* g_debug_ptr = nullptr;
-int g_variant[8] = {0, 0, 0, 0, 0, 0, 0, 0};
+int g_variant[16] = {0};
 static void* const* g_stage_events = nullptr;
 static int g_stage_count = 0;
 bool stage_events_armed() { return g_stage_events != nullptr; }
@@ -114,7 +114,7 @@
 const char* sfa_last_error(void) { return g_err; }
 const char* sfa_last_path(void) { return g_path; }
 int sfa_debug_set_variant(int which, int value) {
-    if (which < 0 || which >= 8) return SFA_ERR_INVALID_ARGUMENT;
+    if (which < 0 || which >= 16) return SFA_ERR_INVALID_ARGUMENT;
     __atomic_store_n(&sfa::g_variant[which], value, __ATOMIC_RELAXED);
     return SFA_OK;
 }
@@ -130,8 +130,9 @@
     return SFA_OK;
 }
 
-int sfa_fwd(const sfa_tensor* q, const sfa_tensor* k, const sfa_tensor* v, const sfa_tensor* o, float* lse,
-            const float* s_aux, int num_sink, int window, float scale, unsigned flags, void* stream) {
+static int fwd_entry(const sfa_tensor* q, const sfa_tensor* k, const sfa_tensor* v, const sfa_tensor* o, float* lse,
+                     const float* s_aux, int num_sink, int window, float scale, unsigned flags, void* workspace,
+                     size_t workspace_bytes, void* stream) {
     g_err[0] = 0;
     Problem p;
     int st = check_prefill(q, k, v, &p, num_sink, window, scale);
@@ -142,12 +143,32 @@
     SFA_CHECK_ARG(lse != nullptr, "lse: null pointer");
     hipStream_t s = (hipStream_t)stream;
     if (!(flags & SFA_FLAG_FORCE_GENERIC) && fwd_mfma_supported(q->dtype, p.D))
-        return fwd_mfma(q, k, v, o, lse, s_aux, p, s);
+        return fwd_mfma(q, k, v, o, lse, s_aux, p, workspace, workspace_bytes, s);
     if (p.Nk != p.N) {
         set_error("N_q != N_kv is served by the MFMA kernels only (16-bit dtypes, head dims 64/80/96/128)");
         return SFA_ERR_UNSUPPORTED;
     }
     return fwd_generic(q, k, v, o, lse, s_aux, p, s);
+}
+
+int sfa_fwd(const sfa_tensor* q, const sfa_tensor* k, const sfa_tensor* v, const sfa_tensor* o, float* lse,
+            const float* s_aux, int num_sink, int window, float scale, unsigned flags, void* stream) {
+    return fwd_entry(q, k, v, o, lse, s_aux, num_sink, window, scale, flags, nullptr, 0, stream);
+}
+
+size_t sfa_fwd_workspace_bytes(int64_t B, int64_t Hq, int64_t Hkv, int64_t N, int64_t D, int dtype, int num_sink,
+                               int window, unsigned flags) {
+    if ((flags & SFA_FLAG_FORCE_GENERIC) || B <= 0 || Hq <= 0 || Hkv <= 0 || N <= 0 || D <= 0 || N >= (1ll << 30) ||
+        B * Hq >= (1ll << 30))
+        return 0;
+    Problem p{(int)B, (int)Hq, (int)Hkv, (int)N, (int)D, num_sink, window, 1.f};
+    return fwd_mfma_workspace_bytes(p, dtype);
+}
+
+int sfa_fwd_ws(const sfa_tensor* q, const sfa_tensor* k, const sfa_tensor* v, const sfa_tensor* o, float* lse,
+               const float* s_aux, int num_sink, int window, float scale, unsigned flags, void* workspace,
+               size_t workspace_bytes, void* stream) {
+    return fwd_entry(q, k, v, o, lse, s_aux, num_sink, window, scale, flags, workspace, workspace_bytes, stream);
 }
 
 size_t sfa_bwd_workspace_bytes(int64_t B, int64_t Hq, int64_t Hkv, int64_t N, int64_t D, int dtype, int num_sink,
@@ -227,9 +248,10 @@
     return SFA_OK;
 }
 
-int sfa_fwd_varlen(const sfa_tensor* q, const sfa_tensor* k, const sfa_tensor* v, const sfa_tensor* o, float* lse,
-                   const float* s_aux, const int32_t* cu_seqlens, int n_seq, int max_seqlen, int num_sink, int window,
-                   float scale, unsigned flags, void* stream) {
+static int fwd_varlen_entry(const sfa_tensor* q, const sfa_tensor* k, const sfa_tensor* v, const sfa_tensor* o, float* lse,
+                            const float* s_aux, const int32_t* cu_seqlens, int n_seq, int max_seqlen, int num_sink,
+                            int window, float scale, unsigned flags, void* workspace, size_t workspace_bytes,
+                            void* stream) {
     g_err[0] = 0;
     (void)flags;
     Problem p, run;
@@ -238,7 +260,30 @@
     if ((st = check_tensor(o, "o")) || (st = same_shape(q, o, "q", "o"))) return st;
     if (p.Hq == 0 || p.N == 0) return SFA_OK;
     SFA_CHECK_ARG(lse != nullptr, "lse: null pointer");
-    return fwd_mfma(q, k, v, o, lse, s_aux, run, (hipStream_t)stream);
+    return fwd_mfma(q, k, v, o, lse, s_aux, run, workspace, workspace_bytes, (hipStream_t)stream);
+}
+
+int sfa_fwd_varlen(const sfa_tensor* q, const sfa_tensor* k, const sfa_tensor* v, const sfa_tensor* o, float* lse,
+                   const float* s_aux, const int32_t* cu_seqlens, int n_seq, int max_seqlen, int num_sink, int window,
+                   float scale, unsigned flags, void* stream) {
+    return fwd_varlen_entry(q, k, v, o, lse, s_aux, cu_seqlens, n_seq, max_seqlen, num_sink, window, scale, flags,
+                            nullptr, 0, stream);
+}
+
+size_t sfa_fwd_varlen_workspace_bytes(int64_t Hq, int64_t Hkv, int64_t D, int dtype, int n_seq, int max_seqlen,
+                                      int num_sink, int window, unsigned flags) {
+    (void)flags;
+    if (Hq <= 0 || Hkv <= 0 || D <= 0 || n_seq <= 0 || max_seqlen <= 0 || (int64_t)n_seq * Hq >= (1ll << 30)) return 0;
+    if (!sfa_varlen_supported(dtype, D)) return 0;
+    Problem p{n_seq, (int)Hq, (int)Hkv, max_seqlen, (int)D, num_sink, window, 1.f};
+    return fwd_mfma_workspace_bytes(p, dtype);
+}
+
+int sfa_fwd_varlen_ws(const sfa_tensor* q, const sfa_tensor* k, const sfa_tensor* v, const sfa_tensor* o, float* lse,
+                      const float* s_aux, const int32_t* cu_seqlens, int n_seq, int max_seqlen, int num_sink,
+                      int window, float scale, unsigned flags, void* workspace, size_t workspace_bytes, void* stream) {
+    return fwd_varlen_entry(q, k, v, o, lse, s_aux, cu_seqlens, n_seq, max_seqlen, num_sink, window, scale, flags,
+                            workspace, workspace_bytes, stream);
 }
 
 int sfa_bwd_varlen(const sfa_tensor* q, const sfa_tensor* k, const sfa_tensor* v, const sfa_tensor* o,
diff --git a/sink-flash-attention-kernel_amd/csrc/sfa_bwd_mfma.hip b/sink-flash-attention-kernel_amd/csrc/sfa_bwd_mfma.hip
--- a/sink-flash-attention-kernel_amd/csrc/sfa_bwd_mfma.hip
+++ b/sink-flash-attention-kernel_amd/csrc/sfa_bwd_mfma.hip
@@ -945,10 +945,7 @@
         for (int i = 0; i < SFA_WL_DESC_DWORDS; ++i) d[i] = 0;
         int64_t r_dyn = -1;
         if (!first) {
-            __syncthreads();
-            if (tid == 0) reinterpret_cast<volatile int*>(smem)[8] = (int)atomicAdd(a.tickets + kDynTicketDword, 1u);
-            __syncthreads();
-            r_dyn = n_static + reinterpret_cast<volatile int*>(smem)[8];
+            r_dyn = n_static + wl_claim(a.tickets + kDynTicketDword, reinterpret_cast<int*>(smem) + 8);
             if (r_dyn >= n_ranks) break;
         }
         {
@@ -1816,7 +1813,8 @@
             a4.n_base = a4.n_kblocks * a.Hkv * B;
             const int surplus = ((a4.n_base / 8 + 7) / 8) * 8;
             grid += surplus;
-            (void)hipMemsetAsync(a4.tickets, 0, 1024, stream);
+            const int st = memset_status(hipMemsetAsync(a4.tickets, 0, 1024, stream), "bwd_dkdv_asm tickets");
+            if (st) return st;
         }
 #ifdef SFA_AB
         if (variant(0) == 1 && std::is_same<T, bf16_t>::value && D == 128) {
@@ -1898,11 +1896,12 @@
         {
             static const int dyn_knob = env_int("SFA_WL_DYN", 1);
             const int64_t rounds = cdiv64(nblk, Gd);
-            if (dyn_knob == 1 && variant(5) == 0 && Gd == device_cu_count() && rounds >= 12 && a.tickets != nullptr) {
+            if (dyn_knob == 1 && variant(5) == 0 && Gd == device_cu_count() && rounds >= kWlDynMinRounds && a.tickets != nullptr) {
                 int64_t tail = 2;
                 if (variant(6) > 0) tail = variant(6);
-                a4.wl_dyn = (rounds - tail) * Gd;
-                (void)hipMemsetAsync(a.tickets + kDynTicketDword, 0, 128, dqs);
+                a4.wl_dyn = wl_tail_start(rounds, tail, Gd);
+                const int st = memset_status(hipMemsetAsync(a.tickets + kDynTicketDword, 0, 128, dqs), "bwd_dq_asm_pk counter");
+                if (st) return st;
             }
         }
         kpk<<<dim3((unsigned)Gd), dim3(256), SFA_DQPK_LDS_BYTES, dqs>>>(a4);
diff --git a/sink-flash-attention-kernel_amd/csrc/sfa_common.hpp b/sink-flash-attention-kernel_amd/csrc/sfa_common.hpp
--- a/sink-flash-attention-kernel_amd/csrc/sfa_common.hpp
+++ b/sink-flash-attention-kernel_amd/csrc/sfa_common.hpp
@@ -18,7 +18,7 @@
 void record_stage(int i, hipStream_t stream);
 bool stage_events_armed();
 extern void* g_debug_ptr;
-extern int g_variant[8];
+extern int g_variant[16];
 #ifdef SFA_AB
 inline int variant(int which) { return __atomic_load_n(&g_variant[which], __ATOMIC_RELAXED); }
 #else
@@ -57,6 +57,14 @@
     hipError_t e = hipGetLastError();
     if (e != hipSuccess) {
         set_error("%s: launch failed: %s", what, hipGetErrorString(e));
+        return (int)e;
+    }
+    return SFA_OK;
+}
+
+inline int memset_status(hipError_t e, const char* what) {
+    if (e != hipSuccess) {
+        set_error("%s: hipMemsetAsync failed: %s", what, hipGetErrorString(e));
         return (int)e;
     }
     return SFA_OK;
diff --git a/sink-flash-attention-kernel_amd/csrc/sfa_fwd_mfma.hip b/sink-flash-attention-kernel_amd/csrc/sfa_fwd_mfma.hip
--- a/sink-flash-attention-kernel_amd/csrc/sfa_fwd_mfma.hip
+++ b/sink-flash-attention-kernel_amd/csrc/sfa_fwd_mfma.hip
@@ -52,6 +52,8 @@
     int strip, n_strips;
     int ring, ts;
     char* dbg;
+    unsigned* wl_counter;
+    int64_t wl_dyn;
 };
 
 __device__ __forceinline__ void sync_lds() { asm volatile("s_waitcnt lgkmcnt(0)\n\ts_barrier" ::: "memory"); }
@@ -746,13 +748,23 @@
     s.pos0 = u((unsigned)(a.cu ? 0 : a.Nk - a.N)); s.W = u((unsigned)a.window); s.ns = u((unsigned)ns);
     s.hpw_log2 = u(a.hpw == 4 ? 2u : (a.hpw == 2 ? 1u : 0u));
     s.c_log2 = u(__float_as_uint(a.scale_log2)); s.ln2 = u(__float_as_uint(kLn2));
-    {
+    const int64_t n_static = a.wl_dyn > 0 && a.wl_dyn < n_ranks ? a.wl_dyn : n_ranks;
+    int n_done = 0;
+    for (bool first = true;; first = false) {
         const int j = (int)tid;
         bool valid = false;
         unsigned d[SFA_WL_DESC_DWORDS];
 #pragma unroll
         for (int i = 0; i < SFA_WL_DESC_DWORDS; ++i) d[i] = 0;
-        const int64_t r = (int64_t)j * G < n_ranks ? wl_rank(j, w, G) : -1;
+        int64_t r = -1;
+        if (first) {
+            if ((int64_t)j * G < n_static) r = wl_rank(j, w, G);
+            if (r >= n_static) r = -1;
+        } else {
+            const int64_t r_dyn = n_static + wl_claim(a.wl_counter, reinterpret_cast<int*>(smem) + 8);
+            if (r_dyn >= n_ranks) break;
+            if (j == 0) r = r_dyn;
+        }
         if (r >= 0 && r < n_ranks) {
             const int qt = a.n_qtiles - 1 - (int)(r / n_groups);
             int rest = (int)(r % n_groups);
@@ -812,6 +824,7 @@
         }
         __syncthreads();
         s.n_items = u((unsigned)n_items);
+        n_done += n_items;
         if (n_items > 0) {
 #ifdef SFA_AB
             if constexpr (ALT == 1) asm volatile(SFA_FWDPK_ASM_BF16_ALT : : SFA_FWDPK_INPUTS(s), [tid] "v"(tid) : SFA_FWDPK_CLOBBERS);
@@ -826,20 +839,44 @@
             SFA_FWDPK_BODY(64) SFA_FWDPK_BODY(80) SFA_FWDPK_BODY(96) SFA_FWDPK_BODY(128)
 #undef SFA_FWDPK_BODY
         }
+        if (n_static >= n_ranks) break;
+    }
 #ifdef SFA_WL_STAMPS
-        if (a.dbg && threadIdx.x == 0) {
-            unsigned* rec = reinterpret_cast<unsigned*>(a.dbg) + 4 * blockIdx.x;
-            rec[0] = wl_t0;
-            rec[1] = (unsigned)__builtin_amdgcn_s_memrealtime();
-            rec[2] = (unsigned)__builtin_amdgcn_s_getreg(20 | (3 << 11));
-            rec[3] = (s.n_items & 1023u) | ((((unsigned)__builtin_amdgcn_s_memtime() - wl_c0) >> 4) << 10);
-        }
+    if (a.dbg && threadIdx.x == 0) {
+        unsigned* rec = reinterpret_cast<unsigned*>(a.dbg) + 4 * blockIdx.x;
+        rec[0] = wl_t0;
+        rec[1] = (unsigned)__builtin_amdgcn_s_memrealtime();
+        rec[2] = (unsigned)__builtin_amdgcn_s_getreg(20 | (3 << 11));
+        rec[3] = ((unsigned)n_done & 1023u) | ((((unsigned)__builtin_amdgcn_s_memtime() - wl_c0) >> 4) << 10);
+    }
 #endif
-    }
+    (void)n_done;
+}
+
+int cu_count() {
+    int dev = 0, n_cu = 256;
+    if (hipGetDevice(&dev) != hipSuccess || hipDeviceGetAttribute(&n_cu, hipDeviceAttributeMultiprocessorCount, dev) != hipSuccess || n_cu <= 0) n_cu = 256;
+    return n_cu;
+}
+
+int64_t worklist_items(const Problem& p) {
+    const int g = p.Hq / p.Hkv;
+    const int hpw = g % 4 == 0 ? 4 : (g % 2 == 0 ? 2 : 1);
+    return cdiv64(p.N, 64 * (4 / hpw)) * (g / hpw) * p.Hkv * p.B;
+}
+
+constexpr int kFwdTailRounds = 2;
+constexpr size_t kFwdWsBytes = 256;
+bool worklist_tail_shape(int64_t nblk, int n_cu) {
+    return nblk >= (int64_t)kWlDynMinRounds * n_cu - (n_cu - 1) && cdiv64(nblk, SFA_WL_MAX_ITEMS) <= n_cu;
+}
+
+__global__ void wl_zero_kernel(unsigned* counter) {
+    if (threadIdx.x == 0) *counter = 0u;
 }
 
 template <typename T, int D>
-int launch_asm(const FwdArgs& a0, const Problem& p, hipStream_t stream) {
+int launch_asm(const FwdArgs& a0, const Problem& p, void* ws, size_t ws_bytes, hipStream_t stream) {
     FwdArgs a = a0;
     const int g = p.Hq / p.Hkv;
     a.hpw = g % 4 == 0 ? 4 : (g % 2 == 0 ? 2 : 1);
@@ -861,13 +898,33 @@
         ensure_dynamic_lds((const void*)kpk, SFA_FWDPK_LDS_BYTES, &done_alt);
     }
 #endif
-    int dev = 0, n_cu = 256;
-    if (hipGetDevice(&dev) != hipSuccess || hipDeviceGetAttribute(&n_cu, hipDeviceAttributeMultiprocessorCount, dev) != hipSuccess || n_cu <= 0) n_cu = 256;
+    const int n_cu = cu_count();
     int64_t grid = nblk < n_cu ? nblk : n_cu;
     const int64_t need = cdiv64(nblk, SFA_WL_MAX_ITEMS);
     if (grid < need) grid = need;
+    a.wl_dyn = 0;
+    a.wl_counter = nullptr;
+    int tail = 0;
+    {
+        static const int dyn_knob = env_int("SFA_FWD_DYN", 1);
+        const int64_t rounds = cdiv64(nblk, grid);
+        if (dyn_knob == 1 && variant(4) == 0 && ws != nullptr && ws_bytes >= kFwdWsBytes && ((uintptr_t)ws & 3) == 0 && grid == n_cu &&
+            rounds >= kWlDynMinRounds) {
+            tail = variant(8) > 0 ? variant(8) : kFwdTailRounds;
+            a.wl_dyn = wl_tail_start(rounds, tail, grid);
+            if (a.wl_dyn > 0) {
+                a.wl_counter = reinterpret_cast<unsigned*>(ws);
+                wl_zero_kernel<<<dim3(1), dim3(64), 0, stream>>>(a.wl_counter);
+                const int st = launch_status("fwd_asm_pk counter");
+                if (st) return st;
+            } else
+                tail = 0;
+        }
+    }
     kpk<<<dim3((unsigned)grid), dim3(256), SFA_FWDPK_LDS_BYTES, stream>>>(a);
-    set_path("fwd_mfma_%s_d%d_asm4x64pk_hpw%d", DT<T>::id == SFA_DTYPE_BF16 ? "bf16" : "f16", D, a.hpw);
+    char dyn_name[16] = "";
+    if (tail > 0) snprintf(dyn_name, sizeof dyn_name, "_dyn%d", tail);
+    set_path("fwd_mfma_%s_d%d_asm4x64pk_hpw%d%s", DT<T>::id == SFA_DTYPE_BF16 ? "bf16" : "f16", D, a.hpw, dyn_name);
     return launch_status("fwd_asm_pk");
 }
 
@@ -1067,8 +1124,17 @@
            (D == 32 || D == 64 || D == 80 || D == 96 || D == 128 || D == 256);
 }
 
+size_t fwd_mfma_workspace_bytes(const Problem& p, int dtype) {
+    if (!(dtype == SFA_DTYPE_BF16 || dtype == SFA_DTYPE_F16)) return 0;
+    if (!(p.D == 64 || p.D == 80 || p.D == 96 || p.D == 128) || p.Hkv <= 0 || p.Hq % p.Hkv != 0 || p.N <= 0) return 0;
+    const int Nk = p.cu ? p.N : (p.Nk > 0 ? p.Nk : p.N);
+    const int window = p.window < 0 ? 0 : (p.window > Nk ? Nk : p.window);
+    if (!(p.D == 128 || window > 256) || !(window > 0 || p.num_sink > 0)) return 0;
+    return worklist_tail_shape(worklist_items(p), cu_count()) ? kFwdWsBytes : 0;
+}
+
 int fwd_mfma(const sfa_tensor* q, const sfa_tensor* k, const sfa_tensor* v, const sfa_tensor* o, float* lse,
-             const float* s_aux, const Problem& p, hipStream_t stream) {
+             const float* s_aux, const Problem& p, void* ws, size_t ws_bytes, hipStream_t stream) {
     if (!(slice_ok(q) && slice_ok(k) && slice_ok(v) && slice_ok(o))) {
         if (p.cu || (p.Nk > 0 && p.Nk != p.N)) {
             set_error("packed (varlen) / N_q != N_kv forward needs 16-byte aligned rows, < 4 GiB head slices and < 4 GiB head strides");
@@ -1098,6 +1164,8 @@
     a.prio = prio_knob;
     a.q_range = slice_range(q); a.k_range = slice_range(k); a.v_range = slice_range(v); a.o_range = slice_range(o);
     a.dbg = (char*)g_debug_ptr;
+    a.wl_counter = nullptr;
+    a.wl_dyn = 0;
     static const int strip_knob = env_int("SFA_FWD_STRIP", 1);
     static const int strip_maxw = env_int("SFA_FWD_STRIP_MAXW", 256);
     static const int strip_asm_knob = env_int("SFA_FWD_STRIP_ASM", 1);
@@ -1134,10 +1202,10 @@
     if (fwd_asm_knob == 1 && (p.D == 128 || a.window > asm_min_window) && (a.window > 0 || p.num_sink > 0)) {
         const bool bf = q->dtype == SFA_DTYPE_BF16;
         switch (p.D) {
-            case 64: return bf ? launch_asm<bf16_t, 64>(a, p, stream) : launch_asm<f16_t, 64>(a, p, stream);
-            case 80: return bf ? launch_asm<bf16_t, 80>(a, p, stream) : launch_asm<f16_t, 80>(a, p, stream);
-            case 96: return bf ? launch_asm<bf16_t, 96>(a, p, stream) : launch_asm<f16_t, 96>(a, p, stream);
-            case 128: return bf ? launch_asm<bf16_t, 128>(a, p, stream) : launch_asm<f16_t, 128>(a, p, stream);
+            case 64: return bf ? launch_asm<bf16_t, 64>(a, p, ws, ws_bytes, stream) : launch_asm<f16_t, 64>(a, p, ws, ws_bytes, stream);
+            case 80: return bf ? launch_asm<bf16_t, 80>(a, p, ws, ws_bytes, stream) : launch_asm<f16_t, 80>(a, p, ws, ws_bytes, stream);
+            case 96: return bf ? launch_asm<bf16_t, 96>(a, p, ws, ws_bytes, stream) : launch_asm<f16_t, 96>(a, p, ws, ws_bytes, stream);
+            case 128: return bf ? launch_asm<bf16_t, 128>(a, p, ws, ws_bytes, stream) : launch_asm<f16_t, 128>(a, p, ws, ws_bytes, stream);
         }
     }
     const int64_t nblk = (int64_t)a.n_qtiles * a.hgroups * p.Hkv * p.B;
diff --git a/sink-flash-attention-kernel_amd/csrc/sfa_internal.hpp b/sink-flash-attention-kernel_amd/csrc/sfa_internal.hpp
--- a/sink-flash-attention-kernel_amd/csrc/sfa_internal.hpp
+++ b/sink-flash-attention-kernel_amd/csrc/sfa_internal.hpp
@@ -15,8 +15,9 @@
                 const sfa_tensor* dv, const Problem& p, hipStream_t stream);
 
 bool fwd_mfma_supported(int dtype, int D);
+size_t fwd_mfma_workspace_bytes(const Problem& p, int dtype);
 int fwd_mfma(const sfa_tensor* q, const sfa_tensor* k, const sfa_tensor* v, const sfa_tensor* o, float* lse,
-             const float* s_aux, const Problem& p, hipStream_t stream);
+             const float* s_aux, const Problem& p, void* ws, size_t ws_bytes, hipStream_t stream);
 
 bool bwd_mfma_supported(int dtype, int D);
 bool bwd_mfma_varlen_supported(int dtype, int D);
diff --git a/sink-flash-attention-kernel_amd/csrc/sfa_worklist.hpp b/sink-flash-attention-kernel_amd/csrc/sfa_worklist.hpp
--- a/sink-flash-attention-kernel_amd/csrc/sfa_worklist.hpp
+++ b/sink-flash-attention-kernel_amd/csrc/sfa_worklist.hpp
@@ -26,6 +26,19 @@
     return base + __popcll(m & ((1ull << lane) - 1ull));
 }
 
+__device__ __forceinline__ int wl_claim(unsigned* counter, int* scratch) {
+    __syncthreads();
+    if (threadIdx.x == 0) *reinterpret_cast<volatile int*>(scratch) = (int)atomicAdd(counter, 1u);
+    __syncthreads();
+    return *reinterpret_cast<volatile int*>(scratch);
+}
+
+inline int64_t wl_tail_start(int64_t rounds, int64_t tail, int64_t G) {
+    if (tail > rounds - 1) tail = rounds - 1;
+    return tail > 0 ? (rounds - tail) * G : 0;
+}
+constexpr int kWlDynMinRounds = 12;
+
 __device__ __forceinline__ int wl_ticket(unsigned* heads, int n, int* scratch) {
     if (threadIdx.x == 0) {
         const int x = (int)__builtin_amdgcn_s_getreg(20 | (3 << 11)) & 7;
diff --git a/sink-flash-attention-kernel_amd/sink_attention/_native.py b/sink-flash-attention-kernel_amd/sink_attention/_native.py
--- a/sink-flash-attention-kernel_amd/sink_attention/_native.py
+++ b/sink-flash-attention-kernel_amd/sink_attention/_native.py
@@ -76,6 +76,10 @@
     lib.sfa_debug_set_stage_events.argtypes = [ctypes.POINTER(ctypes.c_void_p), i32]
     lib.sfa_fwd.restype = i32
     lib.sfa_fwd.argtypes = [P, P, P, P, vp, vp, i32, i32, f32, u32, vp]
+    lib.sfa_fwd_workspace_bytes.restype = sz
+    lib.sfa_fwd_workspace_bytes.argtypes = [i64, i64, i64, i64, i64, i32, i32, i32, u32]
+    lib.sfa_fwd_ws.restype = i32
+    lib.sfa_fwd_ws.argtypes = [P, P, P, P, vp, vp, i32, i32, f32, u32, vp, sz, vp]
     lib.sfa_bwd_workspace_bytes.restype = sz
     lib.sfa_bwd_workspace_bytes.argtypes = [i64, i64, i64, i64, i64, i32, i32, i32, u32]
     lib.sfa_bwd.restype = i32
@@ -84,6 +88,10 @@
     lib.sfa_varlen_supported.argtypes = [i32, i64]
     lib.sfa_fwd_varlen.restype = i32
     lib.sfa_fwd_varlen.argtypes = [P, P, P, P, vp, vp, vp, i32, i32, i32, i32, f32, u32, vp]
+    lib.sfa_fwd_varlen_workspace_bytes.restype = sz
+    lib.sfa_fwd_varlen_workspace_bytes.argtypes = [i64, i64, i64, i32, i32, i32, i32, i32, u32]
+    lib.sfa_fwd_varlen_ws.restype = i32
+    lib.sfa_fwd_varlen_ws.argtypes = [P, P, P, P, vp, vp, vp, i32, i32, i32, i32, f32, u32, vp, sz, vp]
     lib.sfa_bwd_varlen.restype = i32
     lib.sfa_bwd_varlen.argtypes = [P, P, P, P, P, vp, vp, P, P, P, vp, vp, i32, i32, vp, sz, i32, i32, f32, u32, vp]
     lib.sfa_decode_workspace_bytes.restype = sz
diff --git a/sink-flash-attention-kernel_amd/sink_attention/sink_flash_attention.py b/sink-flash-attention-kernel_amd/sink_attention/sink_flash_attention.py
--- a/sink-flash-attention-kernel_amd/sink_attention/sink_flash_attention.py
+++ b/sink-flash-attention-kernel_amd/sink_attention/sink_flash_attention.py
@@ -34,11 +34,14 @@
             o = torch.empty((B, H_q, Nq, D), device=q.device, dtype=q.dtype)
         lse = torch.empty((B, H_q, Nq), device=q.device, dtype=torch.float32)
         lib = N.lib()
+        ws_bytes = int(lib.sfa_fwd_workspace_bytes(B, H_q, k.shape[1], Nq, D, N.SFA_DTYPE[q.dtype], num_sink, window_size,
+                                                   flags))
+        ws = torch.empty((ws_bytes,), device=q.device, dtype=torch.uint8) if ws_bytes else None
         with torch.cuda.device(q.device):
-            st = lib.sfa_fwd(N.desc(q), N.desc(k), N.desc(v), N.desc(o), lse.data_ptr(),
-                             s_aux_f.data_ptr() if use_s_aux else None, num_sink, window_size, scale, flags,
-                             N.stream_ptr(q.device))
-        N.check(st, "sfa_fwd")
+            st = lib.sfa_fwd_ws(N.desc(q), N.desc(k), N.desc(v), N.desc(o), lse.data_ptr(),
+                                s_aux_f.data_ptr() if use_s_aux else None, num_sink, window_size, scale, flags,
+                                ws.data_ptr() if ws_bytes else None, ws_bytes, N.stream_ptr(q.device))
+        N.check(st, "sfa_fwd_ws")
 
         ctx.save_for_backward(q, k, v, o, lse, s_aux_f if use_s_aux else torch.empty(0, device=q.device))
         ctx.num_sink, ctx.window_size, ctx.scale = num_sink, window_size, scale
diff --git a/sink-flash-attention-kernel_amd/sink_attention/varlen.py b/sink-flash-attention-kernel_amd/sink_attention/varlen.py
--- a/sink-flash-attention-kernel_amd/sink_attention/varlen.py
+++ b/sink-flash-attention-kernel_amd/sink_attention/varlen.py
@@ -32,11 +32,15 @@
         o = alloc((1, H_q, T, D), device=q.device, dtype=q.dtype)
         lse = alloc((H_q, T), device=q.device, dtype=torch.float32)
         lib = N.lib()
+        ws_bytes = int(lib.sfa_fwd_varlen_workspace_bytes(H_q, k.shape[1], D, N.SFA_DTYPE[q.dtype], cu_dev.numel() - 1,
+                                                          max_seqlen, num_sink, window_size, 0))
+        ws = torch.empty((ws_bytes,), device=q.device, dtype=torch.uint8) if ws_bytes else None
         with torch.cuda.device(q.device):
-            st = lib.sfa_fwd_varlen(N.desc(q), N.desc(k), N.desc(v), N.desc(o), lse.data_ptr(),
-                                    s_aux_f.data_ptr() if use_s_aux else None, cu_dev.data_ptr(), cu_dev.numel() - 1,
-                                    max_seqlen, num_sink, window_size, scale, 0, N.stream_ptr(q.device))
-        N.check(st, "sfa_fwd_varlen")
+            st = lib.sfa_fwd_varlen_ws(N.desc(q), N.desc(k), N.desc(v), N.desc(o), lse.data_ptr(),
+                                       s_aux_f.data_ptr() if use_s_aux else None, cu_dev.data_ptr(), cu_dev.numel() - 1,
+                                       max_seqlen, num_sink, window_size, scale, 0, ws.data_ptr() if ws_bytes else None,
+                                       ws_bytes, N.stream_ptr(q.device))
+        N.check(st, "sfa_fwd_varlen_ws")
         ctx.save_for_backward(q, k, v, o, lse, cu_dev, s_aux_f if use_s_aux else torch.empty(0, device=q.device))
         ctx.cfg = (max_seqlen, num_sink, window_size, scale, use_s_aux, s_aux.dtype if use_s_aux else None, checked)
         return o
```

Result: no change. 984.6 (median of 6 runs) (+0.3%).
